# louiskirsch/speechT

Measured on AMD Instinct MI355X. Metric: utterances/sec (training step, 10 s@16 kHz, batch 32), higher is better.
Workload: dtype f32

## Files before the change

include/speecht_hip.h:

```cpp
#ifndef SPEECHT_HIP_H
#define SPEECHT_HIP_H

#include <stddef.h>
#include <stdint.h>

#ifdef __cplusplus
extern "C" {
#endif

#define ST_OK 0
#define ST_EINVAL (-1)
#define ST_ELAUNCH (-2)
#define ST_EWORKSPACE (-3)
#define ST_ECOMM (-4)

typedef struct st_tensor3 {
  float* base;
  int32_t batch;
  int32_t frames;
  int32_t channels;
  int32_t halo;
  int32_t t_pitch;
  int32_t c_pitch;
} st_tensor3;

int st_version(void);
const char* st_last_error(void);

int st_trace_begin(void);
int st_trace_begin_timed(void);
int st_trace_timed_filter(const char* text);
size_t st_trace_end(char* host_buf, size_t capacity);
int st_set_tuning(const char* name, int value);
uint32_t st_host_crc32c(const void* host_data, size_t n, uint32_t crc);

int st_packed_dims(int width, int cin_pitch, int cout, int* k_valid, int* k_pad, int* n_pad);
int st_pack_filters_f32(const float* filters, int width, int cin, int cout, int cin_pitch,
                        float* packed, void* stream);
int st_unpack_filters_f32(const float* packed, int width, int cin, int cout, int cin_pitch,
                          float* filters, void* stream);
int st_filters_flip_transpose_f32(const float* packed, int width, int cin, int cout,
                                  int cin_pitch, int cout_pitch, float* packed_t, void* stream);

int st_conv1d_nwc_fwd_f32(const st_tensor3* x, const float* packed, const float* bias, int width,
                          int stride, int pad_left, int relu, const st_tensor3* y, void* stream);
size_t st_conv1d_fwd_ws(const st_tensor3* x, const st_tensor3* y, int width);
int st_conv1d_nwc_fwd_ws_f32(const st_tensor3* x, const float* packed, const float* bias, int width,
                             int stride, int pad_left, int relu, const st_tensor3* y, void* workspace,
                             size_t workspace_bytes, void* stream);

int st_conv1d_fft_plan(int width, int frames, int batch, int* n, int* valid, int* blocks, int* bins, int* rows_pad);
int st_gemm_nn_batched_f32(const float* a, int64_t lda, int64_t a_batch, const float* b, int64_t b_batch, float* c,
                           int64_t ldc, int64_t c_batch, int m, int k, int n, int batches, void* stream);
size_t st_gemm_nn_batched_ws_bytes(void);
size_t st_gemm_nn_batched_ctrl_bytes(void);
int st_streamk_lost_ptr(void** device_word);
int st_streamk_lost_count(unsigned* count);
int st_streamk_lost_fetch_async(unsigned* host_word, void* stream);
int st_gemm_nn_batched_ws_f32(const float* a, int64_t lda, int64_t a_batch, const float* b, int64_t b_batch, float* c,
                              int64_t ldc, int64_t c_batch, int m, int k, int n, int batches, void* workspace,
                              size_t workspace_bytes, void* stream);
int st_gemm_nn_batched_bt_ws_f32(const float* a, int64_t lda, int64_t a_batch, const float* bt, int64_t bt_batch, float* c,
                                 int64_t ldc, int64_t c_batch, int m, int k, int n, int batches, void* workspace,
                                 size_t workspace_bytes, void* stream);
int st_gemm_tn_batched_f32(const float* a, int64_t lda, int64_t a_batch, const float* z, int64_t ldz, int64_t z_batch,
                           float* out, int64_t out_batch, int m, int k, int n, int batches, void* stream);
int st_gemm_tn_batched_shared_f32(const float* a, int64_t lda, int64_t a_batch, const float* z, int64_t ldz, int64_t z_batch,
                                  float* out, int64_t out_batch, int m, int k, int n, int batches, int z_batch_shift, void* stream);
int st_gemm_tn_batched_tile_f32(const float* a, int64_t lda, int64_t a_batch, const float* z, int64_t ldz, int64_t z_batch,
                                float* out, int64_t out_batch, int m, int k, int n, int batches, int z_batch_shift, int tile_n,
                                void* stream);
int st_gemm_nn_g3_batched_f32(const float* a, int64_t lda, int64_t a_batch, const int64_t* a_off, const float* b, int64_t ldb,
                              int64_t b_batch, const int64_t* b_off, int b_transposed, float* c, int64_t ldc, int64_t c_batch,
                              int64_t c_off2, int m, int k, int n, int batches, void* stream);
int st_gemm_tn_g3_batched_f32(const float* a, int64_t lda, int64_t a_batch, const int64_t* a_off, const float* z, int64_t ldz,
                              int64_t z_batch, const int64_t* z_off, float* out, int64_t out_batch, int64_t out_part, int m, int k,
                              int n, int batches, void* stream);
int st_conv1d_fft_three_products(int width, int cin_pitch, int cout);
size_t st_conv1d_fft_table_floats(void);
int st_conv1d_fft_tables_f32(int width, int pad_left, float* tables, size_t table_floats, void* stream);
size_t st_conv1d_fft_filter_floats(int width, int cin_pitch, int cout);
int st_conv1d_fft_filters_f32(const float* packed, int width, int cin, int cout, int cin_pitch, const float* tables, float* gfwd,
                              void* stream);
size_t st_conv1d_fft_sf_floats(const st_tensor3* x, const st_tensor3* y, int width);
size_t st_conv1d_fft_zf_floats(const st_tensor3* dz, int width);
size_t st_conv1d_fft_ws(const st_tensor3* x, const st_tensor3* y, int width);
int st_conv1d_nwc_fwd_fft_f32(const st_tensor3* x, const float* gfwd, const float* bias, int width, int pad_left, int relu,
                              const st_tensor3* y, const float* tables, float* sf, void* workspace,
                              size_t workspace_bytes, void* stream);
int st_conv1d_nwc_fwd_fft_chain_f32(const st_tensor3* x, const float* gfwd, const float* bias, int width, int pad_left, int relu,
                                    const st_tensor3* y, const float* tables, float* sf, int sf_ready, const float* next_tables,
                                    float* next_sf, int next_width, int next_pad_left, int* next_sf_written, void* workspace,
                                    size_t workspace_bytes, void* stream);
int st_conv1d_fft_dz_spectra_f32(const st_tensor3* dz, int width, const float* tables, float* zf, void* stream);
int st_conv1d_fft_bias_grad_f32(const st_tensor3* dz, int width, const float* zf, float* dbias, void* stream);
int st_conv1d_nwc_bwd_data_fft_f32(const st_tensor3* dz, const float* zf, const float* gfwd, int width, int pad_left,
                                   const st_tensor3* act, const st_tensor3* dx, const float* tables, void* workspace,
                                   size_t workspace_bytes, void* stream);
int st_conv1d_nwc_bwd_data_fft_chain_f32(const st_tensor3* dz, const float* zf, const float* gfwd, int width, int pad_left,
                                         const st_tensor3* act, const st_tensor3* dx, const float* tables, const float* below_tables,
                                         float* below_zf, int below_width, int* below_zf_written, void* workspace,
                                         size_t workspace_bytes, void* stream);
int st_conv1d_nwc_bwd_filter_fft_f32(const st_tensor3* x, const st_tensor3* dz, const float* sf, const float* zf, int width,
                                     const float* tables, float* dpacked, void* workspace, size_t workspace_bytes,
                                     void* stream);

size_t st_conv1d_fft_filter_plane_elems(int width, int cin_pitch, int cout);
int st_conv1d_fft_filters_planes(const float* packed, int width, int cin, int cout, int cin_pitch, const float* tables, void* g_planes,
                                 void* gt_planes, int planes, void* stream);
size_t st_conv1d_fft_planes_ws(const st_tensor3* x, const st_tensor3* y, int width, int planes);
int st_conv1d_nwc_fwd_fft_planes(const st_tensor3* x, const void* x_bf16, const void* gt_planes, const float* bias, int width,
                                 int pad_left, int relu, const st_tensor3* y, void* y_bf16, const float* tables, void* sf_planes,
                                 int planes, void* workspace, size_t workspace_bytes, void* stream);
int st_conv1d_fft_dz_spectra_planes(const st_tensor3* dz, const void* dz_bf16, int width, const float* tables, void* zf_planes,
                                    int planes, float* dc, void* stream);
int st_conv1d_fft_bias_grad_dc_f32(const float* dc, int rows, int channels, int n_pad, float* dbias, void* stream);
int st_conv1d_nwc_bwd_data_fft_planes(const st_tensor3* dz, const void* zf_planes, const void* g_planes, int width, int pad_left,
                                      const st_tensor3* act, const void* act_bf16, const st_tensor3* dx, void* dx_bf16,
                                      const float* tables, int planes, void* workspace, size_t workspace_bytes, void* stream);
int st_conv1d_nwc_bwd_filter_fft_planes(const st_tensor3* x, const st_tensor3* dz, const void* sf_planes, const void* zf_planes, int width,
                                        const float* tables, float* dpacked, int planes, void* workspace, size_t workspace_bytes,
                                        void* stream);

size_t st_conv1d_bwd_data_ws(const st_tensor3* dz, const st_tensor3* dx, int width);
int st_conv1d_nwc_bwd_data_f32(const st_tensor3* dz, const float* packed_t, int width,
                               int pad_left, const st_tensor3* act, const st_tensor3* dx,
                               void* workspace, size_t workspace_bytes, void* stream);
size_t st_conv1d_bwd_data_bias_ws(const st_tensor3* dz, const st_tensor3* dx, int width);
int st_conv1d_nwc_bwd_data_bias_f32(const st_tensor3* dz, const float* packed_t, int width, int pad_left,
                                    const st_tensor3* act, const st_tensor3* dx, float* dbias_dx,
                                    void* workspace, size_t workspace_bytes, void* stream);
int st_conv1d_1tap_bwd_data_bias_f32(const st_tensor3* dz, const float* packed, const st_tensor3* act, const st_tensor3* dx,
                                     float* dbias_dx, void* workspace, size_t workspace_bytes, void* stream);
size_t st_conv1d_bwd_filter_ws(const st_tensor3* x, const st_tensor3* dz, int width);
size_t st_bias_grad_ws(const st_tensor3* dz);
int st_bias_grad_f32(const st_tensor3* dz, float* dbias, void* workspace, size_t workspace_bytes, void* stream);
int st_conv1d_nwc_bwd_filter_f32(const st_tensor3* x, const st_tensor3* dz, int width, int stride,
                                 int pad_left, float* dpacked, float* dbias, void* workspace,
                                 size_t workspace_bytes, void* stream);

size_t st_ctc_ws(int batch, int frames, int max_label_len);
int st_ctc_loss_grad_f32(const st_tensor3* logits, const int32_t* label_ids,
                         const int32_t* label_offsets, const int32_t* seq_lens, int max_label_len,
                         float grad_scale, float* loss, const st_tensor3* grad, int32_t* status,
                         void* workspace, size_t workspace_bytes, void* stream);
int st_ctc_loss_grad_hilo_f32(const st_tensor3* logits, const int32_t* label_ids,
                              const int32_t* label_offsets, const int32_t* seq_lens, int max_label_len,
                              float grad_scale, float* loss, float* loss_lo, const st_tensor3* grad, int32_t* status,
                              void* workspace, size_t workspace_bytes, void* stream);

int st_ctc_greedy_decode(const st_tensor3* logits, const int32_t* seq_lens, int merge_repeated,
                         int32_t* ids, int max_out, int32_t* out_lens, float* neg_sum_logits,
                         void* stream);

size_t st_ctc_align_ws(int batch, int frames, int max_label_len);
int st_ctc_align_f32(const st_tensor3* logits, const int32_t* label_ids, const int32_t* label_offsets,
                     const int32_t* seq_lens, int max_label_len, int32_t* spans, int32_t* states, float* score,
                     int32_t* status, void* workspace, size_t workspace_bytes, void* stream);
int st_ctc_align_host(const float* logits, int batch, int frames, int classes, const int32_t* label_ids,
                      const int32_t* label_offsets, const int32_t* seq_lens, int max_label_len, int32_t* spans,
                      int32_t* states, float* score, int32_t* status, void* workspace, size_t workspace_bytes);

size_t st_ctc_align_long_ws(long frames, int label_len);
int st_ctc_align_long_f32(const float* logits, long frames, int classes, int row_pitch, const int32_t* label_ids, int label_len,
                          int32_t* spans, double* score, int32_t* status, void* workspace, size_t workspace_bytes,
                          void* stream);
int st_ctc_align_long_host(const float* logits, long frames, int classes, int row_pitch, const int32_t* label_ids, int label_len,
                           int32_t* spans, double* score, int32_t* status, void* workspace, size_t workspace_bytes);

size_t st_ctc_word_conf_ws(int batch, int frames, int max_label_len, int max_jobs);
int st_ctc_word_conf_f32(const st_tensor3* logits, const int32_t* label_ids, const int32_t* label_offsets,
                         const int32_t* seq_lens, int max_label_len, int space_id, const int32_t* word_spans, int n_words,
                         double* log_prob, double* log_conf, int32_t* status, void* workspace, size_t workspace_bytes,
                         void* stream);
int st_ctc_word_conf_host(const float* logits, int batch, int frames, int classes, const int32_t* label_ids,
                          const int32_t* label_offsets, const int32_t* seq_lens, int max_label_len, int space_id,
                          const int32_t* word_spans, int n_words, double* log_prob, double* log_conf, int32_t* status,
                          void* workspace, size_t workspace_bytes);

size_t st_ctc_spot_ws(int batch, int frames, int max_keyword_len, int n_jobs);
int st_ctc_spot_f32(const st_tensor3* logits, const int32_t* seq_lens, const int32_t* kw_ids, const int32_t* kw_offsets,
                    int n_keywords, int max_keyword_len, const int32_t* jobs, int n_jobs, double* score, int32_t* span,
                    double* trace_score, int32_t* trace_start, int32_t* status, void* workspace, size_t workspace_bytes,
                    void* stream);
int st_ctc_spot_host(const float* logits, int batch, int frames, int classes, const int32_t* seq_lens, const int32_t* kw_ids,
                     const int32_t* kw_offsets, int n_keywords, int max_keyword_len, const int32_t* jobs, int n_jobs,
                     double* score, int32_t* span, double* trace_score, int32_t* trace_start, int32_t* status, void* workspace,
                     size_t workspace_bytes);

size_t st_ctc_beam_ws(int batch, int frames, int beam_width);
int st_ctc_beam_search_decode(const st_tensor3* logits, const int32_t* seq_lens, int beam_width,
                              int32_t* ids, int max_out, int32_t* out_lens, float* log_prob,
                              void* workspace, size_t workspace_bytes, void* stream);
int st_ctc_beam_search_decode_ex(const st_tensor3* logits, const int32_t* seq_lens, int beam_width, int input_transform,
                                 int32_t* ids, int max_out, int32_t* out_lens, float* log_prob,
                                 void* workspace, size_t workspace_bytes, void* stream);

int st_lm_create_arpa(const char* text, size_t bytes, void** handle, char* err, size_t errlen);
int st_lm_info(void* handle, int* order, int64_t* counts, int64_t* skipped_words, int64_t* trie_nodes, size_t* device_bytes);
int st_lm_upload(void* handle, void* stream);
int st_lm_word_id(void* handle, const char* word, int32_t* id);
int st_lm_query_host(void* handle, const int32_t* ctx, int n, int32_t word, float* logp);
int st_lm_trie_lookup(void* handle, const char* prefix, int32_t* node, float* min_logp, int32_t* word);
int st_lm_destroy(void* handle);
int st_ctc_beam_search_decode_lm(const st_tensor3* logits, const int32_t* seq_lens, int beam_width, int input_transform, void* lm,
                                 float lm_weight, float word_count_weight, float valid_word_count_weight, float oov_score,
                                 int32_t* ids, int max_out, int32_t* out_lens, float* log_prob, void* workspace,
                                 size_t workspace_bytes, void* stream);
size_t st_ctc_beam_lm_candidates_ws(int batch, int frames, int beam_width, int candidates);
int st_ctc_beam_search_decode_lm_candidates(const st_tensor3* logits, const int32_t* seq_lens, int beam_width, int input_transform,
                                            void* lm, const float* weights, int candidates, float oov_score, int32_t* ids,
                                            int max_out, int32_t* out_lens, float* log_prob, void* workspace,
                                            size_t workspace_bytes, void* stream);

int st_ctc_beam_search_decode_nbest(const st_tensor3* logits, const int32_t* seq_lens, int beam_width, int input_transform, int n_best,
                                    int32_t* ids, int max_out, int32_t* out_lens, float* log_prob, int32_t* n_hyps, void* workspace,
                                    size_t workspace_bytes, void* stream);
int st_ctc_beam_search_decode_lm_nbest(const st_tensor3* logits, const int32_t* seq_lens, int beam_width, int input_transform, void* lm,
                                       float lm_weight, float word_count_weight, float valid_word_count_weight, float oov_score,
                                       int n_best, int32_t* ids, int max_out, int32_t* out_lens, float* log_prob, int32_t* n_hyps,
                                       void* workspace, size_t workspace_bytes, void* stream);

typedef struct st_bias_tables {
  const int32_t* next;
  const float* gain;
  const float* fin;
  int32_t n_states;
} st_bias_tables;
int st_ctc_beam_search_decode_bias_nbest(const st_tensor3* logits, const int32_t* seq_lens, int beam_width, int input_transform,
                                         const st_bias_tables* bias, int n_best, int32_t* ids, int max_out, int32_t* out_lens,
                                         float* log_prob, int32_t* n_hyps, void* workspace, size_t workspace_bytes, void* stream);
int st_ctc_beam_search_decode_lm_bias_nbest(const st_tensor3* logits, const int32_t* seq_lens, int beam_width, int input_transform,
                                            void* lm, float lm_weight, float word_count_weight, float valid_word_count_weight,
                                            float oov_score, const st_bias_tables* bias, int n_best, int32_t* ids, int max_out,
                                            int32_t* out_lens, float* log_prob, int32_t* n_hyps, void* workspace,
                                            size_t workspace_bytes, void* stream);

int st_lm_score_prefixes_f64(void* lm, const int32_t* ids, int pitch, const int32_t* lens, int n, double* g, int32_t* n_words,
                             int32_t* n_valid, void* stream);
int st_lm_score_prefixes_host(void* lm, const int32_t* ids, int pitch, const int32_t* lens, int n, double* g, int32_t* n_words,
                              int32_t* n_valid);

int st_edit_distance_max_len(void);
int st_edit_distance_pairs(const int32_t* expected, int expected_rows, int expected_pitch, const int32_t* expected_lens,
                           const int32_t* decoded, int decoded_rows, int decoded_pitch, const int32_t* decoded_lens,
                           const int32_t* pairs, int n_pairs, int32_t* distances, void* stream);

size_t st_global_norm_ws(size_t n);
int st_global_norm_clip_adam_f32(float* params, const float* grads, float* m, float* v, size_t n,
                                 float clip_norm, float lr_t, float beta1, float beta2, float eps,
                                 float* stats, void* workspace, size_t workspace_bytes,
                                 void* stream);
int st_ctc_status_gate_f32(const int32_t* status, int batch, float* gate, void* stream);
int st_ctc_status_gate_loss_f32(const int32_t* status, int batch, const float* loss_hi, const float* loss_lo, float loss_scale,
                                float* gate, void* stream);
int st_global_norm_clip_adam_gated_f32(float* params, const float* grads, float* m, float* v, size_t n,
                                       float clip_norm, float lr_t, float beta1, float beta2, float eps,
                                       float* stats, const float* gate, void* workspace,
// ... 224 lines not shown
```

speecht_amd/_lib.py:

```python
import ctypes
import os
from ctypes import POINTER, c_char_p, c_float, c_int, c_int32, c_int64, c_long, c_size_t, c_void_p

from .build import LIB_PATH


class Tensor3(ctypes.Structure):
  _fields_ = [('base', c_void_p), ('batch', c_int32), ('frames', c_int32), ('channels', c_int32),
              ('halo', c_int32), ('t_pitch', c_int32), ('c_pitch', c_int32)]


class BiasTables(ctypes.Structure):
  _fields_ = [('next', c_void_p), ('gain', c_void_p), ('fin', c_void_p), ('n_states', c_int32)]


class SpeechtHipError(RuntimeError):
  pass


_T3P = POINTER(Tensor3)
_SIGNATURES = {
    'st_version': (c_int, []),
    'st_last_error': (c_char_p, []),
    'st_trace_begin': (c_int, []),
    'st_trace_begin_timed': (c_int, []),
    'st_trace_timed_filter': (c_int, [c_char_p]),
    'st_trace_end': (c_size_t, [c_char_p, c_size_t]),
    'st_set_tuning': (c_int, [c_char_p, c_int]),
    'st_host_crc32c': (ctypes.c_uint32, [c_void_p, c_size_t, ctypes.c_uint32]),
    'st_packed_dims': (c_int, [c_int, c_int, c_int, POINTER(c_int), POINTER(c_int), POINTER(c_int)]),
    'st_pack_filters_f32': (c_int, [c_void_p, c_int, c_int, c_int, c_int, c_void_p, c_void_p]),
    'st_unpack_filters_f32': (c_int, [c_void_p, c_int, c_int, c_int, c_int, c_void_p, c_void_p]),
    'st_filters_flip_transpose_f32': (c_int, [c_void_p, c_int, c_int, c_int, c_int, c_int, c_void_p, c_void_p]),
    'st_conv1d_nwc_fwd_f32': (c_int, [_T3P, c_void_p, c_void_p, c_int, c_int, c_int, c_int, _T3P, c_void_p]),
    'st_conv1d_fwd_ws': (c_size_t, [_T3P, _T3P, c_int]),
    'st_conv1d_nwc_fwd_ws_f32': (c_int, [_T3P, c_void_p, c_void_p, c_int, c_int, c_int, c_int, _T3P, c_void_p, c_size_t,
                                          c_void_p]),
    'st_conv1d_fft_plan': (c_int, [c_int, c_int, c_int, POINTER(c_int), POINTER(c_int), POINTER(c_int), POINTER(c_int),
                                   POINTER(c_int)]),
    'st_gemm_nn_batched_f32': (c_int, [c_void_p, c_int64, c_int64, c_void_p, c_int64, c_void_p, c_int64, c_int64, c_int, c_int,
                                       c_int, c_int, c_void_p]),
    'st_gemm_nn_batched_ws_bytes': (c_size_t, []),
    'st_gemm_nn_batched_ctrl_bytes': (c_size_t, []),
    'st_streamk_lost_ptr': (c_int, [POINTER(c_void_p)]),
    'st_streamk_lost_count': (c_int, [POINTER(ctypes.c_uint32)]),
    'st_streamk_lost_fetch_async': (c_int, [c_void_p, c_void_p]),
    'st_gemm_nn_batched_ws_f32': (c_int, [c_void_p, c_int64, c_int64, c_void_p, c_int64, c_void_p, c_int64, c_int64, c_int, c_int,
                                          c_int, c_int, c_void_p, c_size_t, c_void_p]),
    'st_gemm_nn_batched_bt_ws_f32': (c_int, [c_void_p, c_int64, c_int64, c_void_p, c_int64, c_void_p, c_int64, c_int64, c_int, c_int,
                                             c_int, c_int, c_void_p, c_size_t, c_void_p]),
    'st_gemm_tn_batched_f32': (c_int, [c_void_p, c_int64, c_int64, c_void_p, c_int64, c_int64, c_void_p, c_int64, c_int, c_int,
                                       c_int, c_int, c_void_p]),
    'st_gemm_tn_batched_shared_f32': (c_int, [c_void_p, c_int64, c_int64, c_void_p, c_int64, c_int64, c_void_p, c_int64, c_int, c_int,
                                              c_int, c_int, c_int, c_void_p]),
    'st_gemm_tn_batched_tile_f32': (c_int, [c_void_p, c_int64, c_int64, c_void_p, c_int64, c_int64, c_void_p, c_int64, c_int, c_int,
                                            c_int, c_int, c_int, c_int, c_void_p]),
    'st_gemm_nn_g3_batched_f32': (c_int, [c_void_p, c_int64, c_int64, POINTER(c_int64), c_void_p, c_int64, c_int64, POINTER(c_int64), c_int,
                                          c_void_p, c_int64, c_int64, c_int64, c_int, c_int, c_int, c_int, c_void_p]),
    'st_gemm_tn_g3_batched_f32': (c_int, [c_void_p, c_int64, c_int64, POINTER(c_int64), c_void_p, c_int64, c_int64, POINTER(c_int64),
                                          c_void_p, c_int64, c_int64, c_int, c_int, c_int, c_int, c_void_p]),
    'st_conv1d_fft_three_products': (c_int, [c_int, c_int, c_int]),
    'st_conv1d_fft_table_floats': (c_size_t, []),
    'st_conv1d_fft_tables_f32': (c_int, [c_int, c_int, c_void_p, c_size_t, c_void_p]),
    'st_conv1d_fft_filter_floats': (c_size_t, [c_int, c_int, c_int]),
    'st_conv1d_fft_filters_f32': (c_int, [c_void_p, c_int, c_int, c_int, c_int, c_void_p, c_void_p, c_void_p]),
    'st_conv1d_fft_sf_floats': (c_size_t, [_T3P, _T3P, c_int]),
    'st_conv1d_fft_zf_floats': (c_size_t, [_T3P, c_int]),
    'st_conv1d_fft_ws': (c_size_t, [_T3P, _T3P, c_int]),
    'st_conv1d_nwc_fwd_fft_f32': (c_int, [_T3P, c_void_p, c_void_p, c_int, c_int, c_int, _T3P, c_void_p, c_void_p, c_void_p,
                                          c_size_t, c_void_p]),
    'st_conv1d_nwc_fwd_fft_chain_f32': (c_int, [_T3P, c_void_p, c_void_p, c_int, c_int, c_int, _T3P, c_void_p, c_void_p, c_int, c_void_p,
                                                c_void_p, c_int, c_int, POINTER(c_int), c_void_p, c_size_t, c_void_p]),
    'st_conv1d_nwc_bwd_data_fft_chain_f32': (c_int, [_T3P, c_void_p, c_void_p, c_int, c_int, _T3P, _T3P, c_void_p, c_void_p, c_void_p, c_int,
                                                     POINTER(c_int), c_void_p, c_size_t, c_void_p]),
    'st_conv1d_fft_filter_plane_elems': (c_size_t, [c_int, c_int, c_int]),
    'st_conv1d_fft_filters_planes': (c_int, [c_void_p, c_int, c_int, c_int, c_int, c_void_p, c_void_p, c_void_p, c_int, c_void_p]),
    'st_conv1d_fft_planes_ws': (c_size_t, [_T3P, _T3P, c_int, c_int]),
    'st_conv1d_nwc_fwd_fft_planes': (c_int, [_T3P, c_void_p, c_void_p, c_void_p, c_int, c_int, c_int, _T3P, c_void_p, c_void_p, c_void_p,
                                             c_int, c_void_p, c_size_t, c_void_p]),
    'st_conv1d_fft_dz_spectra_planes': (c_int, [_T3P, c_void_p, c_int, c_void_p, c_void_p, c_int, c_void_p, c_void_p]),
    'st_conv1d_fft_bias_grad_dc_f32': (c_int, [c_void_p, c_int, c_int, c_int, c_void_p, c_void_p]),
    'st_conv1d_nwc_bwd_data_fft_planes': (c_int, [_T3P, c_void_p, c_void_p, c_int, c_int, _T3P, c_void_p, _T3P, c_void_p, c_void_p, c_int,
                                                  c_void_p, c_size_t, c_void_p]),
    'st_conv1d_nwc_bwd_filter_fft_planes': (c_int, [_T3P, _T3P, c_void_p, c_void_p, c_int, c_void_p, c_void_p, c_int, c_void_p, c_size_t,
                                                    c_void_p]),
    'st_conv1d_fft_dz_spectra_f32': (c_int, [_T3P, c_int, c_void_p, c_void_p, c_void_p]),
    'st_conv1d_fft_bias_grad_f32': (c_int, [_T3P, c_int, c_void_p, c_void_p, c_void_p]),
    'st_conv1d_nwc_bwd_data_fft_f32': (c_int, [_T3P, c_void_p, c_void_p, c_int, c_int, _T3P, _T3P, c_void_p, c_void_p, c_size_t,
                                               c_void_p]),
    'st_conv1d_nwc_bwd_filter_fft_f32': (c_int, [_T3P, _T3P, c_void_p, c_void_p, c_int, c_void_p, c_void_p, c_void_p,
                                                 c_size_t, c_void_p]),
    'st_conv1d_bwd_data_ws': (c_size_t, [_T3P, _T3P, c_int]),
    'st_conv1d_nwc_bwd_data_f32': (c_int, [_T3P, c_void_p, c_int, c_int, _T3P, _T3P, c_void_p, c_size_t, c_void_p]),
    'st_conv1d_bwd_data_bias_ws': (c_size_t, [_T3P, _T3P, c_int]),
    'st_conv1d_nwc_bwd_data_bias_f32': (c_int, [_T3P, c_void_p, c_int, c_int, _T3P, _T3P, c_void_p, c_void_p, c_size_t,
                                                c_void_p]),
    'st_conv1d_1tap_bwd_data_bias_f32': (c_int, [_T3P, c_void_p, _T3P, _T3P, c_void_p, c_void_p, c_size_t, c_void_p]),
    'st_conv1d_bwd_filter_ws': (c_size_t, [_T3P, _T3P, c_int]),
    'st_conv1d_nwc_bwd_filter_f32': (c_int, [_T3P, _T3P, c_int, c_int, c_int, c_void_p, c_void_p, c_void_p,
                                             c_size_t, c_void_p]),
    'st_bias_grad_ws': (c_size_t, [_T3P]),
    'st_bias_grad_f32': (c_int, [_T3P, c_void_p, c_void_p, c_size_t, c_void_p]),
    'st_ctc_ws': (c_size_t, [c_int, c_int, c_int]),
    'st_ctc_loss_grad_f32': (c_int, [_T3P, c_void_p, c_void_p, c_void_p, c_int, c_float, c_void_p, _T3P,
                                     c_void_p, c_void_p, c_size_t, c_void_p]),
    'st_ctc_loss_grad_hilo_f32': (c_int, [_T3P, c_void_p, c_void_p, c_void_p, c_int, c_float, c_void_p, c_void_p, _T3P,
                                     c_void_p, c_void_p, c_size_t, c_void_p]),
    'st_ctc_greedy_decode': (c_int, [_T3P, c_void_p, c_int, c_void_p, c_int, c_void_p, c_void_p, c_void_p]),
    'st_ctc_align_ws': (c_size_t, [c_int, c_int, c_int]),
    'st_ctc_align_f32': (c_int, [_T3P, c_void_p, c_void_p, c_void_p, c_int, c_void_p, c_void_p, c_void_p, c_void_p,
                                 c_void_p, c_size_t, c_void_p]),
    'st_ctc_align_host': (c_int, [c_void_p, c_int, c_int, c_int, c_void_p, c_void_p, c_void_p, c_int, c_void_p, c_void_p,
                                  c_void_p, c_void_p, c_void_p, c_size_t]),
    'st_ctc_align_long_ws': (c_size_t, [c_long, c_int]),
    'st_ctc_align_long_f32': (c_int, [c_void_p, c_long, c_int, c_int, c_void_p, c_int, c_void_p, c_void_p, c_void_p, c_void_p,
                                      c_size_t, c_void_p]),
    'st_ctc_align_long_host': (c_int, [c_void_p, c_long, c_int, c_int, c_void_p, c_int, c_void_p, c_void_p, c_void_p, c_void_p,
                                       c_size_t]),
    'st_ctc_word_conf_ws': (c_size_t, [c_int, c_int, c_int, c_int]),
    'st_ctc_word_conf_f32': (c_int, [_T3P, c_void_p, c_void_p, c_void_p, c_int, c_int, c_void_p, c_int, c_void_p, c_void_p,
                                     c_void_p, c_void_p, c_size_t, c_void_p]),
    'st_ctc_word_conf_host': (c_int, [c_void_p, c_int, c_int, c_int, c_void_p, c_void_p, c_void_p, c_int, c_int, c_void_p, c_int,
                                      c_void_p, c_void_p, c_void_p, c_void_p, c_size_t]),
    'st_ctc_spot_ws': (c_size_t, [c_int, c_int, c_int, c_int]),
    'st_ctc_spot_f32': (c_int, [_T3P, c_void_p, c_void_p, c_void_p, c_int, c_int, c_void_p, c_int, c_void_p, c_void_p, c_void_p,
                                c_void_p, c_void_p, c_void_p, c_size_t, c_void_p]),
    'st_ctc_spot_host': (c_int, [c_void_p, c_int, c_int, c_int, c_void_p, c_void_p, c_void_p, c_int, c_int, c_void_p, c_int,
                                 c_void_p, c_void_p, c_void_p, c_void_p, c_void_p, c_void_p, c_size_t]),
    'st_ctc_beam_ws': (c_size_t, [c_int, c_int, c_int]),
    'st_ctc_beam_search_decode': (c_int, [_T3P, c_void_p, c_int, c_void_p, c_int, c_void_p, c_void_p, c_void_p,
                                          c_size_t, c_void_p]),
    'st_ctc_beam_search_decode_ex': (c_int, [_T3P, c_void_p, c_int, c_int, c_void_p, c_int, c_void_p, c_void_p, c_void_p,
                                             c_size_t, c_void_p]),
    'st_lm_create_arpa': (c_int, [c_char_p, c_size_t, POINTER(c_void_p), c_char_p, c_size_t]),
    'st_lm_info': (c_int, [c_void_p, POINTER(c_int), POINTER(c_int64), POINTER(c_int64), POINTER(c_int64), POINTER(c_size_t)]),
    'st_lm_upload': (c_int, [c_void_p, c_void_p]),
    'st_lm_word_id': (c_int, [c_void_p, c_char_p, POINTER(c_int32)]),
    'st_lm_query_host': (c_int, [c_void_p, POINTER(c_int32), c_int, c_int32, POINTER(c_float)]),
    'st_lm_trie_lookup': (c_int, [c_void_p, c_char_p, POINTER(c_int32), POINTER(c_float), POINTER(c_int32)]),
    'st_lm_destroy': (c_int, [c_void_p]),
    'st_ctc_beam_search_decode_lm': (c_int, [_T3P, c_void_p, c_int, c_int, c_void_p, c_float, c_float, c_float, c_float, c_void_p,
                                             c_int, c_void_p, c_void_p, c_void_p, c_size_t, c_void_p]),
    'st_ctc_beam_lm_candidates_ws': (c_size_t, [c_int, c_int, c_int, c_int]),
    'st_ctc_beam_search_decode_lm_candidates': (c_int, [_T3P, c_void_p, c_int, c_int, c_void_p, POINTER(c_float), c_int, c_float,
                                                        c_void_p, c_int, c_void_p, c_void_p, c_void_p, c_size_t, c_void_p]),
    'st_ctc_beam_search_decode_nbest': (c_int, [_T3P, c_void_p, c_int, c_int, c_int, c_void_p, c_int, c_void_p, c_void_p, c_void_p,
                                                c_void_p, c_size_t, c_void_p]),
    'st_ctc_beam_search_decode_lm_nbest': (c_int, [_T3P, c_void_p, c_int, c_int, c_void_p, c_float, c_float, c_float, c_float, c_int,
                                                   c_void_p, c_int, c_void_p, c_void_p, c_void_p, c_void_p, c_size_t, c_void_p]),
    'st_ctc_beam_search_decode_bias_nbest': (c_int, [_T3P, c_void_p, c_int, c_int, c_void_p, c_int, c_void_p, c_int, c_void_p, c_void_p,
                                                     c_void_p, c_void_p, c_size_t, c_void_p]),
    'st_ctc_beam_search_decode_lm_bias_nbest': (c_int, [_T3P, c_void_p, c_int, c_int, c_void_p, c_float, c_float, c_float, c_float,
                                                        c_void_p, c_int, c_void_p, c_int, c_void_p, c_void_p, c_void_p, c_void_p,
                                                        c_size_t, c_void_p]),
    'st_lm_score_prefixes_f64': (c_int, [c_void_p, c_void_p, c_int, c_void_p, c_int, c_void_p, c_void_p, c_void_p, c_void_p]),
    'st_lm_score_prefixes_host': (c_int, [c_void_p, c_void_p, c_int, c_void_p, c_int, c_void_p, c_void_p, c_void_p]),
    'st_edit_distance_max_len': (c_int, []),
    'st_edit_distance_pairs': (c_int, [c_void_p, c_int, c_int, c_void_p, c_void_p, c_int, c_int, c_void_p, c_void_p, c_int, c_void_p,
                                       c_void_p]),
    'st_global_norm_ws': (c_size_t, [c_size_t]),
    'st_global_norm_clip_adam_f32': (c_int, [c_void_p, c_void_p, c_void_p, c_void_p, c_size_t, c_float, c_float,
                                             c_float, c_float, c_float, c_void_p, c_void_p, c_size_t, c_void_p]),
    'st_ctc_status_gate_f32': (c_int, [c_void_p, c_int, c_void_p, c_void_p]),
    'st_ctc_status_gate_loss_f32': (c_int, [c_void_p, c_int, c_void_p, c_void_p, c_float, c_void_p, c_void_p]),
    'st_global_norm_clip_adam_gated_f32': (c_int, [c_void_p, c_void_p, c_void_p, c_void_p, c_size_t, c_float, c_float,
                                                   c_float, c_float, c_float, c_void_p, c_void_p, c_void_p, c_size_t,
                                                   c_void_p]),
    'st_global_norm_clip_adam_counted_f32': (c_int, [c_void_p, c_void_p, c_void_p, c_void_p, c_size_t, c_float, ctypes.c_double,
                                                     ctypes.c_double, ctypes.c_double, c_float, c_void_p, c_void_p, c_void_p, c_void_p,
                                                     c_size_t, c_void_p]),
    'st_global_norm_f32': (c_int, [c_void_p, c_size_t, c_float, c_void_p, c_void_p, c_size_t, c_void_p]),
    'st_melspec_plan_bytes': (c_size_t, []),
    'st_melspec_plan_f32': (c_int, [c_void_p, c_int, c_int, c_void_p, c_size_t, c_void_p]),
    'st_melspec_planned_f32': (c_int, [c_void_p, c_void_p, c_int, c_int64, c_void_p, c_int, c_int, c_int, c_void_p,
                                       c_int64, c_void_p, c_void_p, c_size_t, c_void_p]),
    'st_melspec_ws': (c_size_t, [c_int, c_int64, c_int]),
    'st_melspec_f32': (c_int, [c_void_p, c_void_p, c_int, c_int64, c_void_p, c_int, c_int, c_int, c_void_p,
                               c_int64, c_void_p, c_void_p, c_size_t, c_void_p]),
    'st_cast_bf16': (c_int, [c_void_p, c_size_t, c_void_p, c_void_p]),
    'st_filters_bf16': (c_int, [c_void_p, c_int, c_int, c_void_p, c_void_p]),
    'st_filters_bwd_bf16': (c_int, [c_void_p, c_int, c_int, c_int, c_int, c_int, c_void_p, c_void_p]),
    'st_conv1d_nwc_fwd_bf16': (c_int, [_T3P, c_void_p, c_void_p, c_void_p, c_int, c_int, c_int, c_int, _T3P, c_void_p,
                                       c_void_p, c_void_p]),
    'st_conv1d_fwd_bf16_ws': (c_size_t, [_T3P, _T3P, c_int]),
    'st_conv1d_nwc_fwd_ws_bf16': (c_int, [_T3P, c_void_p, c_void_p, c_void_p, c_int, c_int, c_int, c_int, _T3P, c_void_p,
                                          c_void_p, c_void_p, c_size_t, c_void_p]),
    'st_conv1d_bwd_data_bf16_ws': (c_size_t, [_T3P, _T3P, c_int]),
    'st_conv1d_nwc_bwd_data_bf16': (c_int, [_T3P, c_void_p, c_void_p, c_int, c_int, _T3P, c_void_p, _T3P, c_void_p,
                                            c_void_p, c_size_t, c_void_p]),
    'st_conv1d_bwd_filter_bf16_ws': (c_size_t, [_T3P, _T3P, c_int, c_int, c_int]),
    'st_conv1d_nwc_bwd_filter_bf16': (c_int, [_T3P, c_void_p, _T3P, c_void_p, c_int, c_int, c_int, c_void_p, c_void_p,
                                              c_void_p, c_size_t, c_void_p]),
    'st_conv1d_bwd_filter_tr_bf16_slack_rows': (c_int, []),
    'st_conv1d_bwd_filter_tr_bf16_ws': (c_size_t, [_T3P, _T3P, c_int, c_int, c_int]),
    'st_conv1d_nwc_bwd_filter_tr_bf16': (c_int, [_T3P, c_void_p, _T3P, c_void_p, c_int, c_int, c_int, c_void_p, c_void_p,
                                                 c_void_p, c_size_t, c_void_p]),
    'st_comm_unique_id_bytes': (c_int, []),
    'st_comm_unique_id': (c_int, [c_void_p, c_size_t]),
    'st_comm_init': (c_int, [c_void_p, c_size_t, c_int, c_int, POINTER(c_void_p)]),
    'st_comm_destroy': (c_int, [c_void_p]),
    'st_comm_count': (c_int, [c_void_p, POINTER(c_int)]),
    'st_allreduce_f32': (c_int, [c_void_p, c_void_p, c_size_t, c_void_p]),
    'st_allreduce_buckets_f32': (c_int, [c_void_p, c_void_p, POINTER(c_size_t), POINTER(c_size_t), c_int, c_void_p]),
    'st_mfcc_ws': (c_size_t, [c_int, c_int64, c_int, c_int]),
    'st_mfcc_f32': (c_int, [c_void_p, c_void_p, c_int, c_int64, c_void_p, c_int, c_int, c_int, c_int, c_void_p,
                            c_int64, c_void_p, c_void_p, c_size_t, c_void_p]),
    'st_resample_kaiser_f32': (c_int, [c_void_p, c_void_p, c_int, c_void_p, c_int, c_void_p, c_void_p, c_int64, c_void_p, c_int64,
                                       c_void_p, c_void_p]),
    'st_resample_kaiser_host': (c_int, [c_void_p, c_void_p, c_int, c_void_p, c_int, c_void_p, c_void_p, c_void_p, c_int64, c_void_p]),
    'st_resample_stream_state_bytes': (c_size_t, [c_int, c_int]),
    'st_resample_stream_f32': (c_int, [c_void_p, c_void_p, c_int, c_int, c_void_p, c_int64, c_void_p, c_size_t, c_int, c_void_p, c_int64,
                                       c_void_p, c_void_p]),
    'st_resample_stream_host': (c_int, [c_void_p, c_void_p, c_int, c_int, c_void_p, c_int64, c_void_p, c_size_t, c_int, c_void_p, c_void_p,
                                        c_int64, c_void_p]),
    'st_segment_chunks_f32': (c_int, [c_void_p, c_void_p, c_void_p, c_void_p, c_int, c_int64, c_float, c_void_p, c_void_p, c_void_p,
                                      c_void_p, c_void_p, c_void_p]),
    'st_segment_runs': (c_int, [c_void_p, c_void_p, c_void_p, c_int, c_int, c_int, c_void_p, c_void_p, c_void_p, c_void_p, c_void_p,
                                c_void_p, c_void_p, c_void_p]),
    'st_segment_gather_f32': (c_int, [c_void_p, c_void_p, c_void_p, c_void_p, c_void_p, c_int, c_int64, c_void_p, c_void_p]),
    'st_mask_rows': (c_int, [_T3P, c_void_p, c_int, c_void_p]),
    'st_stream_conv_slices': (c_int, [c_int, c_int, c_int, POINTER(c_int), POINTER(c_int)]),
    'st_stream_conv_ws': (c_size_t, [c_int, c_int, c_int, c_int]),
    'st_stream_conv_f32': (c_int, [c_void_p, c_int, c_int, c_void_p, c_void_p, c_int, c_int, c_void_p, c_void_p, c_int, c_int, c_int,
                                   c_int, c_void_p, c_int, c_int, c_void_p, c_void_p, c_size_t, c_void_p]),
    'st_stream_feed_f32': (c_int, [c_void_p, c_int, c_void_p, c_int, c_int, c_void_p, c_int, c_int, c_void_p]),
    'st_stream_advance': (c_int, [c_void_p, c_int, c_void_p, c_int, c_void_p]),
    'st_melspec_stream_state_bytes': (c_size_t, [c_int, c_int, c_int, c_int]),
    'st_melspec_stream_ws': (c_size_t, [c_int, c_int]),
    'st_melspec_stream_f32': (c_int, [c_void_p, c_void_p, c_int, c_int, c_void_p, c_int, c_int, c_int, c_int, c_int, c_float, c_float,
                                      c_float, c_void_p, c_size_t, c_void_p, c_int, c_int, c_void_p, c_size_t, c_void_p]),
    'st_ctc_greedy_stream': (c_int, [c_void_p, c_int, c_int, c_void_p, c_void_p, c_int, c_void_p, c_void_p, c_void_p, c_int, c_void_p,
                                     c_void_p, c_void_p]),
    'st_ctc_beam_stream_state_bytes': (c_size_t, [c_int, c_int]),
    'st_ctc_beam_stream_pool_bytes': (c_size_t, [c_int, c_int]),
    'st_ctc_beam_stream_ws': (c_size_t, [c_int]),
    'st_ctc_beam_stream_step': (c_int, [c_void_p, c_int, c_int, c_void_p, c_void_p, c_int, c_int, c_int, c_int, c_void_p, c_float, c_float,
                                        c_float, c_float, c_void_p, c_void_p, c_int, c_void_p, c_size_t, c_void_p]),
    'st_ctc_beam_stream_read': (c_int, [c_void_p, c_int, c_int, c_void_p, c_float, c_float, c_float, c_float, c_void_p, c_void_p, c_int,
                                        c_void_p, c_int, c_void_p, c_void_p]),
    'st_stream_endpoint_state_bytes': (c_size_t, []),
    'st_stream_endpoint_score_bytes': (c_size_t, []),
    'st_stream_endpoint_pieces': (c_int, [c_int, c_int, c_int, c_int]),
    'st_ctc_greedy_endpoint_stream': (c_int, [c_void_p, c_int, c_int, c_void_p, c_void_p, c_int, c_int, c_int, c_int, c_int, c_int, c_void_p,
                                              c_void_p, c_void_p, c_int, c_void_p, c_void_p, c_void_p, c_void_p, c_int, c_void_p]),
    'st_stream_endpoint_host': (c_int, [c_void_p, c_int, c_int, c_void_p, c_void_p, c_int, c_int, c_int, c_int, c_int, c_int, c_void_p,
                                        c_void_p, c_void_p, c_int, c_void_p, c_void_p, c_void_p, c_void_p, c_int]),
    'st_ctc_beam_stream_step_pieces': (c_int, [c_void_p, c_int, c_int, c_void_p, c_void_p, c_int, c_int, c_int, c_int, c_int, c_void_p,
                                               c_float, c_float, c_float, c_float, c_void_p, c_void_p, c_int, c_void_p, c_size_t, c_void_p,
                                               c_int, c_void_p, c_void_p]),
    'st_ctc_beam_stream_bias_state_bytes': (c_size_t, [c_int, c_int]),
    'st_ctc_beam_stream_step_bias': (c_int, [c_void_p, c_int, c_int, c_void_p, c_void_p, c_int, c_int, c_int, c_int, c_void_p, c_float,
                                             c_float, c_float, c_float, c_void_p, c_void_p, c_int, c_void_p, c_size_t, c_void_p, c_void_p,
                                             c_void_p]),
    'st_ctc_beam_stream_read_bias': (c_int, [c_void_p, c_int, c_int, c_void_p, c_float, c_float, c_float, c_float, c_void_p, c_void_p,
                                             c_int, c_void_p, c_int, c_void_p, c_void_p, c_void_p, c_void_p]),
    'st_ctc_beam_stream_step_pieces_bias': (c_int, [c_void_p, c_int, c_int, c_void_p, c_void_p, c_int, c_int, c_int, c_int, c_int, c_void_p,
                                                    c_float, c_float, c_float, c_float, c_void_p, c_void_p, c_int, c_void_p, c_size_t,
                                                    c_void_p, c_int, c_void_p, c_void_p, c_void_p, c_void_p]),
    'st_ctc_beam_stream_read_nbest': (c_int, [c_void_p, c_int, c_int, c_void_p, c_float, c_float, c_float, c_float, c_void_p, c_void_p,
                                              c_int, c_void_p, c_int, c_void_p, c_void_p, c_void_p, c_void_p, c_int, c_void_p, c_int,
                                              c_void_p]),
    'st_ctc_beam_stream_step_pieces_nbest': (c_int, [c_void_p, c_int, c_int, c_void_p, c_void_p, c_int, c_int, c_int, c_int, c_int, c_void_p,
                                                     c_float, c_float, c_float, c_float, c_void_p, c_void_p, c_int, c_void_p, c_size_t,
                                                     c_void_p, c_int, c_void_p, c_void_p, c_void_p, c_void_p, c_int, c_void_p, c_int,
                                                     c_void_p]),
    'st_stream_keep_rows': (c_int, [c_int, c_int]),
    'st_stream_keep_f32': (c_int, [c_void_p, c_int, c_int, c_void_p, c_int, c_int, c_void_p, c_int, c_void_p]),
    'st_ctc_align_ring_f32': (c_int, [c_void_p, c_int, c_int, c_int, c_void_p, c_int, c_int, c_void_p, c_void_p, c_int, c_void_p, c_void_p,
                                      c_void_p, c_void_p, c_void_p, c_size_t, c_void_p]),
    'st_ctc_align_ring_host': (c_int, [c_void_p, c_int, c_int, c_int, c_void_p, c_int, c_int, c_void_p, c_void_p, c_int, c_void_p, c_void_p,
                                       c_void_p, c_void_p, c_void_p, c_size_t]),
    'st_ctc_word_conf_ring_f32': (c_int, [c_void_p, c_int, c_int, c_int, c_void_p, c_int, c_int, c_void_p, c_void_p, c_int, c_int, c_void_p,
                                          c_int, c_void_p, c_void_p, c_void_p, c_void_p, c_size_t, c_void_p]),
    'st_ctc_word_conf_ring_host': (c_int, [c_void_p, c_int, c_int, c_int, c_void_p, c_int, c_int, c_void_p, c_void_p, c_int, c_int, c_void_p,
                                           c_int, c_void_p, c_void_p, c_void_p, c_void_p, c_size_t]),
    'st_ctc_spot_stream_plan_bytes': (c_size_t, [c_void_p, c_void_p, c_int, c_int, c_int]),
    'st_ctc_spot_stream_plan': (c_int, [c_void_p, c_void_p, c_int, c_int, c_int, c_void_p, c_void_p]),
    'st_ctc_spot_stream_plan_bind': (c_int, [c_void_p, c_void_p]),
    'st_ctc_spot_stream_state_bytes': (c_size_t, [c_void_p]),
    'st_ctc_spot_stream_step': (c_int, [c_void_p, c_int, c_int, c_void_p, c_void_p, c_int, c_int, c_void_p, ctypes.c_double, c_int,
                                        c_void_p, c_void_p, c_int, c_void_p, c_void_p]),
    'st_ctc_spot_stream_host': (c_int, [c_void_p, c_int, c_int, c_void_p, c_void_p, c_int, c_int, c_void_p, ctypes.c_double, c_int,
                                        c_void_p, c_void_p, c_int, c_void_p]),
    'st_ctc_follow_stream_state_bytes': (c_size_t, [c_int]),
    'st_ctc_follow_stream_ws': (c_size_t, [c_int, c_int, c_int]),
    'st_ctc_follow_stream_step': (c_int, [c_void_p, c_int, c_int, c_void_p, c_void_p, c_int, c_int, c_int, c_int, c_void_p, c_void_p,
                                          c_void_p, c_void_p, c_int, c_int, c_void_p, c_void_p, c_int, c_void_p, c_void_p, c_void_p,
                                          c_size_t, c_void_p]),
    'st_ctc_follow_stream_host': (c_int, [c_void_p, c_int, c_int, c_void_p, c_void_p, c_int, c_int, c_int, c_int, c_void_p, c_void_p,
                                          c_void_p, c_void_p, c_int, c_int, c_void_p, c_void_p, c_int, c_void_p, c_void_p, c_void_p,
                                          c_size_t]),
    'st_spec_augment_f32': (c_int, [c_void_p, c_int, c_int, c_int, c_void_p, c_void_p, ctypes.c_uint64, c_int, c_int, c_int, c_int, c_int,
                                    c_int, _T3P, c_void_p, c_void_p]),
    'st_spec_augment_host': (c_int, [c_void_p, c_int, c_int, c_int, c_void_p, c_void_p, ctypes.c_uint64, c_int, c_int, c_int, c_int, c_int,
                                     c_int, _T3P, c_void_p]),
    'st_spec_augment_plan_host': (c_int, [c_void_p, c_void_p, c_int, c_int, ctypes.c_uint64, c_int, c_int, c_int, c_int, c_int, c_int,
                                          c_void_p]),
    'st_fill_f32': (c_int, [c_void_p, c_float, c_size_t, c_void_p]),
    'st_zero_halos_f32': (c_int, [_T3P, c_void_p]),
    'st_zero_regions': (c_int, [c_void_p, c_int, c_void_p]),
}
EXPORTED_SYMBOLS = tuple(_SIGNATURES)

_EXPERIMENTAL = {
    'st_exp_split3_bf16': (c_int, [c_void_p, c_size_t, c_void_p, c_void_p]),
    'st_exp_split3_transpose_bf16': (c_int, [c_void_p, c_int, c_int, c_void_p, c_void_p]),
    'st_exp_conv1d_fwd_bf16x6': (c_int, [_T3P, c_void_p, c_void_p, c_void_p, c_int, c_int, c_int, c_int, _T3P,
                                         c_void_p, c_void_p]),
    'st_exp_conv1d_bwd_data_bf16x6_ws': (c_size_t, [_T3P, _T3P, c_int]),
    'st_exp_conv1d_bwd_data_bf16x6': (c_int, [_T3P, c_void_p, c_void_p, c_int, c_int, _T3P, _T3P, c_void_p, c_void_p, c_size_t,
                                              c_void_p]),
    'st_exp_transpose_split3_bf16': (c_int, [_T3P, c_int, c_int, c_int, c_size_t, c_void_p, c_void_p]),
    'st_exp_conv1d_bwd_filter_bf16x6': (c_int, [c_void_p, c_void_p, c_int, c_int, c_int, c_int, c_int, c_int, c_void_p, c_void_p]),
}

_lib = None


def load():
  global _lib
  if _lib is None:
    import torch
    bundled = os.path.join(os.path.dirname(torch.__file__), 'lib', 'libamdhip64.so')
    if os.path.exists(bundled):
      ctypes.CDLL(bundled, mode=ctypes.RTLD_GLOBAL)
    if not os.path.exists(LIB_PATH):
      raise SpeechtHipError('{} is missing: build it with `python -c "import __graft_entry__ as g; g.build()"` '
                            '(there is no CPU fallback)'.format(LIB_PATH))
    lib = ctypes.CDLL(LIB_PATH)
    for name, (res, args) in list(_SIGNATURES.items()) + list(_EXPERIMENTAL.items()):
      fn = getattr(lib, name)
      fn.restype = res
      fn.argtypes = args
    _lib = lib
    for item in filter(None, os.environ.get('ST_TUNE', '').split(',')):
      name, _, value = item.partition('=')
      check(lib.st_set_tuning(name.strip().encode(), int(value)), 'ST_TUNE ' + item)
  return _lib


def check(code, what):
  if code != 0:
    raise SpeechtHipError('{} failed ({}): {}'.format(what, code, load().st_last_error().decode()))


def call(name, *args):
  check(getattr(load(), name)(*args), name)


class launch_trace:

  def __init__(self, timed=False, only=None):
    self.timed, self.only = timed, only

  def __enter__(self):
    if self.timed:
      load().st_trace_timed_filter((self.only or '').encode())
      load().st_trace_begin_timed()
    else:
      load().st_trace_begin()
    self.lines = []
    return self

  def __exit__(self, *exc):
    lib = load()
    need = lib.st_trace_end(None, 0)
    buf = ctypes.create_string_buffer(int(need))
    lib.st_trace_end(buf, need)
    self.lines = [l for l in buf.value.decode().split('\n') if l]
    return False


TUNING_EPOCH = [0]


def set_tuning(name, value):
  TUNING_EPOCH[0] += 1
  call('st_set_tuning', name.encode(), int(value))
```

speecht_amd/csrc/api.hip:

```cpp
#include <algorithm>
#include <atomic>
#include <mutex>
#include <string>
#include <vector>
#include <string.h>

#include "st_common.h"

namespace st {
static thread_local char g_err[512] = "";
void set_error(const char* fmt, ...) {
  va_list ap;
  va_start(ap, fmt);
  vsnprintf(g_err, sizeof(g_err), fmt, ap);
  va_end(ap);
}

static std::atomic<int> g_trace_on{0};
static std::mutex g_trace_mu;
static std::vector<std::string> g_lines;
constexpr int kMaxTimed = 1 << 14;
struct TimedLaunch { int line; hipEvent_t e0, e1; };
static std::vector<TimedLaunch> g_timed;
static thread_local int g_last_line = -1;
static std::string g_timed_filter;
bool trace_on() { return g_trace_on.load(std::memory_order_relaxed) != 0; }
void trace(const char* fmt, ...) {
  if (!trace_on()) return;
  char line[320];
  va_list ap;
  va_start(ap, fmt);
  vsnprintf(line, sizeof(line), fmt, ap);
  va_end(ap);
  std::lock_guard<std::mutex> lock(g_trace_mu);
  if (g_lines.size() < (1u << 16)) {
    g_last_line = (int)g_lines.size();
    g_lines.emplace_back(line);
  } else {
    g_last_line = -1;
  }
}
LaunchTimer::LaunchTimer(hipStream_t) : start_(nullptr), stop_(nullptr) {
  const int line = g_last_line;
  g_last_line = -1;
  if (g_trace_on.load(std::memory_order_relaxed) != 2 || line < 0) return;
  hipEvent_t e0 = nullptr, e1 = nullptr;
  if (hipEventCreate(&e0) != hipSuccess) return;
  if (hipEventCreate(&e1) != hipSuccess) { hipEventDestroy(e0); return; }
  std::lock_guard<std::mutex> lock(g_trace_mu);
  if ((int)g_timed.size() >= kMaxTimed || line >= (int)g_lines.size() ||
      (!g_timed_filter.empty() && g_lines[line].find(g_timed_filter) == std::string::npos)) {
    hipEventDestroy(e0);
    hipEventDestroy(e1);
    return;
  }
  g_timed.push_back(TimedLaunch{line, e0, e1});
  start_ = e0;
  stop_ = e1;
}

static const char* const kTuneNames[TUNE_COUNT] = {"streamk", "streamk_slots", "streamk_test_drop", "no_fused_transforms",
                                                   "bf16_lag_copies", "filters_idft_valu", "bf16_taps_panel", "no_g3", "g3_tile"};
static std::atomic<int> g_tune[TUNE_COUNT];
int tuning(int key) { return g_tune[key].load(std::memory_order_relaxed); }
}

extern "C" {
int st_version(void) { return 200; }
const char* st_last_error(void) { return st::g_err; }

static int trace_begin(int mode) {
  std::lock_guard<std::mutex> lock(st::g_trace_mu);
  st::g_lines.clear();
  for (auto& t : st::g_timed) { hipEventDestroy(t.e0); hipEventDestroy(t.e1); }
  st::g_timed.clear();
  st::g_last_line = -1;
  st::g_trace_on.store(mode);
  return ST_OK;
}
int st_trace_begin(void) { return trace_begin(1); }
int st_trace_begin_timed(void) { return trace_begin(2); }
int st_trace_timed_filter(const char* text) {
  std::lock_guard<std::mutex> lock(st::g_trace_mu);
  st::g_timed_filter = text ? text : "";
  return ST_OK;
}

size_t st_trace_end(char* host_buf, size_t capacity) {
  st::g_trace_on.store(0);
  std::lock_guard<std::mutex> lock(st::g_trace_mu);
  for (auto& t : st::g_timed) {
    float ms = -1.f;
    if (hipEventSynchronize(t.e1) != hipSuccess || hipEventElapsedTime(&ms, t.e0, t.e1) != hipSuccess) ms = -1.f;
    char tail[48];
    snprintf(tail, sizeof(tail), " ms=%.5f", ms);
    if (t.line >= 0 && t.line < (int)st::g_lines.size()) st::g_lines[t.line] += tail;
    hipEventDestroy(t.e0);
    hipEventDestroy(t.e1);
  }
  st::g_timed.clear();
  size_t need = 1;
  for (const auto& l : st::g_lines) need += l.size() + 1;
  if (host_buf && capacity > 0) {
    size_t at = 0;
    for (const auto& l : st::g_lines) {
      if (at + l.size() + 1 >= capacity) break;
      memcpy(host_buf + at, l.data(), l.size());
      at += l.size();
      host_buf[at++] = '\n';
    }
    host_buf[at] = 0;
  }
  return need;
}

uint32_t st_host_crc32c(const void* host_data, size_t n, uint32_t crc) {
  static uint32_t table[8][256];
  static std::once_flag once;
  std::call_once(once, [] {
    for (uint32_t i = 0; i < 256; ++i) {
      uint32_t c = i;
      for (int k = 0; k < 8; ++k) c = (c >> 1) ^ (0x82F63B78u & (0u - (c & 1u)));
      table[0][i] = c;
    }
    for (uint32_t i = 0; i < 256; ++i)
      for (int t = 1; t < 8; ++t) table[t][i] = (table[t - 1][i] >> 8) ^ table[0][table[t - 1][i] & 0xFF];
  });
  const unsigned char* p = reinterpret_cast<const unsigned char*>(host_data);
  crc = ~crc;
  while (n >= 8) {
    uint32_t lo, hi;
    memcpy(&lo, p, 4);
    memcpy(&hi, p + 4, 4);
    lo ^= crc;
    crc = table[7][lo & 0xFF] ^ table[6][(lo >> 8) & 0xFF] ^ table[5][(lo >> 16) & 0xFF] ^ table[4][lo >> 24] ^
          table[3][hi & 0xFF] ^ table[2][(hi >> 8) & 0xFF] ^ table[1][(hi >> 16) & 0xFF] ^ table[0][hi >> 24];
    p += 8;
    n -= 8;
  }
  while (n--) crc = (crc >> 8) ^ table[0][(crc ^ *p++) & 0xFF];
  return ~crc;
}

int st_set_tuning(const char* name, int value) {
  ST_REQUIRE(name, "st_set_tuning: null name");
  for (int i = 0; i < st::TUNE_COUNT; ++i)
    if (!strcmp(name, st::kTuneNames[i])) {
      st::g_tune[i].store(value);
      return ST_OK;
    }
  st::set_error("st_set_tuning: unknown knob '%s'", name);
  return ST_EINVAL;
}
}
```

speecht_amd/csrc/conv_fft.hip:

```cpp
#include <algorithm>

#include "st_common.h"

namespace {

typedef float f32x2 __attribute__((ext_vector_type(2)));
typedef float f32x4 __attribute__((ext_vector_type(4)));
typedef float f32x16 __attribute__((ext_vector_type(16)));

constexpr int V = 64;
constexpr int KP = 96;
constexpr int HB = KP / 2;
constexpr int T_FS = 0;
constexpr int T_FZ = T_FS + KP * KP;
constexpr int T_IY = T_FZ + KP * KP;
constexpr int T_IX = T_IY + V * KP;
constexpr int T_TW = T_IX + 3 * V * KP;
constexpr int T_FW = T_TW + 256;
constexpr int T_FP = T_FW + HB * 34 * 2;
constexpr int FUSE_BLOCKS = 8, FUSE_HALO = 4, FUSE_Q = 32 + FUSE_HALO;
constexpr int T_IW = T_FP + FUSE_Q * KP * 2;
constexpr int T_ZP = T_IW + KP * KP;
constexpr int T_END = T_ZP + 32 * KP * 2;
__host__ __device__ inline int fused_column(int q, int hh, int n, int pad_left) {
  const int right = n - V - pad_left;
  if (q < 32) return pad_left + 32 * (q >> 4) + (q & 3) + 8 * ((q & 15) >> 2) + 4 * hh;
  if (hh == 0) return (q - 32) < pad_left ? (q - 32) : -1;
  return (q - 32) < right ? V + pad_left + (q - 32) : -1;
}

int half_of(int cp) { return (int)st::round_up(cp, 64); }

struct Plan {
  int n, blocks, bins, rows, rows_pad;
};
constexpr int ROWS_F32 = 64;
Plan make_plan(int width, int frames, int batch, int row_granule = 128) {
  Plan p;
  p.n = V + width - 1;
  p.blocks = st::ceil_div(frames, V);
  p.bins = p.n / 2 + 1;
  p.rows = batch * p.blocks;
  p.rows_pad = (int)st::round_up(p.rows, row_granule);
  return p;
}

__global__ void tables_kernel(int n, int pad_left, float* __restrict__ t) {
  const int bins = n / 2 + 1, width = n - V + 1;
  const float inv_n = 1.f / (float)n;
  for (int i = blockIdx.x * blockDim.x + threadIdx.x; i < T_END; i += gridDim.x * blockDim.x) {
    float val = 0.f;
    if (i < T_IY) {
      const int z = i >= T_FZ, r = (i - (z ? T_FZ : T_FS)) / KP, col = (i - (z ? T_FZ : T_FS)) % KP;
      const int k = r < HB ? r : r - HB;
      if (k < bins && col < (z ? V : n)) {
        float sn, cs;
        sincospif(2.0f * (float)((k * col) % n) * inv_n, &sn, &cs);
        val = r < HB ? cs : -sn;
      }
    } else if (i < T_TW) {
      const int which = i < T_IX ? 0 : 1 + (i - T_IX) / (V * KP);
      const int rem = i < T_IX ? i - T_IY : (i - T_IX) % (V * KP);
      const int tp = rem / KP, col = rem % KP;
      const int k = col < HB ? col : col - HB;
      int m = tp;
      if (which == 1) m = tp + pad_left;
      if (which == 2) m = tp + V + pad_left;
      if (which == 3) m = tp - V + pad_left;
      if (k < bins && m >= 0 && m < n) {
        const float wk = (k == 0 || 2 * k == n) ? inv_n : 2.f * inv_n;
        float sn, cs;
        sincospif(2.0f * (float)((k * m) % n) * inv_n, &sn, &cs);
        val = col < HB ? wk * cs : -wk * sn;
      }
    } else if (i < T_FW) {
      const int j = (i - T_TW) / 2;
      if (j < n) {
        float sn, cs;
        sincospif(2.0f * (float)j * inv_n, &sn, &cs);
        val = (i - T_TW) % 2 ? sn : cs;
      }
    } else if (i < T_FP) {
      const int e = (i - T_FW) / 2, k = e / width, w = e % width;
      if (k < bins) {
        float sn, cs;
        sincospif(2.0f * (float)((k * w) % n) * inv_n, &sn, &cs);
        val = (i - T_FW) % 2 ? sn : cs;
      }
    } else if (i < T_IW) {
      const int e = i - T_FP, q = e / (KP * 2), r = (e - q * (KP * 2)) >> 1, hh = e & 1;
      const int k = r < HB ? r : r - HB, col = fused_column(q, hh, n, pad_left);
      if (k < bins && col >= 0 && col < n) {
        float sn, cs;
        sincospif(2.0f * (float)((k * col) % n) * inv_n, &sn, &cs);
        val = r < HB ? cs : -sn;
      }
    } else if (i < T_ZP) {
      const int e = i - T_IW, r = e / KP, col = e % KP;
      const int k = col < HB ? col : col - HB;
      int m = -1;
      if (r < V) m = r + pad_left;
      else if (r < V + 4) m = (r - V) < pad_left ? r - V : -1;
      else if (r < V + 8) m = (r - V - 4) < width - 1 - pad_left ? V + pad_left + (r - V - 4) : -1;
      if (k < bins && m >= 0 && m < n) {
        const float wk = (k == 0 || 2 * k == n) ? inv_n : 2.f * inv_n;
        float sn, cs;
        sincospif(2.0f * (float)((k * m) % n) * inv_n, &sn, &cs);
        val = col < HB ? wk * cs : -wk * sn;
      }
    } else {
      const int e = i - T_ZP, q = e / (KP * 2), r = (e - q * (KP * 2)) >> 1, hh = e & 1;
      const int k = r < HB ? r : r - HB, col = fused_column(q, hh, V, 0);
      if (k < bins && col < V) {
        float sn, cs;
        sincospif(2.0f * (float)((k * col) % n) * inv_n, &sn, &cs);
        val = r < HB ? cs : -sn;
      }
    }
    t[i] = val;
  }
}

struct RowsIn {
  const float* base;
  const unsigned short* base_b;
  long batch_stride;
  int c_pitch, channels_read;
  int t_lo, t_hi;
};

constexpr int CH = 12;

template <int R, int COUNT = 1>
__device__ inline void stage_matrix(float* __restrict__ dst, const float* __restrict__ src) {
  constexpr int IT = R * KP / 4 / 256;
  static_assert(IT * 256 * 4 == R * KP, "the matrix must be a whole number of 256-thread passes");
  f32x4 v[COUNT * IT];
#pragma unroll
  for (int it = 0; it < COUNT * IT; ++it) v[it] = reinterpret_cast<const f32x4*>(src)[threadIdx.x + 256 * it];
#pragma unroll
  for (int it = 0; it < COUNT * IT; ++it) {
    const int m = it / IT, i = threadIdx.x + 256 * (it % IT);
    const int row = (i * 4) / KP, k = (i * 4) % KP;
    f32x2* d = reinterpret_cast<f32x2*>(dst + m * R * KP) + ((k >> 1) * R + row);
    d[0] = f32x2{v[it][0], v[it][1]};
    d[R] = f32x2{v[it][2], v[it][3]};
  }
}

__device__ __forceinline__ void split3_bits(float x, unsigned short& h, unsigned short& m, unsigned short& l) {
  const __bf16 bh = (__bf16)x;
  const float r1 = x - (float)bh;
  const __bf16 bm = (__bf16)r1;
  const __bf16 bl = (__bf16)(r1 - (float)bm);
// ... 320 lines not shown
    else { if (j + 1 < blocks && e < right_next) v = halo[j + 1][0][e][l31]; }
#pragma unroll
    for (int i = 0; i < 3; ++i) sacc[i] = __builtin_amdgcn_mfma_f32_32x32x2f32(af2[((32 + e) * KP + i * 32) * 2], v, sacc[i], 0, 0, 0);
  }
  if (c < half_next) {
#pragma unroll
    for (int i = 0; i < 3; ++i)
#pragma unroll
      for (int r = 0; r < 16; ++r) {
        const int m = i * 32 + (r & 3) + 8 * (r >> 2) + 4 * h;
        const int bin = m < HB ? m : m - HB, col = (m < HB ? 0 : half_next) + c;
        if (bin < bins_next) {
          const long o = (long)bin * bin_stride + (long)row * 2 * half_next;
          out[o + col] = sacc[i][r];
          if (out2) out2[o + (m < HB ? half_next : 0) + c] = m < HB ? -sacc[i][r] : sacc[i][r];
        }
      }
  }
}

template <int HP>
__global__ __launch_bounds__(64 * FUSE_BLOCKS, 1) void idft_ola_dft_rows_kernel(
    const float* __restrict__ in, const float* __restrict__ winv, int blocks, int rows_pad, int bins, int half_in, int nchunks, RowsOut y,
    int pad_left, int right, const float* __restrict__ mask, long mask_batch_stride, int mask_c_pitch,
    const float* __restrict__ wz_below, int bins_below, int half_below, float* __restrict__ zf_below) {
  constexpr int NST = 2 * HP / CH;
  static_assert(2 * HP % CH == 0 && HP <= HB / 2, "pairs per term must fill whole stages");
  __shared__ __attribute__((aligned(16))) float wl[KP * KP];
  __shared__ __attribute__((aligned(16))) float wf[32 * KP * 2];
  constexpr int SPILL = FUSE_BLOCKS * FUSE_HALO * 32;
  constexpr bool SPILL_IN_WL = (HB / 2 - HP) * KP * 2 >= SPILL;
  __shared__ float spill_own[SPILL_IN_WL ? 32 : 2 * SPILL];
  float* const spill_before = SPILL_IN_WL ? wl + HP * KP * 2 : spill_own;
  float* const spill_after = SPILL_IN_WL ? wl + (HB / 2 + HP) * KP * 2 : spill_own + SPILL;
  const int tid = threadIdx.x, lane = tid & 63, l31 = lane & 31, h = lane >> 5;
  const int wave = __builtin_amdgcn_readfirstlane(tid >> 6);
  const int b = blockIdx.x / nchunks, chunk = blockIdx.x - b * nchunks;
  const int j = wave, row = b * blocks + j, c = chunk * 32 + l31;
  const bool active = j < blocks;
  const long plane = (long)rows_pad * 2 * half_in;
  const bool cok = c < half_in;
  const float* src = in + (long)(active ? row : 0) * 2 * half_in + min(c, half_in - 1);
  auto load = [&](float (&bf)[CH], int st) {
#pragma unroll
    for (int s = 0; s < CH; ++s) {
      const int p = st * CH + s;
      const int bin = (p < HP ? 2 * p : 2 * (p - HP)) + h;
      bf[s] = src[(long)min(bin, bins - 1) * plane + (p < HP ? 0 : half_in)];
    }
  };
  float bfr[NST][CH];
  float mk[2][16];
  if (active) {
#pragma unroll
    for (int st = 0; st < NST; ++st) load(bfr[st], st);
    if (mask) {
      const float* mp = mask + (long)b * mask_batch_stride + min(c, mask_c_pitch - 1);
#pragma unroll
      for (int i = 0; i < 2; ++i)
#pragma unroll
        for (int r = 0; r < 16; ++r)
          mk[i][r] = mp[(long)min(j * V + i * 32 + (r & 3) + 8 * (r >> 2) + 4 * h, y.frames - 1) * mask_c_pitch];
    }
  }
  if (tid < 256) stage_matrix<KP, 1>(wl, winv);
  if (wz_below) {
    constexpr int N4 = 32 * KP * 2 / 4;
    for (int idx = tid; idx < N4; idx += 64 * FUSE_BLOCKS) reinterpret_cast<f32x4*>(wf)[idx] = reinterpret_cast<const f32x4*>(wz_below)[idx];
  }
  __syncthreads();
  f32x16 acc[3];
#pragma unroll
  for (int i = 0; i < 3; ++i)
#pragma unroll
    for (int r = 0; r < 16; ++r) acc[i][r] = 0.f;
  if (active) {
    const float* afrag = wl + 2 * l31 + h;
#pragma unroll
    for (int st = 0; st < NST; ++st) {
      __builtin_amdgcn_sched_barrier(0);
#pragma unroll
      for (int s = 0; s < CH; ++s) {
        const int p = st * CH + s;
        const int bin = (p < HP ? 2 * p : 2 * (p - HP)) + h;
        const unsigned keep = (cok && bin < bins) ? 0xffffffffu : 0u;
        const float v = __uint_as_float(__float_as_uint(bfr[st][s]) & keep);
        const int sidx = p < HP ? p : HB / 2 + (p - HP);
#pragma unroll
        for (int i = 0; i < 3; ++i) acc[i] = __builtin_amdgcn_mfma_f32_32x32x2f32(afrag[(sidx * KP + i * 32) * 2], v, acc[i], 0, 0, 0);
      }
      __builtin_amdgcn_sched_barrier(0);
    }
#pragma unroll
    for (int e = 0; e < FUSE_HALO; ++e) (h ? spill_after : spill_before)[(j * FUSE_HALO + e) * 32 + l31] = acc[2][e];
  }
  __syncthreads();
  if (!active) return;
#pragma unroll
  for (int e = 0; e < FUSE_HALO; ++e) {
    if (h == 0) { if (j > 0 && e < right) acc[0][e] += spill_after[((j - 1) * FUSE_HALO + e) * 32 + l31]; }
    else { if (j + 1 < blocks && e >= FUSE_HALO - pad_left) acc[1][12 + e] += spill_before[((j + 1) * FUSE_HALO + e - (FUSE_HALO - pad_left)) * 32 + l31]; }
  }
#pragma unroll
  for (int i = 0; i < 2; ++i)
#pragma unroll
    for (int r = 0; r < 16; ++r) {
      const int t = j * V + i * 32 + (r & 3) + 8 * (r >> 2) + 4 * h;
      float val = c < y.channels ? acc[i][r] : 0.f;
      if (mask) val = mk[i][r] > 0.f ? val : 0.f;
      val = t < y.frames ? val : 0.f;
      asm volatile("" : "+v"(val));
      acc[i][r] = val;
    }
  if (c < y.c_pitch) {
    float* yp = y.base + (long)b * y.batch_stride + c;
#pragma unroll
    for (int i = 0; i < 2; ++i)
#pragma unroll
      for (int r = 0; r < 16; ++r) {
        const int t = j * V + i * 32 + (r & 3) + 8 * (r >> 2) + 4 * h;
        if (t < y.frames) yp[(long)t * y.c_pitch] = acc[i][r];
      }
  }
  if (!wz_below) return;
  f32x16 sacc[3];
#pragma unroll
  for (int i = 0; i < 3; ++i)
#pragma unroll
    for (int r = 0; r < 16; ++r) sacc[i][r] = 0.f;
  const float* af2 = wf + 2 * l31 + h;
#pragma unroll
  for (int q = 0; q < 32; ++q) {
    const float v = acc[q >> 4][q & 15];
#pragma unroll
    for (int i = 0; i < 3; ++i) sacc[i] = __builtin_amdgcn_mfma_f32_32x32x2f32(af2[(q * KP + i * 32) * 2], v, sacc[i], 0, 0, 0);
  }
  if (c < half_below) {
    const long zplane = (long)rows_pad * 2 * half_below;
#pragma unroll
    for (int i = 0; i < 3; ++i)
#pragma unroll
      for (int r = 0; r < 16; ++r) {
        const int m = i * 32 + (r & 3) + 8 * (r >> 2) + 4 * h;
        const int bin = m < HB ? m : m - HB, col = (m < HB ? 0 : half_below) + c;
        if (bin < bins_below) zf_below[(long)bin * zplane + (long)row * 2 * half_below + col] = sacc[i][r];
      }
  }
}

template <int WT, int OUTP = 0>
__global__ __launch_bounds__(256) void filters_dft_fwd_kernel(const float* __restrict__ packed, int width_rt, int cin, int cout,
                                                              int cpi, int cph, int npo, int n, int bins,
                                                              const f32x2* __restrict__ tw, float* __restrict__ gfwd,
                                                              unsigned short* __restrict__ gb, size_t g_plane) {
  const int width = WT ? WT : width_rt;
  const int o = blockIdx.x * 256 + threadIdx.x, c = blockIdx.y;
  if (o >= npo) return;
  float f[WT ? WT : 64];
  const bool live = c < cin && o < cout;
#pragma unroll
  for (int w = 0; w < width; ++w) f[w] = live ? packed[((long)w * cpi + c) * npo + o] : 0.f;
  const long plane = (long)2 * cph * 2 * npo;
  const int per = (bins + gridDim.z - 1) / gridDim.z, k_lo = blockIdx.z * per, k_hi = min(bins, k_lo + per);
  for (int k = k_lo; k < k_hi; ++k) {
    float gr = 0.f, gi = 0.f;
    const f32x2* row = tw + k * width;
#pragma unroll
    for (int w = 0; w < width; ++w) {
      const f32x2 t = row[w];
      gr = fmaf(f[w], t[0], gr);
      gi = fmaf(-f[w], t[1], gi);
    }
    auto put = [&](long o_, float v) {
      if (OUTP == 0) gfwd[o_] = v;
      else if (OUTP == 1) gb[o_] = __builtin_bit_cast(unsigned short, (__bf16)v);
      else {
        unsigned short sh, sm, sl;
        split3_bits(v, sh, sm, sl);
        gb[o_] = sh; gb[g_plane + o_] = sm; gb[2 * g_plane + o_] = sl;
      }
    };
    if constexpr (OUTP == 4) {
      const long g3 = (long)k * 3 * cph * npo + (long)c * npo + o;
      gfwd[g3] = gr;
      gfwd[g3 + (long)cph * npo] = gi - gr;
      gfwd[g3 + 2L * cph * npo] = -(gr + gi);
      continue;
    }
    const long g0 = (long)k * plane;
    put(g0 + (long)c * 2 * npo + o, gr);
    put(g0 + (long)c * 2 * npo + npo + o, -gi);
    put(g0 + (long)(cph + c) * 2 * npo + o, gi);
    put(g0 + (long)(cph + c) * 2 * npo + npo + o, gr);
  }
}

template <int WT>
__global__ __launch_bounds__(256) void filters_idft_kernel(const float* __restrict__ q, int width_rt, int cin, int cout, int cpi, int cph,
                                                           int npo, int n, int bins, const f32x2* __restrict__ tw,
                                                           float* __restrict__ dpacked, int split) {
  const int width = WT ? WT : width_rt;
  const int o = blockIdx.x * 256 + threadIdx.x, c = blockIdx.y;
  if (o >= npo) return;
  float acc[WT ? WT : 64];
#pragma unroll
  for (int w = 0; w < width; ++w) acc[w] = 0.f;
  const bool live = c < cin && o < cout;
  const long plane = split ? (long)2 * cph * npo : (long)2 * cph * 2 * npo;
  const float inv_n = 1.f / (float)n;
  if (live) {
    for (int k = 0; k < bins; ++k) {
      const float* p = q + (long)k * plane;
      const float wk = (k == 0 || 2 * k == n) ? inv_n : 2.f * inv_n;
      float re, im;
      if (split) {
        re = p[(long)c * npo + o] * wk;
        im = p[(long)cph * npo + (long)c * npo + o] * wk;
      } else {
        re = (p[(long)c * 2 * npo + o] + p[(long)(cph + c) * 2 * npo + npo + o]) * wk;
        im = (p[(long)(cph + c) * 2 * npo + o] - p[(long)c * 2 * npo + npo + o]) * wk;
      }
      const f32x2* row = tw + k * width;
#pragma unroll
      for (int w = 0; w < width; ++w) {
        const f32x2 t = row[w];
        acc[w] = fmaf(re, t[0], acc[w]);
        acc[w] = fmaf(-im, t[1], acc[w]);
      }
    }
  }
#pragma unroll
  for (int w = 0; w < width; ++w) dpacked[((long)w * cpi + c) * npo + o] = acc[w];
}

constexpr int FI_CH = 12;
constexpr int FI_SMAX = 96;
struct IdftParts { long off[4]; };
template <int VW>
__global__ __launch_bounds__(256, 2) void filters_idft_mfma_kernel(const float* __restrict__ q, int width, int cin, int cout, int cpi,
                                                                   int npo, int n, int bins, const f32x2* __restrict__ tw,
                                                                   float* __restrict__ dpacked, int pshift, long plane, IdftParts parts,
                                                                   int ld, int ochunks, int items) {
  typedef float vec __attribute__((ext_vector_type(VW)));
  __shared__ float tl[FI_SMAX * 32 * 2];
  const int nparts = 1 << pshift, S = (nparts * bins) >> 1, stages = (S + FI_CH - 1) / FI_CH;
  {
    const float inv_n = 1.f / (float)n;
    for (int i = threadIdx.x; i < stages * FI_CH * 64; i += 256) {
      const int hh = i & 1, m = (i >> 1) & 31, sidx = i >> 6;
      float v = 0.f;
      if (sidx < S && m < width) {
        const int kk = 2 * sidx + hh, k = kk >> pshift, part = kk & (nparts - 1);
        const float wk = (k == 0 || 2 * k == n) ? inv_n : 2.f * inv_n;
        const f32x2 t = tw[k * width + m];
        if (nparts == 2) v = part == 0 ? wk * t[0] : -wk * t[1];
        else v = part < 2 ? wk * t[0] : (part == 2 ? -wk * t[1] : wk * t[1]);
      }
      tl[i] = v;
    }
  }
  __syncthreads();
  const int lane = threadIdx.x & 63, l31 = lane & 31, h = lane >> 5;
  const int gw = blockIdx.x * 4 + (threadIdx.x >> 6), total = gridDim.x * 4;
  const float* afrag = tl + 2 * l31 + h;
  for (int item = gw; item < items; item += total) {
    const int c = item / ochunks, o0 = (item - c * ochunks) * (32 * VW) + l31 * VW;
    f32x16 acc[VW];
#pragma unroll
    for (int e = 0; e < VW; ++e)
#pragma unroll
      for (int r = 0; r < 16; ++r) acc[e][r] = 0.f;
    if (c < cin) {
      const float* base = q + (long)c * ld + o0;
      auto load = [&](vec (&bf)[FI_CH], int st) {
#pragma unroll
        for (int j = 0; j < FI_CH; ++j) {
          const int kk = 2 * min(st * FI_CH + j, S - 1) + h;
          bf[j] = *reinterpret_cast<const vec*>(base + (long)(kk >> pshift) * plane + parts.off[kk & (nparts - 1)]);
        }
      };
      auto mac = [&](const vec (&bf)[FI_CH], int st) {
        const float* a = afrag + st * (FI_CH * 64);
#pragma unroll
        for (int j = 0; j < FI_CH; ++j)
#pragma unroll
          for (int e = 0; e < VW; ++e) {
            acc[e] = __builtin_amdgcn_mfma_f32_32x32x2f32(a[j * 64], bf[j][e], acc[e], 0, 0, 0);
          }
      };
      vec bfr[2][FI_CH];
      load(bfr[0], 0);
      for (int st = 0; st < stages; st += 2) {
        if (st + 1 < stages) load(bfr[1], st + 1);
        __builtin_amdgcn_sched_barrier(0);
        mac(bfr[0], st);
        __builtin_amdgcn_sched_barrier(0);
        if (st + 1 < stages) {
          if (st + 2 < stages) load(bfr[0], st + 2);
          __builtin_amdgcn_sched_barrier(0);
          mac(bfr[1], st + 1);
          __builtin_amdgcn_sched_barrier(0);
        }
      }
    }
    if (c < cpi) {
#pragma unroll
      for (int r = 0; r < 16; ++r) {
        const int w = (r & 3) + 8 * (r >> 2) + 4 * h;
        if (w < width) {
          vec v;
#pragma unroll
          for (int e = 0; e < VW; ++e) {
            v[e] = o0 + e < cout ? acc[e][r] : 0.f;
          }
          *reinterpret_cast<vec*>(dpacked + ((long)w * cpi + c) * npo + o0) = v;
        }
      }
    }
  }
}

__global__ __launch_bounds__(256) void bias_from_spectra_kernel(const float* __restrict__ zf, int rows, int ld, int channels, int np,
                                                                float* __restrict__ dbias) {
  __shared__ float red[8][33];
  const int cl = threadIdx.x & 31, r = threadIdx.x >> 5;
  const int c = blockIdx.x * 32 + cl;
  float s = 0.f;
  if (c < channels) {
    float p0 = 0.f, p1 = 0.f, p2 = 0.f, p3 = 0.f;
    int k = r;
    for (; k + 24 < rows; k += 32) {
      const float a = zf[(long)k * ld + c], b = zf[(long)(k + 8) * ld + c], d = zf[(long)(k + 16) * ld + c],
                  e = zf[(long)(k + 24) * ld + c];
      p0 += a; p1 += b; p2 += d; p3 += e;
    }
    for (; k < rows; k += 8) p0 += zf[(long)k * ld + c];
    s = (p0 + p1) + (p2 + p3);
  }
  red[r][cl] = s;
  __syncthreads();
  if (r == 0 && c < np) {
    float t = red[0][cl];
#pragma unroll
    for (int k = 1; k < 8; ++k) t += red[k][cl];
    dbias[c] = t;
  }
}

RowsIn rows_in(const st_tensor3& t) {
  RowsIn r;
  r.base_b = nullptr;
  r.base = t.base + (long)t.halo * t.c_pitch;
  r.batch_stride = (long)t.t_pitch * t.c_pitch;
  r.c_pitch = t.c_pitch;
  r.channels_read = t.c_pitch;
  r.t_lo = -t.halo;
  r.t_hi = t.t_pitch - t.halo;
  return r;
}

constexpr int TRANSFORM_WGS_DEFAULT = 512;

void launch_dft(const st_tensor3& t, const void* tb, const Plan& pl, const float* wm, int start, int frames_used, int half, float* out,
                void* outb, int planes, size_t out_plane, float* dc, hipStream_t s, long bin_stride = 0, float* out2 = nullptr,
                int form = 0) {
  if (bin_stride == 0) bin_stride = (long)pl.rows_pad * (form == 4 ? 4 : form == 5 ? 3 : 2) * half;
  const int nchunks = st::ceil_div(half, 32);
  const int wgs = std::min(TRANSFORM_WGS_DEFAULT, st::ceil_div(pl.rows_pad * nchunks, 4));
  const int nst = frames_used <= 6 * CH ? 3 : 4;
  const double esz_in = tb ? 2.0 : 4.0, esz_out = planes == 0 ? 4.0 : 2.0 * planes;
  st::trace("dft_rows<%d%s%s> rows=%d chunks=%d bins=%d gflop=%.3f mb=%.2f", nst, tb ? ",bf16-in" : "",
            planes == 1 ? ",bf16-out" : planes == 3 ? ",x3-out" : form == 4 ? ",4-part" : form == 5 ? ",3-part" : "",
            pl.rows, nchunks, pl.bins, 4096e-9 * pl.rows * (double)nchunks * nst * CH * 3,
            1e-6 * ((double)t.batch * t.frames * t.c_pitch * esz_in +
                    (double)pl.bins * pl.rows * half * esz_out * (form == 4 ? 4 : form == 5 ? 3 : out2 ? 4 : 2)));
  RowsIn x = rows_in(t);
  if (tb) x.base_b = reinterpret_cast<const unsigned short*>(tb) + (long)t.halo * t.c_pitch;
  unsigned short* ob = reinterpret_cast<unsigned short*>(outb);
  st::LaunchTimer timer(s);
#define ST_DFT(NSTV, INB, OUTPV)                                                                                         \
  st::launch_timed(timer, dft_rows_kernel<NSTV, INB, OUTPV>, dim3(wgs), dim3(256), s, x, wm, pl.blocks, pl.rows, pl.rows_pad, start, \
                   pl.bins, half, nchunks, out, ob, out_plane, dc, bin_stride, out2)
#define ST_DFT_N(INB, OUTPV) do { if (nst == 3) ST_DFT(3, INB, OUTPV); else ST_DFT(4, INB, OUTPV); } while (0)
  if (!tb && planes == 0 && form == 4) ST_DFT_N(false, 4);
  else if (!tb && planes == 0 && form == 5) ST_DFT_N(false, 5);
  else if (!tb && planes == 0) ST_DFT_N(false, 0);
  else if (!tb && planes == 3) ST_DFT_N(false, 3);
  else if (tb && planes == 1) ST_DFT_N(true, 1);
  else st::set_error("dft: unsupported operand form (bf16 in: %d, planes %d)", tb ? 1 : 0, planes);
#undef ST_DFT_N
#undef ST_DFT
}

template <int TERMS>
void launch_idft(const float* in, const float* winv, const Plan& p, int half_in, int nchunks, const RowsOut& out, const float* bias,
                 int relu, const void* mask, long mask_batch_stride, int mask_c_pitch, hipStream_t s) {
  const dim3 grid(std::min(TRANSFORM_WGS_DEFAULT, st::ceil_div(p.rows * nchunks, 4)));
  const int hp = p.bins <= 36 ? 18 : 24;
  const bool bf = out.base_b != nullptr;
  st::trace("idft_rows<%d,%d%s> rows=%d chunks=%d bins=%d gflop=%.3f mb=%.2f", TERMS, hp, bf ? ",bf16" : "", p.rows, nchunks, p.bins,
            4096e-9 * p.rows * (double)nchunks * 2 * hp * (TERMS + 1),
            1e-6 * ((double)p.bins * p.rows * 2 * half_in * 4 + (double)p.rows * V * out.c_pitch * (bf ? 2.0 : 4.0) * (mask ? 2 : 1)));
  const float* mk = reinterpret_cast<const float*>(mask);
  st::LaunchTimer timer(s);
#define ST_IDFT(HPV, BFV)                                                                                                     \
  st::launch_timed(timer, idft_rows_kernel<TERMS, HPV, BFV>, grid, dim3(256), s, in, winv, p.blocks, p.rows, p.rows_pad, p.bins, half_in, \
                   nchunks, out, bias, relu, mk, mask_batch_stride, mask_c_pitch)
  if (p.bins <= 36) { if (bf) ST_IDFT(18, true); else ST_IDFT(18, false); }
  else { if (bf) ST_IDFT(24, true); else ST_IDFT(24, false); }
#undef ST_IDFT
}

bool width_ok(int width) { return width >= 2 && V + width - 1 <= KP && (V + width - 1) / 2 + 1 <= HB; }
constexpr int G3_MIN_WIDTH = 2 * FUSE_HALO + 2;
bool zf3_form(int width, int cout) { return width >= G3_MIN_WIDTH && st::npad_of(cout) >= 512 && st::tuning(st::TUNE_NO_G3) == 0; }
bool g3_form(int width, int cin_pitch, int cout) { return zf3_form(width, cout) && half_of(cin_pitch) % 128 == 0; }
bool split_lag_products(int half) { return half % 128 == 0; }

template <int OUTP>
void launch_filters_planes(int width, const dim3& grid, hipStream_t s, const float* packed, int cin, int cout, int cin_pitch, int cph,
                           int npo, int n, int bins, const f32x2* tw, unsigned short* gb, size_t g_plane) {
  float* none = nullptr;
  if (width == 32) hipLaunchKernelGGL((filters_dft_fwd_kernel<32, OUTP>), grid, dim3(256), 0, s, packed, width, cin, cout, cin_pitch, cph, npo, n, bins, tw, none, gb, g_plane);
  else if (width == 25) hipLaunchKernelGGL((filters_dft_fwd_kernel<25, OUTP>), grid, dim3(256), 0, s, packed, width, cin, cout, cin_pitch, cph, npo, n, bins, tw, none, gb, g_plane);
  else if (width == 7) hipLaunchKernelGGL((filters_dft_fwd_kernel<7, OUTP>), grid, dim3(256), 0, s, packed, width, cin, cout, cin_pitch, cph, npo, n, bins, tw, none, gb, g_plane);
  else hipLaunchKernelGGL((filters_dft_fwd_kernel<0, OUTP>), grid, dim3(256), 0, s, packed, width, cin, cout, cin_pitch, cph, npo, n, bins, tw, none, gb, g_plane);
}

bool planes_ok(int planes) { return planes == 1 || planes == 3; }

bool can_fuse_next(const Plan& p, const st_tensor3& y, int next_width, int next_pad_left) {
  if (next_width < 2 || !width_ok(next_width) || next_pad_left < 0 || next_pad_left >= next_width) return false;
  const int right = next_width - 1 - next_pad_left;
  return p.blocks <= FUSE_BLOCKS && p.rows == p.rows_pad && next_pad_left <= FUSE_HALO && right <= FUSE_HALO &&
         half_of(y.c_pitch) == y.c_pitch && y.c_pitch % 32 == 0 && st::tuning(st::TUNE_NO_FUSED_TRANSFORMS) == 0;
}


void launch_filters_idft(const float* qf, int width, int cin, int cout, int cpi, int cph, int npo, int n, int bins, const f32x2* tw,
                         float* dpacked, int split, hipStream_t s) {
  if (width <= 32 && npo % 128 == 0 && (split ? 2 : 4) * bins <= 2 * FI_SMAX && st::tuning(st::TUNE_FILTERS_IDFT_VALU) == 0) {
    IdftParts parts;
    long plane;
    int ld;
    if (split) {
      plane = 2L * cph * npo; ld = npo;
      parts.off[0] = 0; parts.off[1] = (long)cph * npo; parts.off[2] = parts.off[3] = 0;
    } else {
      plane = 2L * cph * 2 * npo; ld = 2 * npo;
      parts.off[0] = 0; parts.off[1] = (long)cph * 2 * npo + npo; parts.off[2] = (long)cph * 2 * npo; parts.off[3] = npo;
    }
    const int vw = (long)cpi * (npo / 128) >= 2048 ? 4 : ((long)cpi * (npo / 64) >= 2048 ? 2 : 1);
    const int ochunks = npo / (32 * vw), items = cpi * ochunks;
    const dim3 grid(std::min(1024, st::ceil_div(items, 4)));
    st::trace("filters_idft_mfma<%d> taps=%d bins=%d parts=%d items=%d gflop=%.3f mb=%.2f", vw, width, bins, split ? 2 : 4, items,
              4096e-9 * items * (double)vw * st::ceil_div((split ? 2 : 4) * bins / 2, FI_CH) * FI_CH,
              1e-6 * 4 * ((double)(split ? 2 : 4) * bins * cin * npo + (double)width * cpi * npo));
    st::LaunchTimer timer(s);
#define ST_FI(VWV) st::launch_timed(timer, filters_idft_mfma_kernel<VWV>, grid, dim3(256), s, qf, width, cin, cout, cpi, npo, n, bins, tw, dpacked, \
                                    split ? 1 : 2, plane, parts, ld, ochunks, items)
    if (vw == 4) ST_FI(4); else if (vw == 2) ST_FI(2); else ST_FI(1);
#undef ST_FI
    return;
  }
  const dim3 grid(st::ceil_div(npo, 256), cpi);
  if (width == 32) hipLaunchKernelGGL(filters_idft_kernel<32>, grid, dim3(256), 0, s, qf, width, cin, cout, cpi, cph, npo, n, bins, tw, dpacked, split);
  else if (width == 25) hipLaunchKernelGGL(filters_idft_kernel<25>, grid, dim3(256), 0, s, qf, width, cin, cout, cpi, cph, npo, n, bins, tw, dpacked, split);
  else if (width == 7) hipLaunchKernelGGL(filters_idft_kernel<7>, grid, dim3(256), 0, s, qf, width, cin, cout, cpi, cph, npo, n, bins, tw, dpacked, split);
  else hipLaunchKernelGGL(filters_idft_kernel<0>, grid, dim3(256), 0, s, qf, width, cin, cout, cpi, cph, npo, n, bins, tw, dpacked, split);
}

}

extern "C" {

int st_gemm_nn_batched_f32(const float* a, int64_t lda, int64_t a_batch, const float* b, int64_t b_batch, float* c,
                           int64_t ldc, int64_t c_batch, int m, int k, int n, int batches, void* stream) {
  return st::gemm_nn_batched(a, lda, a_batch, b, b_batch, c, ldc, c_batch, m, k, n, batches, st::as_stream(stream));
}

size_t st_gemm_nn_batched_ws_bytes(void) { return (size_t)st::SK_WS_FLOATS * sizeof(float); }
size_t st_gemm_nn_batched_ctrl_bytes(void) { return (size_t)st::SK_CTRL_WORDS * sizeof(unsigned); }

int st_gemm_nn_batched_ws_f32(const float* a, int64_t lda, int64_t a_batch, const float* b, int64_t b_batch, float* c, int64_t ldc,
                              int64_t c_batch, int m, int k, int n, int batches, void* workspace, size_t workspace_bytes,
                              void* stream) {
  float* sk = (workspace && workspace_bytes >= st_gemm_nn_batched_ws_bytes()) ? reinterpret_cast<float*>(workspace) : nullptr;
  return st::gemm_nn_batched(a, lda, a_batch, b, b_batch, c, ldc, c_batch, m, k, n, batches, st::as_stream(stream), sk);
}

int st_gemm_nn_batched_bt_ws_f32(const float* a, int64_t lda, int64_t a_batch, const float* bt, int64_t bt_batch, float* c, int64_t ldc,
                                 int64_t c_batch, int m, int k, int n, int batches, void* workspace, size_t workspace_bytes,
                                 void* stream) {
  float* sk = (workspace && workspace_bytes >= st_gemm_nn_batched_ws_bytes()) ? reinterpret_cast<float*>(workspace) : nullptr;
  return st::gemm_nn_batched(a, lda, a_batch, bt, bt_batch, c, ldc, c_batch, m, k, n, batches, st::as_stream(stream), sk, true);
}

int st_gemm_tn_batched_f32(const float* a, int64_t lda, int64_t a_batch, const float* z, int64_t ldz, int64_t z_batch, float* out,
                           int64_t out_batch, int m, int k, int n, int batches, void* stream) {
  return st::gemm_tn_batched(a, lda, a_batch, z, ldz, z_batch, out, out_batch, m, k, n, batches, st::as_stream(stream));
}

int st_gemm_tn_batched_shared_f32(const float* a, int64_t lda, int64_t a_batch, const float* z, int64_t ldz, int64_t z_batch, float* out,
                                  int64_t out_batch, int m, int k, int n, int batches, int z_batch_shift, void* stream) {
  ST_REQUIRE(z_batch_shift >= 0 && z_batch_shift < 8, "gemm_tn_batched_shared: bad shift");
  return st::gemm_tn_batched(a, lda, a_batch, z, ldz, z_batch, out, out_batch, m, k, n, batches, st::as_stream(stream), z_batch_shift);
}

int st_gemm_tn_batched_tile_f32(const float* a, int64_t lda, int64_t a_batch, const float* z, int64_t ldz, int64_t z_batch, float* out,
                                int64_t out_batch, int m, int k, int n, int batches, int z_batch_shift, int tile_n, void* stream) {
  ST_REQUIRE(z_batch_shift >= 0 && z_batch_shift < 8, "gemm_tn_batched_tile: bad shift");
  ST_REQUIRE(tile_n == 64 || tile_n == 128, "gemm_tn_batched_tile: tile_n is 64 or 128");
  return st::gemm_tn_batched(a, lda, a_batch, z, ldz, z_batch, out, out_batch, m, k, n, batches, st::as_stream(stream), z_batch_shift, tile_n);
}

int st_gemm_nn_g3_batched_f32(const float* a, int64_t lda, int64_t a_batch, const int64_t* a_off, const float* b, int64_t ldb, int64_t b_batch,
                              const int64_t* b_off, int b_transposed, float* c, int64_t ldc, int64_t c_batch, int64_t c_off2, int m, int k, int n,
                              int batches, void* stream) {
  ST_REQUIRE(a_off && b_off, "gemm_nn_g3_batched: null offsets");
  const long ao[3] = {(long)a_off[0], (long)a_off[1], (long)a_off[2]}, bo[3] = {(long)b_off[0], (long)b_off[1], (long)b_off[2]};
  return st::gemm_nn_g3_batched(a, lda, a_batch, ao, b, ldb, b_batch, bo, c, ldc, c_batch, c_off2, m, k, n, batches, st::as_stream(stream),
                                b_transposed != 0);
}

int st_gemm_tn_g3_batched_f32(const float* a, int64_t lda, int64_t a_batch, const int64_t* a_off, const float* z, int64_t ldz, int64_t z_batch,
                              const int64_t* z_off, float* out, int64_t out_batch, int64_t out_part, int m, int k, int n, int batches,
                              void* stream) {
  ST_REQUIRE(a_off && z_off, "gemm_tn_g3_batched: null offsets");
  const long ao[3] = {(long)a_off[0], (long)a_off[1], (long)a_off[2]}, zo[3] = {(long)z_off[0], (long)z_off[1], (long)z_off[2]};
  return st::gemm_tn_g3_batched(a, lda, a_batch, ao, z, ldz, z_batch, zo, out, out_batch, out_part, m, k, n, batches, st::as_stream(stream));
}

int st_conv1d_fft_three_products(int width, int cin_pitch, int cout) {
  return g3_form(width, cin_pitch, cout) ? 2 : (zf3_form(width, cout) ? 1 : 0);
}

int st_conv1d_fft_plan(int width, int frames, int batch, int* n, int* valid, int* blocks, int* bins, int* rows_pad) {
  ST_REQUIRE(width_ok(width) && frames > 0 && batch > 0, "fft plan: filter width must be in [2, 32]");
  const Plan p = make_plan(width, frames, batch);
  if (n) *n = p.n;
  if (valid) *valid = V;
  if (blocks) *blocks = p.blocks;
  if (bins) *bins = p.bins;
  if (rows_pad) *rows_pad = p.rows_pad;
  return ST_OK;
}

size_t st_conv1d_fft_table_floats(void) { return T_END; }

int st_conv1d_fft_tables_f32(int width, int pad_left, float* tables, size_t table_floats, void* stream) {
  ST_REQUIRE(width_ok(width) && pad_left >= 0 && pad_left < width && tables && table_floats >= (size_t)T_END,
             "fft tables: bad argument");
  hipLaunchKernelGGL(tables_kernel, dim3(64), dim3(256), 0, st::as_stream(stream), V + width - 1, pad_left, tables);
  return st::check_launch("fft tables");
}

size_t st_conv1d_fft_filter_floats(int width, int cin_pitch, int cout) {
  if (!width_ok(width)) return 0;
  const size_t bins = (V + width - 1) / 2 + 1;
  return bins * 2 * half_of(cin_pitch) * 2 * st::npad_of(cout);
}

int st_conv1d_fft_filters_f32(const float* packed, int width, int cin, int cout, int cin_pitch, const float* tables, float* gfwd,
                              void* stream) {
  ST_REQUIRE(width_ok(width) && cin_pitch % 16 == 0 && tables && packed && gfwd, "fft filters: bad argument");
  ST_REQUIRE(st::npad_of(cout) % 128 == 0, "fft filters: the output channels must pack to a multiple of 128");
  hipStream_t s = st::as_stream(stream);
  const int n = V + width - 1, bins = n / 2 + 1;
  const f32x2* tw = reinterpret_cast<const f32x2*>(tables + T_FW);
  const int npo = st::npad_of(cout);
#define ST_FFT_WIDTH_DISPATCH(KERNEL, ...)                                                                   \
  do {                                                                                                       \
    if (width == 32) hipLaunchKernelGGL(KERNEL<32>, grid, dim3(256), 0, s, __VA_ARGS__);                     \
    else if (width == 25) hipLaunchKernelGGL(KERNEL<25>, grid, dim3(256), 0, s, __VA_ARGS__);                \
    else if (width == 7) hipLaunchKernelGGL(KERNEL<7>, grid, dim3(256), 0, s, __VA_ARGS__);                  \
    else hipLaunchKernelGGL(KERNEL<0>, grid, dim3(256), 0, s, __VA_ARGS__);                                  \
  } while (0)
  const int gx = st::ceil_div(npo, 256), gy = half_of(cin_pitch);
  const dim3 grid(gx, gy, gx * gy < 1024 ? 4 : 1);
  if (g3_form(width, cin_pitch, cout)) {
    if (width == 32) hipLaunchKernelGGL((filters_dft_fwd_kernel<32, 4>), grid, dim3(256), 0, s, packed, width, cin, cout, cin_pitch, half_of(cin_pitch), npo, n, bins, tw, gfwd, (unsigned short*)nullptr, (size_t)0);
    else hipLaunchKernelGGL((filters_dft_fwd_kernel<0, 4>), grid, dim3(256), 0, s, packed, width, cin, cout, cin_pitch, half_of(cin_pitch), npo, n, bins, tw, gfwd, (unsigned short*)nullptr, (size_t)0);
    return st::check_launch("fft filters (three planes)");
  }
  ST_FFT_WIDTH_DISPATCH(filters_dft_fwd_kernel, packed, width, cin, cout, cin_pitch, half_of(cin_pitch), npo, n, bins, tw, gfwd,
                        (unsigned short*)nullptr, (size_t)0);
  return st::check_launch("fft filters");
}

size_t st_conv1d_fft_sf_floats(const st_tensor3* x, const st_tensor3* y, int width) {
  if (!x || !y || !width_ok(width)) return 0;
  const Plan p = make_plan(width, y->frames, y->batch);
  return (size_t)p.bins * 2 * p.rows_pad * 2 * half_of(x->c_pitch);
}

size_t st_conv1d_fft_zf_floats(const st_tensor3* dz, int width) {
  if (!dz || !width_ok(width)) return 0;
  const Plan p = make_plan(width, dz->frames, dz->batch);
  const bool three = width >= G3_MIN_WIDTH && st::npad_of(dz->channels) >= 512;
  return (size_t)p.bins * p.rows_pad * (three ? 3 : 2) * st::npad_of(dz->channels);
}

size_t st_conv1d_fft_ws(const st_tensor3* x, const st_tensor3* y, int width) {
  if (!x || !y || !width_ok(width)) return 0;
  const Plan p = make_plan(width, y->frames, y->batch);
  const size_t nf = 2 * (size_t)st::npad_of(y->channels), ka = 2 * (size_t)half_of(x->c_pitch), nb = ka;
  const size_t yf = (size_t)p.bins * p.rows_pad * nf, xf = (size_t)p.bins * p.rows_pad * nb, qf = (size_t)p.bins * ka * nf;
  return (st::SK_WS_FLOATS + std::max(yf, std::max(xf, qf)) + 64) * sizeof(float);
}

int st_conv1d_nwc_fwd_fft_chain_f32(const st_tensor3* x, const float* gfwd, const float* bias, int width, int pad_left, int relu,
                                    const st_tensor3* y, const float* tables, float* sf, int sf_ready, const float* next_tables,
                                    float* next_sf, int next_width, int next_pad_left, int* next_sf_written, void* workspace,
                                    size_t workspace_bytes, void* stream) {
  ST_REQUIRE(st::tensor_ok(x) && st::tensor_ok(y) && gfwd && sf && workspace && tables && width_ok(width), "conv fft fwd: bad argument");
  ST_REQUIRE(x->batch == y->batch && x->frames == y->frames && pad_left >= 0 && pad_left < width, "conv fft fwd: stride-1 SAME layers only");
  ST_REQUIRE(st::npad_of(y->channels) % 128 == 0 && workspace_bytes >= st_conv1d_fft_ws(x, y, width), "conv fft fwd: workspace / shape");
  if (next_sf_written) *next_sf_written = 0;
  hipStream_t s = st::as_stream(stream);
  const Plan p = make_plan(width, y->frames, y->batch, ROWS_F32);
  const int ka = 2 * half_of(x->c_pitch), npo = st::npad_of(y->channels), nf = 2 * npo;
  float* const sk = reinterpret_cast<float*>(workspace);
  float* yf = sk + st::SK_WS_FLOATS;
  const int half = half_of(x->c_pitch);
  const long s_bin = 2L * p.rows_pad * ka;
  if (g3_form(width, x->c_pitch, y->channels)) {
    ST_REQUIRE(!sf_ready, "conv fft fwd: a layer in the three-product form transforms its own input");
    launch_dft(*x, nullptr, p, tables + T_FS, -pad_left, p.n, half, sf, nullptr, 0, 0, nullptr, s, 0, nullptr, 4);
    const long plane = (long)half * npo;
    const long a_off[3] = {0, half, 2L * half}, b_off[3] = {0, plane, 2 * plane};
    if (int e = st::gemm_nn_g3_batched(sf, 4L * half, s_bin, a_off, gfwd, npo, 3 * plane, b_off, yf, nf, (long)p.rows_pad * nf, npo,
                                       p.rows_pad, half, npo, p.bins, s))
      return e;
  } else {
  if (!sf_ready)
    launch_dft(*x, nullptr, p, tables + T_FS, -pad_left, p.n, half, sf, nullptr, 0, 0, nullptr, s, s_bin,
               split_lag_products(half) ? sf + (long)p.rows_pad * ka : nullptr);
  if (int e = st::gemm_nn_batched(sf, ka, s_bin, gfwd, (long)ka * nf, yf, nf, (long)p.rows_pad * nf, p.rows_pad, ka, nf, p.bins, s, sk))
    return e;
  }
  RowsOut out{y->base + (long)y->halo * y->c_pitch, (long)y->t_pitch * y->c_pitch, y->c_pitch, y->channels, y->frames, nullptr};
  const int nchunks = st::ceil_div(y->c_pitch, 32);
  if (next_tables && next_sf && can_fuse_next(p, *y, next_width, next_pad_left)) {
    const Plan pn = make_plan(next_width, y->frames, y->batch, ROWS_F32);
    const int half_n = half_of(y->c_pitch), ka_n = 2 * half_n;
    const long sn_bin = 2L * pn.rows_pad * ka_n;
    float* rot = split_lag_products(half_n) ? next_sf + (long)pn.rows_pad * ka_n : nullptr;
    st::trace("idft_dft_rows<%d> rows=%d chunks=%d bins=%d next_bins=%d gflop=%.3f mb=%.2f", p.bins <= 36 ? 18 : 24, p.rows, nchunks, p.bins, pn.bins,
              4096e-9 * p.rows * (double)nchunks * (2 * (p.bins <= 36 ? 18 : 24) * 2 + (32 + FUSE_HALO) * 3),
              1e-6 * 4 * ((double)p.bins * p.rows * 2 * npo + (double)p.rows * V * y->c_pitch + (double)pn.bins * p.rows * 2 * half_n * (rot ? 2 : 1)));
    const dim3 grid(y->batch * nchunks), block(64 * FUSE_BLOCKS);
    st::LaunchTimer timer(s);
    if (p.bins <= 36)
      st::launch_timed(timer, idft_dft_rows_kernel<18>, grid, block, s, yf, tables + T_IY, p.blocks, p.rows_pad, p.bins, npo, nchunks, out, bias, relu,
                       next_tables + T_FP, pn.n, next_pad_left, pn.bins, half_n, next_sf, sn_bin, rot);
    else
      st::launch_timed(timer, idft_dft_rows_kernel<24>, grid, block, s, yf, tables + T_IY, p.blocks, p.rows_pad, p.bins, npo, nchunks, out, bias, relu,
                       next_tables + T_FP, pn.n, next_pad_left, pn.bins, half_n, next_sf, sn_bin, rot);
    if (next_sf_written) *next_sf_written = 1;
    return st::check_launch("conv fft fwd (fused transforms)");
  }
  launch_idft<1>(yf, tables + T_IY, p, npo, nchunks, out, bias, relu, nullptr, 0L, 0, s);
  return st::check_launch("conv fft fwd");
}

int st_conv1d_nwc_fwd_fft_f32(const st_tensor3* x, const float* gfwd, const float* bias, int width, int pad_left, int relu,
                              const st_tensor3* y, const float* tables, float* sf, void* workspace,
                              size_t workspace_bytes, void* stream) {
  return st_conv1d_nwc_fwd_fft_chain_f32(x, gfwd, bias, width, pad_left, relu, y, tables, sf, 0, nullptr, nullptr, 0, 0, nullptr, workspace,
                                         workspace_bytes, stream);
}

int st_conv1d_fft_dz_spectra_f32(const st_tensor3* dz, int width, const float* tables, float* zf, void* stream) {
  ST_REQUIRE(st::tensor_ok(dz) && tables && zf && width_ok(width) && st::npad_of(dz->channels) % 128 == 0, "conv fft dz spectra: bad argument");
  const Plan p = make_plan(width, dz->frames, dz->batch, ROWS_F32);
  launch_dft(*dz, nullptr, p, tables + T_FZ, 0, V, st::npad_of(dz->channels), zf, nullptr, 0, 0, nullptr, st::as_stream(stream), 0, nullptr,
             zf3_form(width, dz->channels) ? 5 : 0);
  return st::check_launch("conv fft dz spectra");
}

int st_conv1d_fft_bias_grad_f32(const st_tensor3* dz, int width, const float* zf, float* dbias, void* stream) {
  ST_REQUIRE(st::tensor_ok(dz) && zf && dbias && width_ok(width) && st::npad_of(dz->channels) % 128 == 0, "conv fft bias grad: bad argument");
  const Plan p = make_plan(width, dz->frames, dz->batch, ROWS_F32);
  const int np = st::npad_of(dz->channels);
  const bool zf3 = zf3_form(width, dz->channels);
  hipLaunchKernelGGL(bias_from_spectra_kernel, dim3(st::ceil_div(np, 32)), dim3(256), 0, st::as_stream(stream), zf + (zf3 ? np : 0), p.rows,
                     (zf3 ? 3 : 2) * np, dz->channels, np, dbias);
  return st::check_launch("conv fft bias grad");
}

int st_conv1d_nwc_bwd_data_fft_chain_f32(const st_tensor3* dz, const float* zf, const float* gfwd, int width, int pad_left,
                                         const st_tensor3* act, const st_tensor3* dx, const float* tables, const float* below_tables,
                                         float* below_zf, int below_width, int* below_zf_written, void* workspace,
                                         size_t workspace_bytes, void* stream) {
  ST_REQUIRE(st::tensor_ok(dz) && st::tensor_ok(dx) && zf && gfwd && workspace && tables && width_ok(width), "conv fft bwd_data: bad argument");
  ST_REQUIRE(dz->batch == dx->batch && dz->frames == dx->frames && pad_left >= 0 && pad_left < width, "conv fft bwd_data: stride-1 layers only");
  ST_REQUIRE(st::npad_of(dz->channels) % 128 == 0 && workspace_bytes >= st_conv1d_fft_ws(dx, dz, width), "conv fft bwd_data: workspace / shape");
  if (act) ST_REQUIRE(st::tensor_ok(act) && act->batch == dx->batch && act->frames == dx->frames && act->c_pitch >= dx->c_pitch,
                      "conv fft bwd_data: mask tensor mismatch");
  if (below_zf_written) *below_zf_written = 0;
  hipStream_t s = st::as_stream(stream);
  const Plan p = make_plan(width, dz->frames, dz->batch, ROWS_F32);
  const int kz = 2 * st::npad_of(dz->channels), cph = half_of(dx->c_pitch), nb = 2 * cph;
  float* const sk = reinterpret_cast<float*>(workspace);
  float* xf = sk + st::SK_WS_FLOATS;
  const int npz = st::npad_of(dz->channels);
  const bool zf3 = zf3_form(width, dz->channels);
  if (g3_form(width, dx->c_pitch, dz->channels)) {
    const long plane = (long)cph * npz;
    const long a_off[3] = {0, 2L * npz, npz}, b_off[3] = {0, 2 * plane, plane};
    if (int e = st::gemm_nn_g3_batched(zf, 3L * npz, (long)p.rows_pad * 3 * npz, a_off, gfwd, npz, 3 * plane, b_off, xf, nb, (long)p.rows_pad * nb,
                                       cph, p.rows_pad, npz, cph, p.bins, s, true))
      return e;
  } else if (int e = st::gemm_nn_batched(zf + (zf3 ? npz : 0), zf3 ? 3L * npz : kz, (long)p.rows_pad * (zf3 ? 3 * npz : kz), gfwd, (long)nb * kz, xf, nb,
                                         (long)p.rows_pad * nb, p.rows_pad, kz, nb, p.bins, s, sk, true))
    return e;
  RowsOut out{dx->base + (long)dx->halo * dx->c_pitch, (long)dx->t_pitch * dx->c_pitch, dx->c_pitch, dx->channels, dx->frames, nullptr};
  const int nchunks = st::ceil_div(dx->c_pitch, 32);
  const float* mask = act ? act->base + (long)act->halo * act->c_pitch : nullptr;
  const long mask_bs = act ? (long)act->t_pitch * act->c_pitch : 0L;
  const int right = width - 1 - pad_left;
  const bool window_form = p.blocks <= FUSE_BLOCKS && p.rows == p.rows_pad && pad_left <= FUSE_HALO && right <= FUSE_HALO &&
                           st::tuning(st::TUNE_NO_FUSED_TRANSFORMS) == 0;
  if (window_form) {
    const bool below = below_tables && below_zf && width_ok(below_width) && st::npad_of(dx->channels) % 128 == 0 &&
                       st::npad_of(dx->channels) == cph && 32 * nchunks == cph && !zf3_form(below_width, dx->channels);
    const Plan pb = make_plan(below ? below_width : width, dx->frames, dx->batch, ROWS_F32);
    st::trace("idft_ola_dft_rows<%d%s> rows=%d chunks=%d bins=%d gflop=%.3f mb=%.2f", p.bins <= 36 ? 18 : 24, below ? ",dz-spectra" : "", p.rows, nchunks, p.bins,
              4096e-9 * p.rows * (double)nchunks * (2 * (p.bins <= 36 ? 18 : 24) * 3 + (below ? 32 * 3 : 0)),
              1e-6 * 4 * ((double)p.bins * p.rows * 2 * cph + (double)p.rows * V * dx->c_pitch * (mask ? 2 : 1) + (below ? (double)pb.bins * p.rows * 2 * cph : 0.0)));
    const dim3 grid(dx->batch * nchunks), block(64 * FUSE_BLOCKS);
    const float* wz = below ? below_tables + T_ZP : nullptr;
    st::LaunchTimer timer(s);
    if (p.bins <= 36)
      st::launch_timed(timer, idft_ola_dft_rows_kernel<18>, grid, block, s, xf, tables + T_IW, p.blocks, p.rows_pad, p.bins, cph, nchunks, out,
                       pad_left, right, mask, mask_bs, act ? act->c_pitch : 0, wz, pb.bins, cph, below ? below_zf : nullptr);
    else
      st::launch_timed(timer, idft_ola_dft_rows_kernel<24>, grid, block, s, xf, tables + T_IW, p.blocks, p.rows_pad, p.bins, cph, nchunks, out,
                       pad_left, right, mask, mask_bs, act ? act->c_pitch : 0, wz, pb.bins, cph, below ? below_zf : nullptr);
    if (below && below_zf_written) *below_zf_written = 1;
    return st::check_launch("conv fft bwd_data (window form)");
  }
  launch_idft<3>(xf, tables + T_IX, p, cph, nchunks, out, nullptr, 0, mask, mask_bs, act ? act->c_pitch : 0, s);
  return st::check_launch("conv fft bwd_data");
}

int st_conv1d_nwc_bwd_data_fft_f32(const st_tensor3* dz, const float* zf, const float* gfwd, int width, int pad_left,
                                   const st_tensor3* act, const st_tensor3* dx, const float* tables, void* workspace,
                                   size_t workspace_bytes, void* stream) {
  return st_conv1d_nwc_bwd_data_fft_chain_f32(dz, zf, gfwd, width, pad_left, act, dx, tables, nullptr, nullptr, 0, nullptr, workspace,
                                              workspace_bytes, stream);
}


size_t st_conv1d_fft_filter_plane_elems(int width, int cin_pitch, int cout) { return st_conv1d_fft_filter_floats(width, cin_pitch, cout); }

int st_conv1d_fft_filters_planes(const float* packed, int width, int cin, int cout, int cin_pitch, const float* tables, void* g_planes,
                                 void* gt_planes, int planes, void* stream) {
  ST_REQUIRE(width_ok(width) && cin_pitch % 16 == 0 && tables && packed && g_planes && gt_planes && planes_ok(planes), "fft filter planes: bad argument");
  ST_REQUIRE(st::npad_of(cout) % 128 == 0, "fft filter planes: the output channels must pack to a multiple of 128");
  hipStream_t s = st::as_stream(stream);
  const int n = V + width - 1, bins = n / 2 + 1, npo = st::npad_of(cout), cph = half_of(cin_pitch);
  const f32x2* tw = reinterpret_cast<const f32x2*>(tables + T_FW);
  const size_t plane = (size_t)bins * 2 * cph * 2 * npo;
  const int gx = st::ceil_div(npo, 256), gy = cph;
  const dim3 grid(gx, gy, gx * gy < 1024 ? 4 : 1);
  unsigned short* g = reinterpret_cast<unsigned short*>(g_planes);
  if (planes == 1) launch_filters_planes<1>(width, grid, s, packed, cin, cout, cin_pitch, cph, npo, n, bins, tw, g, plane);
  else launch_filters_planes<3>(width, grid, s, packed, cin, cout, cin_pitch, cph, npo, n, bins, tw, g, plane);
  if (int e = st::check_launch("fft filter planes")) return e;
  for (int pl = 0; pl < planes; ++pl)
    if (int e = st::transpose_bf16_bins(g + pl * plane, reinterpret_cast<unsigned short*>(gt_planes) + pl * plane, bins, 2 * cph, 2 * npo, s))
      return e;
  return ST_OK;
}

size_t st_conv1d_fft_planes_ws(const st_tensor3* x, const st_tensor3* y, int width, int planes) {
  if (!x || !y || !width_ok(width) || !planes_ok(planes)) return 0;
  const Plan p = make_plan(width, y->frames, y->batch);
  const size_t nf = 2 * (size_t)st::npad_of(y->channels), ka = 2 * (size_t)half_of(x->c_pitch);
  const size_t red = (size_t)p.bins * p.rows_pad;
  const size_t prod = std::max((size_t)p.bins * p.rows_pad * nf, (size_t)p.bins * ka * nf);
  return (st::SK_WS_FLOATS + prod + 64) * sizeof(float) + planes * (2 * ka + nf) * red * 2 + 512;
}

int st_conv1d_nwc_fwd_fft_planes(const st_tensor3* x, const void* x_bf16, const void* gt_planes, const float* bias, int width,
                                 int pad_left, int relu, const st_tensor3* y, void* y_bf16, const float* tables, void* sf_planes,
                                 int planes, void* workspace, size_t workspace_bytes, void* stream) {
  ST_REQUIRE(st::tensor_ok(x) && st::tensor_ok(y) && gt_planes && sf_planes && workspace && tables && width_ok(width) && planes_ok(planes),
             "conv fft planes fwd: bad argument");
  ST_REQUIRE((planes == 1) == (x_bf16 != nullptr) && (planes == 1) == (y_bf16 != nullptr),
             "conv fft planes fwd: one plane goes with bf16 tensors, three planes with fp32 tensors");
  ST_REQUIRE(x->batch == y->batch && x->frames == y->frames && pad_left >= 0 && pad_left < width, "conv fft planes fwd: stride-1 SAME layers only");
  ST_REQUIRE(st::npad_of(y->channels) % 128 == 0 && workspace_bytes >= st_conv1d_fft_planes_ws(x, y, width, planes), "conv fft planes fwd: workspace / shape");
  hipStream_t s = st::as_stream(stream);
  const Plan p = make_plan(width, y->frames, y->batch);
  const int ka = 2 * half_of(x->c_pitch), npo = st::npad_of(y->channels), nf = 2 * npo;
  const size_t s_plane = (size_t)p.bins * p.rows_pad * ka, g_plane = (size_t)p.bins * ka * nf;
  float* yf = reinterpret_cast<float*>(workspace) + st::SK_WS_FLOATS;
  launch_dft(*x, x_bf16, p, tables + T_FS, -pad_left, p.n, half_of(x->c_pitch), nullptr, sf_planes, planes, s_plane, nullptr, s);
  if (int e = st::gemm_bf16_bins(planes, sf_planes, s_plane, ka, (long)p.rows_pad * ka, gt_planes, g_plane, (long)p.bins * ka, ka, yf, nf,
                                 p.rows_pad, ka, nf, p.bins, s))
    return e;
  RowsOut out{y->base + (long)y->halo * y->c_pitch, (long)y->t_pitch * y->c_pitch, y->c_pitch, y->channels, y->frames,
              y_bf16 ? reinterpret_cast<unsigned short*>(y_bf16) + (long)y->halo * y->c_pitch : nullptr};
  launch_idft<1>(yf, tables + T_IY, p, npo, st::ceil_div(y->c_pitch, 32), out, bias, relu, nullptr, 0L, 0, s);
  return st::check_launch("conv fft planes fwd");
}

int st_conv1d_fft_dz_spectra_planes(const st_tensor3* dz, const void* dz_bf16, int width, const float* tables, void* zf_planes,
                                    int planes, float* dc, void* stream) {
  ST_REQUIRE(st::tensor_ok(dz) && tables && zf_planes && width_ok(width) && planes_ok(planes) && st::npad_of(dz->channels) % 128 == 0 &&
                 (planes == 1) == (dz_bf16 != nullptr), "conv fft planes dz spectra: bad argument");
  const Plan p = make_plan(width, dz->frames, dz->batch);
  const int npo = st::npad_of(dz->channels);
  launch_dft(*dz, dz_bf16, p, tables + T_FZ, 0, V, npo, nullptr, zf_planes, planes, (size_t)p.bins * p.rows_pad * 2 * npo, dc,
             st::as_stream(stream));
  return st::check_launch("conv fft planes dz spectra");
}

int st_conv1d_fft_bias_grad_dc_f32(const float* dc, int rows, int channels, int n_pad, float* dbias, void* stream) {
  ST_REQUIRE(dc && dbias && rows > 0 && channels > 0 && n_pad >= channels, "conv fft bias grad (dc): bad argument");
  hipLaunchKernelGGL(bias_from_spectra_kernel, dim3(st::ceil_div(n_pad, 32)), dim3(256), 0, st::as_stream(stream), dc, rows, n_pad, channels,
                     n_pad, dbias);
  return st::check_launch("conv fft bias grad (dc)");
}

int st_conv1d_nwc_bwd_data_fft_planes(const st_tensor3* dz, const void* zf_planes, const void* g_planes, int width, int pad_left,
                                      const st_tensor3* act, const void* act_bf16, const st_tensor3* dx, void* dx_bf16,
                                      const float* tables, int planes, void* workspace, size_t workspace_bytes, void* stream) {
  ST_REQUIRE(st::tensor_ok(dz) && st::tensor_ok(dx) && zf_planes && g_planes && workspace && tables && width_ok(width) && planes_ok(planes),
             "conv fft planes bwd_data: bad argument");
  ST_REQUIRE(dz->batch == dx->batch && dz->frames == dx->frames && pad_left >= 0 && pad_left < width, "conv fft planes bwd_data: stride-1 layers only");
  ST_REQUIRE((planes == 1) == (dx_bf16 != nullptr) && (!act || (planes == 1) == (act_bf16 != nullptr)),
             "conv fft planes bwd_data: one plane goes with bf16 tensors, three planes with fp32 tensors");
  ST_REQUIRE(st::npad_of(dz->channels) % 128 == 0 && workspace_bytes >= st_conv1d_fft_planes_ws(dx, dz, width, planes), "conv fft planes bwd_data: workspace / shape");
  if (act) ST_REQUIRE(st::tensor_ok(act) && act->batch == dx->batch && act->frames == dx->frames && act->c_pitch >= dx->c_pitch,
                      "conv fft planes bwd_data: mask tensor mismatch");
  hipStream_t s = st::as_stream(stream);
  const Plan p = make_plan(width, dz->frames, dz->batch);
  const int kz = 2 * st::npad_of(dz->channels), cph = half_of(dx->c_pitch), nb = 2 * cph;
  float* xf = reinterpret_cast<float*>(workspace) + st::SK_WS_FLOATS;
  if (int e = st::gemm_bf16_bins(planes, zf_planes, (size_t)p.bins * p.rows_pad * kz, kz, (long)p.rows_pad * kz, g_planes, (size_t)p.bins * nb * kz,
                                 kz, (long)nb * kz, xf, nb, p.rows_pad, kz, nb, p.bins, s))
    return e;
  RowsOut out{dx->base + (long)dx->halo * dx->c_pitch, (long)dx->t_pitch * dx->c_pitch, dx->c_pitch, dx->channels, dx->frames,
              dx_bf16 ? reinterpret_cast<unsigned short*>(dx_bf16) + (long)dx->halo * dx->c_pitch : nullptr};
  const void* mask = nullptr;
  if (act) mask = act_bf16 ? static_cast<const void*>(reinterpret_cast<const unsigned short*>(act_bf16) + (long)act->halo * act->c_pitch)
                           : static_cast<const void*>(act->base + (long)act->halo * act->c_pitch);
  launch_idft<3>(xf, tables + T_IX, p, cph, st::ceil_div(dx->c_pitch, 32), out, nullptr, 0, mask, act ? (long)act->t_pitch * act->c_pitch : 0L,
                 act ? act->c_pitch : 0, s);
  return st::check_launch("conv fft planes bwd_data");
}

int st_conv1d_nwc_bwd_filter_fft_planes(const st_tensor3* x, const st_tensor3* dz, const void* sf_planes, const void* zf_planes, int width,
                                        const float* tables, float* dpacked, int planes, void* workspace, size_t workspace_bytes,
                                        void* stream) {
  ST_REQUIRE(st::tensor_ok(x) && st::tensor_ok(dz) && sf_planes && zf_planes && dpacked && workspace && tables && width_ok(width) && planes_ok(planes),
             "conv fft planes bwd_filter: bad argument");
  ST_REQUIRE(x->batch == dz->batch && x->frames == dz->frames, "conv fft planes bwd_filter: stride-1 layers only");
  ST_REQUIRE(st::npad_of(dz->channels) % 128 == 0 && workspace_bytes >= st_conv1d_fft_planes_ws(x, dz, width, planes), "conv fft planes bwd_filter: workspace / shape");
  hipStream_t s = st::as_stream(stream);
  const Plan p = make_plan(width, dz->frames, dz->batch);
  const f32x2* tw = reinterpret_cast<const f32x2*>(tables + T_FW);
  const int half = half_of(x->c_pitch), ka = 2 * half, npo = st::npad_of(dz->channels), nf = 2 * npo;
  const long red = (long)p.bins * p.rows_pad;
  const size_t prod = std::max((size_t)p.bins * p.rows_pad * nf, (size_t)p.bins * ka * nf);
  float* qf = reinterpret_cast<float*>(workspace) + st::SK_WS_FLOATS;
  unsigned short* st_planes = reinterpret_cast<unsigned short*>(qf + prod + 64);
  unsigned short* zt_planes = st_planes + (size_t)planes * 2 * ka * red;
  const unsigned short* sfp = reinterpret_cast<const unsigned short*>(sf_planes);
  const unsigned short* zfp = reinterpret_cast<const unsigned short*>(zf_planes);
  if (split_lag_products(half) && planes == 1 && npo % 128 == 0 && (2 * p.rows_pad) % 32 == 0 && st::tuning(st::TUNE_BF16_LAG_COPIES) == 0) {
    if (int e = st::lag_products_tr_bf16(sfp, zfp, p.bins, p.rows_pad, half, npo, qf, s)) return e;
    launch_filters_idft(qf, width, x->channels, dz->channels, x->c_pitch, half, npo, p.n, p.bins, tw, dpacked, 1, s);
    return st::check_launch("conv fft planes bwd_filter");
  }
  if (split_lag_products(half)) {
    for (int pl = 0; pl < planes; ++pl) {
      if (int e = st::transpose_bf16_bins_split(sfp + (size_t)pl * red * ka, st_planes + (size_t)pl * 2 * ka * red, p.bins, p.rows_pad, ka, 2, s)) return e;
      if (int e = st::transpose_bf16_bins_split(zfp + (size_t)pl * red * nf, zt_planes + (size_t)pl * nf * red, p.bins, p.rows_pad, nf, 1, s)) return e;
    }
    if (int e = st::gemm_bf16_bins(planes, st_planes, (size_t)2 * ka * red, 4 * red, 2L * p.rows_pad, zt_planes, (size_t)nf * red, 2 * red,
                                   2L * p.rows_pad, qf, npo, half, 2 * p.rows_pad, npo, 2 * p.bins, s, 1))
      return e;
    launch_filters_idft(qf, width, x->channels, dz->channels, x->c_pitch, half, npo, p.n, p.bins, tw, dpacked, 1, s);
    return st::check_launch("conv fft planes bwd_filter");
  }
  for (int pl = 0; pl < planes; ++pl) {
    if (int e = st::transpose_bf16_bins(sfp + (size_t)pl * red * ka, st_planes + (size_t)pl * ka * red, p.bins, p.rows_pad, ka, s)) return e;
    if (int e = st::transpose_bf16_bins(zfp + (size_t)pl * red * nf, zt_planes + (size_t)pl * nf * red, p.bins, p.rows_pad, nf, s)) return e;
  }
  if (int e = st::gemm_bf16_bins(planes, st_planes, (size_t)ka * red, red, p.rows_pad, zt_planes, (size_t)nf * red, red, p.rows_pad, qf, nf, ka,
                                 p.rows_pad, nf, p.bins, s))
    return e;
  launch_filters_idft(qf, width, x->channels, dz->channels, x->c_pitch, half, npo, p.n, p.bins, tw, dpacked, 0, s);
  return st::check_launch("conv fft planes bwd_filter");
}

int st_conv1d_nwc_bwd_filter_fft_f32(const st_tensor3* x, const st_tensor3* dz, const float* sf, const float* zf, int width,
                                     const float* tables, float* dpacked, void* workspace, size_t workspace_bytes, void* stream) {
  ST_REQUIRE(st::tensor_ok(x) && st::tensor_ok(dz) && sf && zf && dpacked && workspace && tables && width_ok(width), "conv fft bwd_filter: bad argument");
  ST_REQUIRE(x->batch == dz->batch && x->frames == dz->frames, "conv fft bwd_filter: stride-1 layers only");
  ST_REQUIRE(st::npad_of(dz->channels) % 128 == 0 && workspace_bytes >= st_conv1d_fft_ws(x, dz, width), "conv fft bwd_filter: workspace / shape");
  hipStream_t s = st::as_stream(stream);
  const Plan p = make_plan(width, dz->frames, dz->batch, ROWS_F32);
  const f32x2* tw = reinterpret_cast<const f32x2*>(tables + T_FW);
  const int half = half_of(x->c_pitch), ka = 2 * half, npo = st::npad_of(dz->channels), nf = 2 * npo;
  float* qf = reinterpret_cast<float*>(workspace) + st::SK_WS_FLOATS;
  const long s_bin = 2L * p.rows_pad * ka;
  const bool zf3 = zf3_form(width, dz->channels);
  if (g3_form(width, x->c_pitch, dz->channels)) {
    const long a_off[3] = {2L * half, 3L * half, 0}, z_off[3] = {0, 2L * npo, npo};
    if (int e = st::gemm_tn_g3_batched(sf, 4L * half, s_bin, a_off, zf, 3L * npo, (long)p.rows_pad * 3 * npo, z_off, qf, 2L * half * npo,
                                       (long)half * npo, p.rows_pad, half, npo, p.bins, s))
      return e;
    launch_filters_idft(qf, width, x->channels, dz->channels, x->c_pitch, half, npo, p.n, p.bins, tw, dpacked, 1, s);
  } else if (split_lag_products(half)) {
    if (int e = st::gemm_tn_batched(sf, half, (long)p.rows_pad * ka, zf, npo, (long)p.rows_pad * nf, qf, (long)half * npo, 2 * p.rows_pad,
                                    half, npo, 2 * p.bins, s, 1))
      return e;
    launch_filters_idft(qf, width, x->channels, dz->channels, x->c_pitch, half, npo, p.n, p.bins, tw, dpacked, 1, s);
  } else {
    if (int e = st::gemm_tn_batched(sf, ka, s_bin, zf + (zf3 ? npo : 0), zf3 ? 3L * npo : nf, (long)p.rows_pad * (zf3 ? 3 * npo : nf), qf, (long)ka * nf,
                                    p.rows_pad, ka, nf, p.bins, s))
      return e;
    launch_filters_idft(qf, width, x->channels, dz->channels, x->c_pitch, half, npo, p.n, p.bins, tw, dpacked, 0, s);
  }
  return st::check_launch("conv fft bwd_filter");
}

}
```

speecht_amd/csrc/conv_gemm.hip:

```cpp
#include <algorithm>
#include <atomic>
#include <cmath>
#include <cstdlib>

#include <type_traits>

#include "st_common.h"
#include "streamk_map.h"

namespace {

typedef float f32x16 __attribute__((ext_vector_type(16)));
typedef float f32x4 __attribute__((ext_vector_type(4)));

constexpr int BK = 32;
constexpr int APITCH = BK + 4;
constexpr int NTHREADS = 256;

struct RowMap {
  int frames;
  int row_stride;
  long batch_stride;
  long row0;
  __device__ __forceinline__ long off(int m) const {
    int b = m / frames;
    int t = m - b * frames;
    return (long)b * batch_stride + row0 + (long)t * row_stride;
  }
};

struct NNParams {
  const float* A;  RowMap amap;
  const float* Bm; int Np;
  float* C;        RowMap cmap;
  const float* mask; RowMap mmap;
  const float* bias;
  int M, Kvalid, Kp, n_store, relu;
  int taps, cp;
  int tiles_m, tiles_n, chunk;
  int gm, tm_per, tn_per;
  int splits, steps_per_split;
  float* slab;
  float* colsum;
  int colsum_rows;
  int batches;
  long a_batch, b_batch, c_batch;
  long bt_ld; int bt_rows;
};


__device__ __forceinline__ void dma16_sv(unsigned lds_byte_addr, const void* sbase, unsigned voff_bytes) {
  unsigned keep;
  asm volatile("s_mov_b32 %0, m0\n\ts_mov_b32 m0, %1\n\ts_nop 0\n\tglobal_load_lds_dwordx4 %2, %3\n\ts_mov_b32 m0, %0"
               : "=&s"(keep) : "s"(lds_byte_addr), "v"(voff_bytes), "s"(sbase) : "memory");
}
__device__ __forceinline__ float* at_bytes(float* ubase, unsigned voff_bytes) {
  return reinterpret_cast<float*>(reinterpret_cast<char*>(ubase) + voff_bytes);
}
__device__ __forceinline__ const float* at_bytes(const float* ubase, unsigned voff_bytes) {
  return reinterpret_cast<const float*>(reinterpret_cast<const char*>(ubase) + voff_bytes);
}
__device__ __forceinline__ void dma_wait_all() { asm volatile("s_waitcnt vmcnt(0)" ::: "memory"); }
__device__ __forceinline__ unsigned lds_addr(const float* p) {
  return (unsigned)(size_t)(__attribute__((address_space(3))) const float*)p;
}

template <int N> struct FVec;
template <> struct FVec<1> { typedef float type; };
template <> struct FVec<2> { typedef float type __attribute__((ext_vector_type(2))); };
template <> struct FVec<4> { typedef float type __attribute__((ext_vector_type(4))); };
template <int N> __device__ __forceinline__ float vget(const typename FVec<N>::type& v, int i) { return v[i]; }
template <> __device__ __forceinline__ float vget<1>(const float& v, int) { return v; }
template <int N> __device__ __forceinline__ void vset(typename FVec<N>::type& v, int i, float x) { v[i] = x; }
template <> __device__ __forceinline__ void vset<1>(float& v, int, float x) { v = x; }

__device__ __forceinline__ int swz_slot4(int lane, int row) { return ((lane & 7) ^ ((row >> 1) & 7)) * 4; }
__device__ __forceinline__ int swz_frag(int row, int q, int h) { return row * BK + (((2 * q + h) ^ ((row >> 1) & 7)) * 4); }

template <int BM, int BN, int WMW, int WNW, bool BT>
struct NNStage {
  static constexpr int WTM = BM / WMW, WTN = BN / WNW;
  static constexpr int MT = WTM / 32, NT = WTN / 32;
  static constexpr int A_DMA = BM / 32;
  static constexpr int B_DMA = BN / 32;
  static constexpr int N_DMA = A_DMA + B_DMA;
  static constexpr int A_SZ = BM * BK, B_SZ = BK * BN;
  typedef typename FVec<NT>::type bvec;

  template <int CUR, bool MORE, typename Dma, typename... Next>
  static __device__ __forceinline__ void run(const float* As, const float* Bs, const int (&a_frag)[4], const int (&bt_frag)[4],
                                             int b_frag, f32x16 (&acc)[MT][NT], int nq, Dma& dma_piece, Next... next) {
    const float* as = As + CUR * A_SZ;
    const float* bs = Bs + CUR * B_SZ + (BT ? 0 : b_frag);
    f32x4 af[4][MT];
    bvec bf[4][4];
    f32x4 bft[4][NT];
    auto read_frags = [&](int q) {
#pragma unroll
      for (int i = 0; i < MT; ++i) af[q][i] = *reinterpret_cast<const f32x4*>(as + a_frag[q] + i * 32 * BK);
      if (BT) {
#pragma unroll
        for (int n = 0; n < NT; ++n) bft[q][n] = *reinterpret_cast<const f32x4*>(bs + bt_frag[q] + n * 32 * BK);
      } else {
#pragma unroll
        for (int j = 0; j < 4; ++j) bf[q][j] = *reinterpret_cast<const bvec*>(bs + (8 * q + j) * BN);
      }
    };
    read_frags(0);
#pragma unroll
    for (int q = 0; q < 4; ++q) {
      if (MORE) {
#pragma unroll
        for (int pc = q; pc < N_DMA; pc += 4) dma_piece(pc, next..., CUR ^ 1);
      }
      if (q < 3) read_frags(q + 1);
      if (q < nq) {
#pragma unroll
        for (int j = 0; j < 4; ++j)
#pragma unroll
          for (int i = 0; i < MT; ++i)
#pragma unroll
            for (int n = 0; n < NT; ++n)
              acc[i][n] = __builtin_amdgcn_mfma_f32_32x32x2f32(af[q][i][j], BT ? bft[q][n][j] : vget<NT>(bf[q][j], n), acc[i][n], 0, 0, 0);
      }
#pragma unroll
      for (int k = 0; k < 4; ++k) {
        __builtin_amdgcn_sched_group_barrier(0x008, 1, 0);
        __builtin_amdgcn_sched_group_barrier(0x100, 1, 0);
      }
#pragma unroll
      for (int k = 0; k < 2; ++k) {
        __builtin_amdgcn_sched_group_barrier(0x008, 2, 0);
        __builtin_amdgcn_sched_group_barrier(0x006, 8, 0);
        __builtin_amdgcn_sched_group_barrier(0x010, 1, 0);
      }
      __builtin_amdgcn_sched_group_barrier(0x008, 8, 0);
      __builtin_amdgcn_sched_barrier(0);
    }
    __syncthreads();
  }
};

__device__ __forceinline__ bool bin_tile(int tiles_m, int tiles_n, int batches, int& bin, int& tile_m, int& tile_n) {
  const int xcd = blockIdx.x & 7, local = blockIdx.x >> 3;
  const int per_bin = tiles_m * tiles_n;
  const int set = local / per_bin, t = local - set * per_bin;
  bin = set * 8 + xcd;
  tile_n = t / tiles_m;
  tile_m = t - tile_n * tiles_m;
  return bin < batches;
}

template <typename Stage> __device__ __forceinline__ void nn_stage_pairs(int nk, Stage& stage) {
  using std::integral_constant;
  using std::true_type;
  using std::false_type;
  int kt = 0;
  for (; kt + 2 < nk; kt += 2) {
    stage(integral_constant<int, 0>{}, true_type{});
// ... 1095 lines not shown
  }
  if (Np % 128) return 1;
  const long tiles128 = (long)st::ceil_div(M, 128) * (Np / 128);
  if (tiles128 >= 128) return 1;
  return (int)std::max<long>(1, std::min<long>(256 / tiles128, nk / 4));
}

template <int BM, int BN, int WMW, int WNW, bool FAST = false, bool BT = false>
void launch_nn(NNParams& p, int epi, hipStream_t s) {
  p.tiles_m = st::ceil_div(p.M, BM);
  p.tiles_n = p.Np / BN;
  {
    const double a_bytes = (double)p.M * p.cp * 4.0, b_bytes = (double)p.Kp * p.Np * 4.0;
    double best = 0.0;
    p.gm = 1;
    for (int gm = 1; gm <= 8; gm *= 2) {
      const int gn = 8 / gm;
      if (gm > p.tiles_m || gn > p.tiles_n) continue;
      const int slots = st::ceil_div(p.tiles_m, gm) * st::ceil_div(p.tiles_n, gn) * 8;
      const double cost = (a_bytes * gn + b_bytes * gm) * ((double)slots / (p.tiles_m * p.tiles_n));
      if (best == 0.0 || cost < best) { best = cost; p.gm = gm; }
    }
    if (8 / p.gm > p.tiles_n) p.gm = 8;
    p.tm_per = st::ceil_div(p.tiles_m, p.gm);
    p.tn_per = st::ceil_div(p.tiles_n, 8 / p.gm);
    p.chunk = p.tm_per * p.tn_per;
  }
  p.colsum_rows = p.tiles_m * WMW;
  if (p.batches > 0) p.chunk = st::ceil_div(p.batches, 8) * p.tiles_m * p.tiles_n;
  dim3 grid(p.chunk * 8, p.splits > 1 ? p.splits : 1), block(NTHREADS);
  const double gflop = 2e-9 * p.tiles_m * BM * (double)p.Np * p.Kp * std::max(1, p.batches);
  if (p.batches > 0)
    st::trace("gemm_nn<%d,%d,%d,%d,%s> batched bins=%d M=%d Np=%d Kp=%d gflop=%.3f", BM, BN, WMW, WNW, FAST ? (BT ? "fast-bt" : "fast") : "clamped",
              p.batches, p.M, p.Np, p.Kp, gflop);
  else
    st::trace("gemm_nn<%d,%d,%d,%d,%s> epi=%d splits=%d M=%d Np=%d Kp=%d taps=%d xcd=%dx%d gflop=%.3f", BM, BN, WMW, WNW,
              FAST ? (BT ? "fast-bt" : "fast") : "clamped", epi, p.splits > 1 ? p.splits : 1, p.M, p.Np, p.Kp, p.taps, p.gm, 8 / p.gm, gflop);
  {
    st::LaunchTimer timer(s);
    if (epi == 0) st::launch_timed(timer, gemm_nn_kernel<BM, BN, WMW, WNW, 0, FAST, BT>, grid, block, s, p);
    else st::launch_timed(timer, gemm_nn_kernel<BM, BN, WMW, WNW, 1, FAST, BT>, grid, block, s, p);
  }
  if (p.splits > 1) {
    const long quads = (long)p.M * (p.n_store / 4);
    hipLaunchKernelGGL(splitk_epilogue_kernel, dim3((unsigned)std::min<long>((quads + 255) / 256, 4096)), dim3(256), 0, s,
                       p, epi);
  }
}

int run_nn(NNParams& p, int epi, hipStream_t s) {
  if (p.bt_ld > 0) {
    if (!(p.Np % 128 == 0 && p.taps == 1 && p.cp % 32 == 0 && p.Kvalid % 32 == 0 && p.Kvalid == p.Kp && p.bt_ld % 4 == 0 && p.bt_rows > 0)) {
      st::set_error("gemm_nn: the transposed-operand form needs n_pad %% 128 == 0, one tap and a reduction length that is a multiple of 32");
      return ST_EINVAL;
    }
    const long tiles128 = (long)st::ceil_div(p.M, 128) * (p.Np / 128) * std::max(1, p.batches);
    if ((p.batches > 0 && (tiles128 < 512 || p.M <= 64)) || (p.batches <= 0 && tiles128 < 192 && p.splits <= 1)) launch_nn<64, 128, 2, 2, true, true>(p, epi, s);
    else launch_nn<128, 128, 2, 2, true, true>(p, epi, s);
    return st::check_launch("gemm_nn (bt)");
  }
  if (p.Np % 128 == 0) {
    long tiles128 = (long)st::ceil_div(p.M, 128) * (p.Np / 128) * std::max(1, p.batches);
    if (p.batches > 0 && (tiles128 < 512 || p.M <= 64)) {
      if (p.cp % 32 == 0 && p.Kvalid % 32 == 0) launch_nn<64, 128, 2, 2, true>(p, epi, s);
      else launch_nn<64, 128, 2, 2>(p, epi, s);
    }
    else if ((tiles128 >= 192 || p.splits > 1) && p.cp % 32 == 0 && p.Kvalid % 32 == 0)
      launch_nn<128, 128, 2, 2, true>(p, epi, s);
    else if (tiles128 >= 192 || p.splits > 1) launch_nn<128, 128, 2, 2>(p, epi, s);
    else launch_nn<64, 128, 2, 2>(p, epi, s);
  } else if (p.Np == 64) {
    launch_nn<128, 64, 2, 2>(p, epi, s);
  } else if (p.Np == 32) {
    launch_nn<128, 32, 4, 1>(p, epi, s);
  } else {
    st::set_error("unsupported packed width n_pad=%d", p.Np);
    return ST_EINVAL;
  }
  return st::check_launch("gemm_nn");
}

}

int st::gemm_nn_batched(const float* A, long lda, long a_batch, const float* B, long b_batch, float* C, long ldc,
                        long c_batch, int M, int K, int N, int batches, hipStream_t s, float* sk_ws, bool b_transposed) {
  if (!(A && B && C && M > 0 && K > 0 && K % 32 == 0 && N % 128 == 0 && batches > 0 && lda % 4 == 0 && ldc % 4 == 0)) {
    st::set_error("gemm_nn_batched: bad shape M=%d K=%d N=%d", M, K, N);
    return ST_EINVAL;
  }
  const int knob = st::tuning(st::TUNE_STREAMK);
  if (sk_ws && knob != 2 && M % 64 == 0 && a_batch % 4 == 0 && b_batch % 4 == 0 && (long)64 * lda < (1L << 30) && (long)32 * N < (1L << 30) &&
      (long)64 * ldc < (1L << 29) && (!b_transposed || (long)128 * K < (1L << 29))) {
    const long tiles = (long)batches * (M / 64) * (N / 128);
    const double per_cu = (double)tiles / 256.0;
    const bool uneven = tiles > 256 && tiles <= 768 && std::ceil(per_cu) / per_cu > 1.2;
    int slots = st::tuning(st::TUNE_STREAMK_SLOTS);
    if (slots != 64 && slots != 96) slots = 64;
    st::SkPlan plan;
    if ((knob == 1 || uneven) && tiles < (1L << 24) && st::sk_make_plan((int)tiles, K / BK, slots, plan)) {
      static std::atomic<unsigned> g_epoch{0};
      unsigned epoch = g_epoch.fetch_add(1, std::memory_order_relaxed) + 1;
      if (epoch == 0) epoch = g_epoch.fetch_add(1, std::memory_order_relaxed) + 1;
      BinsParams q{};
      q.A = A; q.B = B; q.C = C;
      q.lda = lda; q.ldb = b_transposed ? K : N; q.ldc = ldc;
      q.a_batch = a_batch; q.b_batch = b_batch; q.c_batch = c_batch;
      q.tiles_m = M / 64; q.tiles_n = N / 128;
      q.plan = plan;
      q.ctrl = reinterpret_cast<unsigned*>(sk_ws);
      q.partial = sk_ws + st::SK_CTRL_WORDS;
      q.epoch = epoch;
      q.pub_epoch = st::tuning(st::TUNE_STREAMK_TEST_DROP) ? (epoch ^ 0x80000000u) : epoch;
      st::trace("gemm_nn_bins<64,128,2,2%s> batched bins=%d M=%d Np=%d Kp=%d streamk wgs=%d upw=%d gflop=%.3f", b_transposed ? ",bt" : "",
                batches, M, N, K, 8 * plan.wgs_per_xcd, plan.upw, 2e-9 * M * (double)N * K * batches);
      {
        st::LaunchTimer timer(s);
        const dim3 grid(8 * plan.wgs_per_xcd), block(NTHREADS);
        if (b_transposed) st::launch_timed(timer, gemm_nn_bins_kernel<64, 128, 2, 2, true>, grid, block, s, q);
        else st::launch_timed(timer, gemm_nn_bins_kernel<64, 128, 2, 2, false>, grid, block, s, q);
      }
      return st::check_launch("gemm_nn_bins");
    }
  }
  if (M % 128 == 64 && M > 128 && (long)K * N >= (1L << 21) && (long)st::ceil_div(M, 128) * (N / 128) * batches >= 512) {
    if (int e = st::gemm_nn_batched(A, lda, a_batch, B, b_batch, C, ldc, c_batch, M - 64, K, N, batches, s, nullptr, b_transposed)) return e;
    return st::gemm_nn_batched(A + (long)(M - 64) * lda, lda, a_batch, B, b_batch, C + (long)(M - 64) * ldc, ldc, c_batch, 64, K, N, batches, s,
                               nullptr, b_transposed);
  }
  NNParams p{};
  p.A = A;
  p.amap.frames = M; p.amap.row_stride = (int)lda; p.amap.batch_stride = 0; p.amap.row0 = 0;
  p.Bm = B;
  p.Np = N;
  p.C = C;
  p.cmap.frames = M; p.cmap.row_stride = (int)ldc; p.cmap.batch_stride = 0; p.cmap.row0 = 0;
  p.M = M;
  p.Kvalid = K;
  p.Kp = K;
  p.n_store = N;
  p.taps = 1;
  p.cp = K;
  p.batches = batches;
  p.a_batch = a_batch; p.b_batch = b_batch; p.c_batch = c_batch;
  if (b_transposed) { p.bt_ld = K; p.bt_rows = N; }
  return run_nn(p, 0, s);
}

int st::gemm_tn_batched(const float* A, long lda, long a_batch, const float* Z, long ldz, long z_batch, float* out,
                        long o_batch, int M, int K, int N, int batches, hipStream_t s, int z_batch_shift, int tile_n) {
  if (!(A && Z && out && M > 0 && M % 32 == 0 && K % 128 == 0 && N % 128 == 0 && batches > 0 && (tile_n == 0 || tile_n == 64 || tile_n == 128))) {
    st::set_error("gemm_tn_batched: bad shape M=%d K=%d N=%d tile_n=%d", M, K, N, tile_n);
    return ST_EINVAL;
  }
  if (tile_n == 0) {
    const long tiles128 = (long)batches * (K / 128) * (N / 128);
    tile_n = (tiles128 > 256 && tiles128 <= 320 && M <= 512) ? 64 : 128;
  }
  TNParams p{};
  p.A = A;
  p.amap.frames = M; p.amap.row_stride = (int)lda; p.amap.batch_stride = 0; p.amap.row0 = 0;
  p.Z = Z;
  p.zmap.frames = M; p.zmap.row_stride = (int)ldz; p.zmap.batch_stride = 0; p.zmap.row0 = 0;
  p.M = M;
  p.Kvalid = K;
  p.Kp = K;
  p.Np = N;
  p.z_cols = N;
  p.rows_per_split = M;
  p.out = out;
  p.tiles_k = K / 128;
  p.tiles_n = N / tile_n;
  p.amap_batches = 1;
  p.adv_b = 32 / M;
  p.adv_t = 32 % M;
  p.a_batch = a_batch; p.z_batch = z_batch; p.o_batch = o_batch;
  p.z_shift = z_batch_shift;
  st::trace("gemm_tn<%d> batched bins=%d M=%d Kp=%d Np=%d gflop=%.3f", tile_n, batches, M, K, N, 2e-9 * M * (double)K * N * batches);
  {
    st::LaunchTimer timer(s);
    const dim3 grid(p.tiles_k * p.tiles_n, 1, batches);
    if (tile_n == 64) st::launch_timed(timer, gemm_tn_kernel<64, 2, 2>, grid, dim3(TN_THREADS), s, p);
    else st::launch_timed(timer, gemm_tn_kernel<128, 2, 2>, grid, dim3(TN_THREADS), s, p);
  }
  return st::check_launch("gemm_tn_batched");
}

int st::gemm_nn_g3_batched(const float* A, long lda, long a_batch, const long a_off[3], const float* B, long ldb, long b_batch,
                           const long b_off[3], float* C, long ldc, long c_batch, long c_off2, int M, int K, int N, int batches,
                           hipStream_t s, bool b_transposed) {
  if (!(A && B && C && M > 0 && K > 0 && K % 64 == 0 && N % 128 == 0 && batches > 0 && lda % 4 == 0 && ldb % 4 == 0 && ldc % 4 == 0 &&
        c_off2 % 4 == 0 && a_off[0] % 4 == 0 && a_off[1] % 4 == 0 && a_off[2] % 4 == 0 && b_off[0] % 4 == 0 && b_off[1] % 4 == 0 && b_off[2] % 4 == 0)) {
    st::set_error("gemm_nn_g3_batched: bad shape M=%d K=%d N=%d", M, K, N);
    return ST_EINVAL;
  }
  if (M % 128 == 64 && M > 128 && (long)batches * st::ceil_div(M, 128) * (N / 128) >= 512 &&
      st::tuning(st::TUNE_G3_TILE) == 0) {
    if (int e = st::gemm_nn_g3_batched(A, lda, a_batch, a_off, B, ldb, b_batch, b_off, C, ldc, c_batch, c_off2, M - 64, K, N, batches, s, b_transposed)) return e;
    return st::gemm_nn_g3_batched(A + (long)(M - 64) * lda, lda, a_batch, a_off, B, ldb, b_batch, b_off, C + (long)(M - 64) * ldc, ldc, c_batch, c_off2,
                                  64, K, N, batches, s, b_transposed);
  }
  G3Params p{};
  p.A = A; p.lda = lda; p.a_batch = a_batch;
  p.B = B; p.ldb = ldb; p.b_batch = b_batch;
  for (int i = 0; i < 3; ++i) { p.a_off[i] = a_off[i]; p.b_off[i] = b_off[i]; }
  p.C = C; p.ldc = ldc; p.c_batch = c_batch; p.c_off2 = c_off2;
  p.M = M; p.N = N; p.batches = batches;
  const long wgs128 = (long)batches * st::ceil_div(M, 128) * (N / 128), wgs64 = (long)batches * st::ceil_div(M, 64) * (N / 128);
  const int tile = st::tuning(st::TUNE_G3_TILE);
  const bool half_rows = tile == 2 ? false : (tile == 1 || tile == 4 || M <= 64 || wgs128 < 512);
  p.ksplit = (half_rows && K % 128 == 0 && (tile == 4 || (tile == 0 && wgs64 < 512))) ? 2 : 1;
  p.K = K / p.ksplit;
  p.tiles_m = st::ceil_div(M, half_rows ? 64 : 128);
  p.tiles_n = N / 128;
  if (p.ksplit > 1)
    hipLaunchKernelGGL(g3_zero_out_kernel, dim3(st::ceil_div(M, 4), batches), dim3(256), 0, s, C, ldc, c_batch, c_off2, M, N);
  const dim3 grid(st::ceil_div(batches, 8) * p.tiles_m * p.tiles_n * 8, p.ksplit), block(NTHREADS);
  st::trace("gemm_nn_g3<%d%s> batched bins=%d M=%d Np=%d Kp=%d ksplit=%d gflop=%.3f", half_rows ? 64 : 128, b_transposed ? ",bt" : "", batches, M, N, K,
            p.ksplit, 2e-9 * p.tiles_m * (half_rows ? 64 : 128) * (double)N * 3 * K * batches);
  st::LaunchTimer timer(s);
  if (half_rows) {
    if (b_transposed) st::launch_timed(timer, gemm_nn_g3_kernel<64, true>, grid, block, s, p);
    else st::launch_timed(timer, gemm_nn_g3_kernel<64, false>, grid, block, s, p);
  } else {
    if (b_transposed) st::launch_timed(timer, gemm_nn_g3_kernel<128, true>, grid, block, s, p);
    else st::launch_timed(timer, gemm_nn_g3_kernel<128, false>, grid, block, s, p);
  }
  return st::check_launch("gemm_nn_g3");
}

int st::gemm_tn_g3_batched(const float* A, long lda, long a_batch, const long a_off[3], const float* Z, long ldz, long z_batch,
                           const long z_off[3], float* out, long o_batch, long o_part, int M, int K, int N, int batches, hipStream_t s) {
  if (!(A && Z && out && M > 0 && M % 32 == 0 && K % 128 == 0 && N % 128 == 0 && batches > 0 && lda % 4 == 0 && ldz % 4 == 0 &&
        (long)32 * lda < (1L << 29) && (long)32 * ldz < (1L << 29))) {
    st::set_error("gemm_tn_g3_batched: bad shape M=%d K=%d N=%d", M, K, N);
    return ST_EINVAL;
  }
  TN3Params p{};
  p.A = A; p.lda = lda; p.a_batch = a_batch;
  p.Z = Z; p.ldz = ldz; p.z_batch = z_batch;
  for (int i = 0; i < 3; ++i) { p.a_off[i] = a_off[i]; p.z_off[i] = z_off[i]; }
  p.out = out; p.o_batch = o_batch; p.o_part = o_part;
  p.M = M; p.K = K; p.N = N; p.tiles_k = K / 128; p.tiles_n = N / 128; p.batches = batches;
  st::trace("gemm_tn_g3<128> batched bins=%d M=%d Kp=%d Np=%d gflop=%.3f", batches, M, K, N, 2e-9 * 3 * M * (double)K * N * batches);
  st::LaunchTimer timer(s);
  st::launch_timed(timer, gemm_tn_g3_kernel, dim3(st::ceil_div(batches, 8) * p.tiles_k * p.tiles_n * 8), dim3(TN_THREADS), s, p);
  return st::check_launch("gemm_tn_g3_batched");
}

static int bwd_data_impl(const st_tensor3* dz, const float* packed_t, bool forward_filters, int width, int pad_left,
                         const st_tensor3* act, const st_tensor3* dx, float* dbias_dx, void* workspace,
                         size_t workspace_bytes, void* stream);

extern "C" {

int st_streamk_lost_ptr(void** device_word) {
  ST_REQUIRE(device_word, "st_streamk_lost_ptr: null argument");
  void* p = nullptr;
  if (hipGetSymbolAddress(&p, HIP_SYMBOL(g_sk_lost)) != hipSuccess || !p) {
    st::set_error("st_streamk_lost_ptr: hipGetSymbolAddress failed");
    return ST_ELAUNCH;
  }
  *device_word = p;
  return ST_OK;
}

int st_streamk_lost_fetch_async(unsigned* host_word, void* stream) {
  ST_REQUIRE(host_word, "st_streamk_lost_fetch_async: null argument");
  if (hipMemcpyFromSymbolAsync(host_word, HIP_SYMBOL(g_sk_lost), sizeof(unsigned), 0, hipMemcpyDeviceToHost, st::as_stream(stream)) !=
      hipSuccess) {
    st::set_error("st_streamk_lost_fetch_async: hipMemcpyFromSymbolAsync failed");
    return ST_ELAUNCH;
  }
  return ST_OK;
}

int st_streamk_lost_count(unsigned* count) {
  ST_REQUIRE(count, "st_streamk_lost_count: null argument");
  if (hipMemcpyFromSymbol(count, HIP_SYMBOL(g_sk_lost), sizeof(unsigned), 0, hipMemcpyDeviceToHost) != hipSuccess) {
    st::set_error("st_streamk_lost_count: hipMemcpyFromSymbol failed");
    return ST_ELAUNCH;
  }
  return ST_OK;
}

int st_packed_dims(int width, int cin_pitch, int cout, int* k_valid, int* k_pad, int* n_pad) {
  ST_REQUIRE(width > 0 && cin_pitch > 0 && cin_pitch % 16 == 0 && cout > 0, "st_packed_dims: bad shape");
  int kv = width * cin_pitch;
  if (k_valid) *k_valid = kv;
  if (k_pad) *k_pad = (int)st::round_up(kv, BK);
  if (n_pad) *n_pad = st::npad_of(cout);
  return ST_OK;
}

int st_fill_f32(float* dst, float value, size_t n, void* stream) {
  if (n == 0) return ST_OK;
  ST_REQUIRE(dst, "st_fill_f32: null");
  int blocks = (int)std::min<size_t>((n + 255) / 256, 4096);
  hipLaunchKernelGGL(fill_kernel, dim3(blocks), dim3(256), 0, st::as_stream(stream), dst, value, n);
  return st::check_launch("fill");
}

int st_zero_regions(const void* regions_device, int n_regions, void* stream) {
  ST_REQUIRE(regions_device && n_regions >= 0 && ((uintptr_t)regions_device & 15) == 0, "st_zero_regions: bad table");
  if (n_regions == 0) return ST_OK;
  hipLaunchKernelGGL(zero_regions_kernel, dim3(n_regions), dim3(256), 0, st::as_stream(stream),
                     reinterpret_cast<const ZeroRegion*>(regions_device));
  return st::check_launch("zero_regions");
}

int st_zero_halos_f32(const st_tensor3* t, void* stream) {
// ... 306 lines not shown
```

speecht_amd/csrc/st_common.h:

```cpp
#pragma once
#include <hip/hip_runtime.h>
#include <hip/hip_ext.h>
#include <stdarg.h>
#include <stdio.h>

#include "speecht_hip.h"

namespace st {

void set_error(const char* fmt, ...);

bool trace_on();
void trace(const char* fmt, ...);
class LaunchTimer {
 public:
  explicit LaunchTimer(hipStream_t s);
  bool active() const { return start_ != nullptr; }
  hipEvent_t start() const { return start_; }
  hipEvent_t stop() const { return stop_; }

 private:
  hipEvent_t start_, stop_;
};
template <typename... KArgs, typename... Args>
inline void launch_timed(const LaunchTimer& t, void (*kernel)(KArgs...), const dim3& grid, const dim3& block, hipStream_t s,
                         Args&&... args) {
  static_assert(sizeof...(KArgs) == sizeof...(Args), "launch_timed: argument count does not match the kernel");
  if (t.active()) hipExtLaunchKernelGGL(kernel, grid, block, 0, s, t.start(), t.stop(), 0, static_cast<KArgs>(args)...);
  else hipLaunchKernelGGL(kernel, grid, block, 0, s, static_cast<KArgs>(args)...);
}
enum { TUNE_STREAMK, TUNE_STREAMK_SLOTS, TUNE_STREAMK_TEST_DROP, TUNE_NO_FUSED_TRANSFORMS, TUNE_BF16_LAG_COPIES, TUNE_FILTERS_IDFT_VALU,
       TUNE_BF16_TAPS_PANEL, TUNE_NO_G3, TUNE_G3_TILE, TUNE_COUNT };
int tuning(int key);

constexpr int SK_FLAGS = 0, SK_TIMEOUTS = 768, SK_CTRL_WORDS = 1024;
constexpr long SK_WS_FLOATS = SK_CTRL_WORDS + 768L * 64 * 128;
int gemm_nn_batched(const float* A, long lda, long a_batch, const float* B, long b_batch, float* C, long ldc, long c_batch,
                    int M, int K, int N, int batches, hipStream_t s, float* sk_ws = nullptr, bool b_transposed = false);
int gemm_tn_batched(const float* A, long lda, long a_batch, const float* Z, long ldz, long z_batch, float* out, long o_batch,
                    int M, int K, int N, int batches, hipStream_t s, int z_batch_shift = 0, int tile_n = 0);
int gemm_nn_g3_batched(const float* A, long lda, long a_batch, const long a_off[3], const float* B, long ldb, long b_batch,
                       const long b_off[3], float* C, long ldc, long c_batch, long c_off2, int M, int K, int N, int batches,
                       hipStream_t s, bool b_transposed = false);
int gemm_tn_g3_batched(const float* A, long lda, long a_batch, const long a_off[3], const float* Z, long ldz, long z_batch,
                       const long z_off[3], float* out, long o_batch, long o_part, int M, int K, int N, int batches, hipStream_t s);

int gemm_bf16_bins(int planes, const void* a_planes, size_t a_plane, long a_rows_apart, long a_bin, const void* bt_planes,
                   size_t b_plane, long ldb, long b_bin, float* c, long ldc, int rows, int k, int n, int bins, hipStream_t s,
                   int b_bin_shift = 0);
int lag_products_tr_bf16(const void* s_plane, const void* z_plane, int bins, int rows, int half, int npo, float* q, hipStream_t s);
bool conv_taps_bf16_eligible(const st_tensor3& a, const st_tensor3& y, int width, int lead, const st_tensor3* act);
int conv_taps_bf16(const st_tensor3& a, const void* a_plane, const void* filters, const float* bias, int width, int lead, int relu,
                   const st_tensor3* act, const void* act_plane, const st_tensor3& y, void* y_plane, hipStream_t s);
int transpose_bf16_bins(const void* src, void* dst, int bins, int rows, int cols, hipStream_t s);
int transpose_bf16_bins_split(const void* src, void* dst, int bins, int rows, int cols, int forms, hipStream_t s);

inline hipStream_t as_stream(void* s) { return reinterpret_cast<hipStream_t>(s); }

inline int check_launch(const char* what) {
  hipError_t e = hipGetLastError();
  if (e != hipSuccess) {
    set_error("%s: %s", what, hipGetErrorString(e));
    return ST_ELAUNCH;
  }
  return ST_OK;
}

#define ST_REQUIRE(cond, ...)      \
  do {                             \
    if (!(cond)) {                 \
      st::set_error(__VA_ARGS__);  \
      return ST_EINVAL;            \
    }                              \
  } while (0)

inline int ceil_div(int a, int b) { return (a + b - 1) / b; }
inline size_t round_up(size_t a, size_t b) { return (a + b - 1) / b * b; }

inline int npad_of(int cout) { return cout <= 32 ? 32 : (cout <= 64 ? 64 : (int)round_up(cout, 128)); }

inline bool tensor_ok(const st_tensor3* t) {
  return t && t->base && t->batch > 0 && t->frames > 0 && t->channels > 0 && t->halo >= 0 && t->c_pitch % 16 == 0 &&
         t->c_pitch >= t->channels && t->t_pitch >= t->halo + t->frames;
}

inline long row_offset(const st_tensor3& x, int b, int t) {
  return ((long)b * x.t_pitch + x.halo + t) * (long)x.c_pitch;
}

typedef __attribute__((address_space(1))) const void* gptr_t;
typedef __attribute__((address_space(3))) void* lptr_t;

__device__ __forceinline__ float wave_sum(float v) {
#pragma unroll
  for (int o = 32; o > 0; o >>= 1) v += __shfl_xor(v, o, 64);
  return v;
}
__device__ __forceinline__ float wave_max(float v) {
#pragma unroll
  for (int o = 32; o > 0; o >>= 1) v = fmaxf(v, __shfl_xor(v, o, 64));
  return v;
}

}
```

speecht_amd/modes/fp32.py:

```python
import ctypes
import os
from types import SimpleNamespace

import torch

from .. import _lib
from .._lib import call
from .base import ModeBase
from .spectral import SpectralLayers


class Fp32Mode(SpectralLayers, ModeBase):
  _one_tap_in_place = True
  _flip_every_layer = False
  masks_padding = True

  def __init__(self, engine):
    super().__init__(engine)
    self._packed_t_fresh, self._packed_t_layers, self._bwd_ready = False, frozenset(), {}
    self._gfwd_fresh, self._gfwd_ready, self._fft_table_key, self._fft_prev = False, {}, {}, None

  def weights_changed(self):
    self._packed_t_fresh = False
    self._gfwd_fresh = False
# ... 14 lines not shown
      part.wgrad_ws_top, _ = e._storage.view('wgrad_ws_top', ws_top // 4 + 64)
    part.fft_layers = {i for i in range(len(e.layers)) if self._use_fft(i, sh.batch, sh.geo)}
    self._alloc_planes(sh, part)
    self._alloc_fft(sh, part)
    return part

  _top_gradient_beside = True

  def reenter(self, sh):
    self._fft_transition(sh.mode.fft, sh.mode.table_keys)

  def _workspace_bytes(self, lib, sh):
    layers, X, dZ = self.e.layers, sh.X, sh.dZ
    ws = max(lib.st_conv1d_bwd_filter_ws(X[i].ref, dZ[i].ref, l.width) for i, l in enumerate(layers))
    ws = max([ws] + [lib.st_conv1d_bwd_data_bias_ws(dZ[i].ref, dZ[i - 1].ref, l.width) for i, l in enumerate(layers) if i > 0])
    return max([ws] + [lib.st_conv1d_fwd_ws(X[i].ref, X[i + 1].ref, l.width) for i, l in enumerate(layers)])

  def _x6_fwd(self, part, i):
    return False
  _x6_bwd = _x6_wgrad = _x6_fwd

  def _alloc_planes(self, sh, part):
    pass

  def _forward_prologue(self):
    pass
  _backward_prologue = _forward_prologue

  def refresh_under_ctc(self):
    if not self._packed_t_ok() and self._flip_layers():
      self.e._on_side_stream(self._refresh_backward_operands)

  def prepare_forward_graph(self):
    e = self.e
    e._join_side_stream()
    if e.shape.mode.fft and e.fft_conv and not self._gfwd_fresh:
      self._refresh_fft_filters()
    self._wait_gfwd()

  def _transposed_in_place(self, i):
    l = self.e.layers[i]
    return (self._one_tap_in_place and i > 0 and l.width == 1 and l.stride == 1 and l.cout_pitch % 32 == 0 and
            l.n_pad >= l.cout_pitch and l.nt_pad % 128 == 0)

  def _flip_layers(self):
    e = self.e
    fft = e.shape.mode.fft if e.fft_conv else ()
    return [i for i in range(1, len(e.layers)) if self._flip_every_layer or not (i in fft or self._transposed_in_place(i))]

  def _refresh_backward_operands(self):
    e, ptr, s, stream, flip = self.e, self.e._ptr, self.e.stream_ptr, self.e.stream, self._flip_layers()
    self._bwd_ready = {}
    for i in reversed(flip):
      l = e.layers[i]
      call('st_filters_flip_transpose_f32', ptr(e._slice(e.params, i)[0]), l.width, l.cin, l.cout, l.cin_pitch, l.cout_pitch,
           ptr(e.packed_t[i]), s)
      ev = torch.cuda.Event()
      ev.record(stream)
      self._bwd_ready[i] = ev
    self._packed_t_fresh = True
    self._packed_t_layers = frozenset(flip)

  def _packed_t_ok(self):
    return self._packed_t_fresh and frozenset(self._flip_layers()) <= self._packed_t_layers

  def _wait_bwd_operands(self, i=None):
    ready = self._bwd_ready
    if not ready:
      return
    keys = [k for k in ready if i is None or k >= i]
    if keys:
      self.e.stream.wait_event(ready[min(keys)])
      for k in keys:
        del ready[k]

  def forward(self, mask_padding=False):
    if mask_padding and not self.masks_padding:
      raise _lib.SpeechtHipError('forward(mask_padding=True) is not supported by this mode')
    e, ptr, sh, s = self.e, self.e._ptr, self.e.shape, self.e.stream_ptr
    valid, top = (e._mask_lengths(), len(e.layers) - 1) if mask_padding else (None, 0)
    X, geo, part = sh.X, sh.geo, sh.mode
    fft = part.fft if e.fft_conv else {}
    ws = part.wgrad_ws
    ws_bytes = ws.numel() * 4 if e.split_small_batches else 0
    self._forward_prologue()
    sf_ready = False
    for i, l in enumerate(e.layers):
      pf, pb = e._slice(e.params, i)
      if i not in fft:
        sf_ready = False
      if self._x6_fwd(part, i):
        self._x6_forward_layer(i, pb)
      elif i in fft:
        f = fft[i]
        if not self._gfwd_fresh:
          e._join_side_stream()
          self._refresh_fft_filters()
        self._wait_gfwd(i)
        nxt = None if mask_padding else fft.get(i + 1)
        if nxt is not None and nxt['shift'] is not None:
          nxt = None
        written = ctypes.c_int(0)
        call('st_conv1d_nwc_fwd_fft_chain_f32', f['xref'], ptr(f['gfwd']), ptr(pb), f['width'], f['pl'], int(l.relu), X[i + 1].ref,
             ptr(f['tables']), ptr(f['sf']), int(sf_ready), ptr(nxt['tables']) if nxt else None, ptr(nxt['sf']) if nxt else None,
             nxt['width'] if nxt else 0, nxt['pl'] if nxt else 0, ctypes.byref(written), ptr(f['ws']), f['ws'].numel() * 4, s)
        sf_ready = written.value == 1
      else:
        call('st_conv1d_nwc_fwd_ws_f32', X[i].ref, ptr(pf), ptr(pb), l.width, l.stride, geo[i][2], int(l.relu), X[i + 1].ref,
             ptr(ws), ws_bytes, s)
      if mask_padding and i < top:
        call('st_mask_rows', X[i + 1].ref, valid(i), 4, s)

  def backward(self, on_layer_done, wanted):
    e, ptr, sh, s, layers = self.e, self.e._ptr, self.e.shape, self.e.stream_ptr, self.e.layers
    X, dZ, geo, part = sh.X, sh.dZ, sh.geo, sh.mode
    fft = part.fft if e.fft_conv else {}
    wgrad_ws, wgrad_ws_bytes = part.wgrad_ws, part.wgrad_ws.numel() * 4
    if not self._packed_t_ok():
      self._refresh_backward_operands()
    if fft and not self._gfwd_fresh:
      e._join_side_stream()
      self._refresh_fft_filters()
    self._wait_gfwd()
    self._backward_prologue()
    wait_all_below = len(layers) - 3
    side_wgrad, deferred = False, None
    top_pending = None
    hook = on_layer_done
    if hook is not None:
      def on_layer_done(j):
        nonlocal top_pending
        if top_pending is not None and top_pending != j:
          e._join_side_stream(second_only=True)
          hook(top_pending)
          top_pending = None
        if top_pending != j:
          hook(j)
    bias_from_above = False
    zf_ready = False
    for i in reversed(range(len(layers))):
      l = layers[i]
      gf, gb = e._slice(e.grads, i)
      need_bias, bias_from_above = not bias_from_above, False
      if self._x6_wgrad(part, i):
        self._x6_filter_gradient(i, gf, gb, need_bias)
      elif i in fft:
        f = fft[i]
        if not zf_ready:
          call('st_conv1d_fft_dz_spectra_f32', dZ[i].ref, f['width'], ptr(f['tables']), ptr(f['zf']), s)
        zf_ready = False
        polyphase = f['shift'] is not None

        def filter_gradient(f=f, l=l, i=i, gf=gf, gb=gb, need_bias=need_bias, polyphase=polyphase, ws=f.get('ws2', f['ws'])):
          call('st_conv1d_nwc_bwd_filter_fft_f32', f['xref'], dZ[i].ref, ptr(f['sf']), ptr(f['zf']), f['width'], ptr(f['tables']),
               ptr(f['dpacked2'] if polyphase else gf), ptr(ws), ws.numel() * 4, e.stream_ptr)
          if polyphase:
            cp = X[i].c_pitch
            n, o = l.width * cp * l.n_pad, f['shift'] * cp * l.n_pad
            with torch.cuda.stream(e.stream):
              gf[:n].copy_(f['dpacked2'][o:o + n], non_blocking=True)
          if need_bias:
            call('st_conv1d_fft_bias_grad_f32', dZ[i].ref, f['width'], ptr(f['zf']), ptr(gb), e.stream_ptr)
        if 'ws2' in f:
          e._on_side_stream(filter_gradient, second=(i % 2 == 1))
          side_wgrad, deferred = True, i
        else:
          filter_gradient()
      elif i + 1 == len(layers) and part.side_wgrad_top:
        def top_gradient(i=i, l=l, gf=gf, gb=gb, need_bias=need_bias, ws=part.wgrad_ws_top):
          call('st_conv1d_nwc_bwd_filter_f32', X[i].ref, dZ[i].ref, l.width, l.stride, geo[i][2], ptr(gf),
               ptr(gb) if need_bias else None, ptr(ws), ws.numel() * 4, e.stream_ptr)
        e._on_side_stream(top_gradient, second=True)
        top_pending = i
      else:
        call('st_conv1d_nwc_bwd_filter_f32', X[i].ref, dZ[i].ref, l.width, l.stride, geo[i][2], ptr(gf),
             ptr(gb) if need_bias else None, ptr(wgrad_ws), wgrad_ws_bytes, s)
      if on_layer_done is not None and deferred != i and wanted(i):
        if side_wgrad:
          e._join_side_stream()
          side_wgrad = False
        on_layer_done(i)
      if i > 0 and self._x6_bwd(part, i):
        self._x6_back_prop(i)
      elif i > 0 and i in fft:
        f = fft[i]
        act = X[i].ref if layers[i - 1].relu else None
        below = part.fft.get(i - 1)
        written = ctypes.c_int(0)
        call('st_conv1d_nwc_bwd_data_fft_chain_f32', dZ[i].ref, ptr(f['zf']), ptr(f['gfwd']), l.width, geo[i][2], act,
             dZ[i - 1].ref, ptr(f['tables']), ptr(below['tables']) if below else None, ptr(below['zf']) if below else None,
             below['width'] if below else 0, ctypes.byref(written), ptr(f['ws']), f['ws'].numel() * 4, s)
        zf_ready = written.value == 1
      elif i > 0:
        act = X[i].ref if layers[i - 1].relu else None
        if self._transposed_in_place(i):
          call('st_conv1d_1tap_bwd_data_bias_f32', dZ[i].ref, ptr(e._slice(e.params, i)[0]), act, dZ[i - 1].ref,
               ptr(e._slice(e.grads, i - 1)[1]), ptr(wgrad_ws), wgrad_ws_bytes, s)
        else:
          self._wait_bwd_operands(i if i > wait_all_below else None)
          call('st_conv1d_nwc_bwd_data_bias_f32', dZ[i].ref, ptr(e.packed_t[i]), l.width, geo[i][2], act, dZ[i - 1].ref,
               ptr(e._slice(e.grads, i - 1)[1]), ptr(wgrad_ws), wgrad_ws_bytes, s)
        bias_from_above = True
      if deferred == i and on_layer_done is not None and wanted(i):
        e._join_side_stream()
        side_wgrad = False
        on_layer_done(i)
      if deferred == i:
        deferred = None
    if side_wgrad or top_pending is not None:
      e._join_side_stream()
    if top_pending is not None and hook is not None:
      hook(top_pending)
```

speecht_amd/modes/spectral.py:

```python
import ctypes

import torch

from .. import _lib
from .._lib import Tensor3, call


class SpectralLayers:

  def _polyphase(self, i, geo):
    l = self.e.layers[i]
    if l.stride != 2:
      return None
    pl = geo[i][2]
    pl2 = (pl + 1) // 2
    shift = 2 * pl2 - pl
    return (l.width + shift + 1) // 2, pl2, shift

  def _use_fft(self, i, batch, geo):
    e = self.e
    l = e.layers[i]
    wide = l.stride == 1 and l.width >= 16
    if not (e.fft_conv and e.conv_mode in ('fp32', 'bf16x6') and l.n_pad % 128 == 0 and
            batch * geo[i][1] >= (e.fft_min_rows if wide else e.fft_min_rows_narrow)):
      return False
    if l.stride == 2:
      width2 = self._polyphase(i, geo)[0]
      return i == 0 and e.fft_first_layer and e.fft_min_width <= width2 <= 32
    return i > 0 and l.stride == 1 and e.fft_min_width <= l.width <= 32 and l.nt_pad % 128 == 0

  def _alloc_fft(self, sh, part):
    lib = _lib.load()
    e, ptr, X, dZ, batch = self.e, self.e._ptr, sh.X, sh.dZ, sh.batch
    part.fft = {}
    for i, l in enumerate(e.layers):
      t_in, t_out, pl, pr = sh.geo[i]
      if i not in part.fft_layers:
        continue
      view = lambda name, numel: e._storage.view('fft%d_%s' % (i, name), numel)
      f = dict(x=X[i].desc, width=l.width, pl=pl, cin=l.cin, cin_pitch=l.cin_pitch, shift=None)
      if l.stride == 2:
        width2, pl2, shift = self._polyphase(i, sh.geo)
        x = X[i]
        assert x.halo % 2 == 0 and x.t_pitch % 2 == 0
        cp2 = 2 * x.c_pitch
        f.update(x=Tensor3(x.buf.data_ptr(), batch, t_out, cp2, x.halo // 2, x.t_pitch // 2, cp2), width=width2, pl=pl2,
                 cin=cp2, cin_pitch=cp2, shift=shift)
        rows = 2 * width2 * x.c_pitch * l.n_pad
        f['packed2'], fresh_p = view('packed2', rows)
        f['dpacked2'] = view('dpacked2', rows)[0]
        if fresh_p:
          f['packed2'].zero_()
          self._gfwd_fresh = False
      f['xref'] = ctypes.byref(f['x'])
      tables, fresh_tables = view('tables', lib.st_conv1d_fft_table_floats())
      if self._fft_table_key.get(i) != (f['width'], f['pl']):
        fresh_tables = True
      self._fft_table_key[i] = (f['width'], f['pl'])
      gfwd, fresh_f = view('gfwd', lib.st_conv1d_fft_filter_floats(f['width'], f['cin_pitch'], l.cout))
      f.update(tables=tables, gfwd=gfwd, sf=view('sf', lib.st_conv1d_fft_sf_floats(f['xref'], X[i + 1].ref, f['width']))[0],
               zf=view('zf', lib.st_conv1d_fft_zf_floats(dZ[i].ref, f['width']))[0],
               ws=view('ws', lib.st_conv1d_fft_ws(f['xref'], X[i + 1].ref, f['width']) // 4 + 64)[0])
      if e.side_filter_gradient and i > 0 and l.cout <= 512:
        f['ws2'] = view('ws2', lib.st_conv1d_fft_ws(f['xref'], X[i + 1].ref, f['width']) // 4 + 64)[0]
      if fresh_tables:
        call('st_conv1d_fft_tables_f32', f['width'], f['pl'], ptr(tables), tables.numel(), e.stream_ptr)
      if fresh_f:
        self._gfwd_fresh = False
      part.fft[i] = f
    part.table_keys = {i: (f['width'], f['pl']) for i, f in part.fft.items()}
    self._fft_transition(part.fft, None)

  def _fft_transition(self, fft, table_keys):
    for i, key in (table_keys or {}).items():
      if self._fft_table_key.get(i) != key:
        f = fft[i]
        call('st_conv1d_fft_tables_f32', f['width'], f['pl'], self.e._ptr(f['tables']), f['tables'].numel(), self.e.stream_ptr)
        self._fft_table_key[i] = key
    if set(fft) != self._fft_prev:
      self._gfwd_fresh = False
      self._packed_t_fresh = False
    self._fft_prev = set(fft)

  def _refresh_fft_filters(self, layers=None):
    e, ptr = self.e, self.e._ptr
    sh, stream = e.shape, e.stream
    if layers is None:
      self._gfwd_ready = {}
    for i, f in sh.mode.fft.items():
      if layers is not None and i not in layers:
        continue
      l = e.layers[i]
      pf = e._slice(e.params, i)[0]
      if f['shift'] is not None:
        cp = sh.X[i].c_pitch
        n = l.width * cp * l.n_pad
        with torch.cuda.stream(stream):
          f['packed2'][f['shift'] * cp * l.n_pad:f['shift'] * cp * l.n_pad + n].copy_(pf[:n], non_blocking=True)
        pf = f['packed2']
      call('st_conv1d_fft_filters_f32', ptr(pf), f['width'], f['cin'], l.cout, f['cin_pitch'], ptr(f['tables']), ptr(f['gfwd']),
           e.stream_ptr)
      if stream is e._side:
        ev = torch.cuda.Event()
        ev.record(stream)
        self._gfwd_ready[i] = ev
    self._gfwd_fresh = True

  def refresh_after_update(self):
    sh = self.e.shape
    if sh is not None and sh.mode.fft:
      fft = sh.mode.fft
      first = min(fft)
      self._gfwd_ready = {}
      self._refresh_fft_filters(layers=[first])
      rest = [i for i in fft if i != first]
      if rest:
        self.e._on_side_stream(lambda: self._refresh_fft_filters(layers=rest))

  def _wait_gfwd(self, i=None):
    ready = self._gfwd_ready
    if not ready:
      return
    order = sorted(self.e.shape.mode.fft)
    if i is not None and i in order and order.index(i) >= 3:
      i = None
    keys = [k for k in ready if i is None or k <= i]
    if keys:
      self.e.stream.wait_event(ready[max(keys)])
      for k in keys:
        del ready[k]
```

Before: 4884.

## Fold polyphase tap shift and bias reduction into FFT filter kernels

Moves the polyphase tap shift into the filter DFT and IDFT kernels, so the shifted packed2/dpacked2 staging buffers and their copies are dropped. The bias-gradient reduction from the spectra now runs as extra blocks inside the filter IDFT MFMA launch, removing a separate small launch. The gemm_tn tile-size choice also moves to a helper that accounts for how full the last wave is. A new tuning knob restores the old separate-launch behaviour, and the extra blocks can add imbalance to the IDFT grid.

```diff
diff --git a/include/speecht_hip.h b/include/speecht_hip.h
--- a/include/speecht_hip.h
+++ b/include/speecht_hip.h
@@ -32,6 +32,8 @@
 int st_trace_timed_filter(const char* text);
 size_t st_trace_end(char* host_buf, size_t capacity);
 int st_set_tuning(const char* name, int value);
+int st_get_tuning(const char* name);
+
 uint32_t st_host_crc32c(const void* host_data, size_t n, uint32_t crc);
 
 int st_packed_dims(int width, int cin_pitch, int cout, int* k_valid, int* k_pad, int* n_pad);
@@ -82,6 +84,8 @@
 size_t st_conv1d_fft_filter_floats(int width, int cin_pitch, int cout);
 int st_conv1d_fft_filters_f32(const float* packed, int width, int cin, int cout, int cin_pitch, const float* tables, float* gfwd,
                               void* stream);
+int st_conv1d_fft_filters_shifted_f32(const float* packed, int width, int cin, int cout, int cin_pitch, const float* tables, float* gfwd,
+                                      int row_shift, int src_rows, void* stream);
 size_t st_conv1d_fft_sf_floats(const st_tensor3* x, const st_tensor3* y, int width);
 size_t st_conv1d_fft_zf_floats(const st_tensor3* dz, int width);
 size_t st_conv1d_fft_ws(const st_tensor3* x, const st_tensor3* y, int width);
@@ -104,6 +108,9 @@
 int st_conv1d_nwc_bwd_filter_fft_f32(const st_tensor3* x, const st_tensor3* dz, const float* sf, const float* zf, int width,
                                      const float* tables, float* dpacked, void* workspace, size_t workspace_bytes,
                                      void* stream);
+int st_conv1d_nwc_bwd_filter_fft_bias_f32(const st_tensor3* x, const st_tensor3* dz, const float* sf, const float* zf, int width,
+                                          const float* tables, float* dpacked, float* dbias, int row_shift, int dst_rows,
+                                          void* workspace, size_t workspace_bytes, void* stream);
 
 size_t st_conv1d_fft_filter_plane_elems(int width, int cin_pitch, int cout);
 int st_conv1d_fft_filters_planes(const float* packed, int width, int cin, int cout, int cin_pitch, const float* tables, void* g_planes,
diff --git a/speecht_amd/_lib.py b/speecht_amd/_lib.py
--- a/speecht_amd/_lib.py
+++ b/speecht_amd/_lib.py
@@ -27,6 +27,7 @@
     'st_trace_timed_filter': (c_int, [c_char_p]),
     'st_trace_end': (c_size_t, [c_char_p, c_size_t]),
     'st_set_tuning': (c_int, [c_char_p, c_int]),
+    'st_get_tuning': (c_int, [c_char_p]),
     'st_host_crc32c': (ctypes.c_uint32, [c_void_p, c_size_t, ctypes.c_uint32]),
     'st_packed_dims': (c_int, [c_int, c_int, c_int, POINTER(c_int), POINTER(c_int), POINTER(c_int)]),
     'st_pack_filters_f32': (c_int, [c_void_p, c_int, c_int, c_int, c_int, c_void_p, c_void_p]),
@@ -64,6 +65,7 @@
     'st_conv1d_fft_tables_f32': (c_int, [c_int, c_int, c_void_p, c_size_t, c_void_p]),
     'st_conv1d_fft_filter_floats': (c_size_t, [c_int, c_int, c_int]),
     'st_conv1d_fft_filters_f32': (c_int, [c_void_p, c_int, c_int, c_int, c_int, c_void_p, c_void_p, c_void_p]),
+    'st_conv1d_fft_filters_shifted_f32': (c_int, [c_void_p, c_int, c_int, c_int, c_int, c_void_p, c_void_p, c_int, c_int, c_void_p]),
     'st_conv1d_fft_sf_floats': (c_size_t, [_T3P, _T3P, c_int]),
     'st_conv1d_fft_zf_floats': (c_size_t, [_T3P, c_int]),
     'st_conv1d_fft_ws': (c_size_t, [_T3P, _T3P, c_int]),
@@ -90,6 +92,8 @@
                                                c_void_p]),
     'st_conv1d_nwc_bwd_filter_fft_f32': (c_int, [_T3P, _T3P, c_void_p, c_void_p, c_int, c_void_p, c_void_p, c_void_p,
                                                  c_size_t, c_void_p]),
+    'st_conv1d_nwc_bwd_filter_fft_bias_f32': (c_int, [_T3P, _T3P, c_void_p, c_void_p, c_int, c_void_p, c_void_p, c_void_p, c_int, c_int,
+                                                      c_void_p, c_size_t, c_void_p]),
     'st_conv1d_bwd_data_ws': (c_size_t, [_T3P, _T3P, c_int]),
     'st_conv1d_nwc_bwd_data_f32': (c_int, [_T3P, c_void_p, c_int, c_int, _T3P, _T3P, c_void_p, c_size_t, c_void_p]),
     'st_conv1d_bwd_data_bias_ws': (c_size_t, [_T3P, _T3P, c_int]),
@@ -377,3 +381,7 @@
 def set_tuning(name, value):
   TUNING_EPOCH[0] += 1
   call('st_set_tuning', name.encode(), int(value))
+
+
+def get_tuning(name):
+  return int(load().st_get_tuning(name.encode()))
diff --git a/speecht_amd/csrc/api.hip b/speecht_amd/csrc/api.hip
--- a/speecht_amd/csrc/api.hip
+++ b/speecht_amd/csrc/api.hip
@@ -60,7 +60,8 @@
 }
 
 static const char* const kTuneNames[TUNE_COUNT] = {"streamk", "streamk_slots", "streamk_test_drop", "no_fused_transforms",
-                                                   "bf16_lag_copies", "filters_idft_valu", "bf16_taps_panel", "no_g3", "g3_tile"};
+                                                   "bf16_lag_copies", "filters_idft_valu", "bf16_taps_panel", "no_g3", "g3_tile",
+                                                   "separate_small_launches"};
 static std::atomic<int> g_tune[TUNE_COUNT];
 int tuning(int key) { return g_tune[key].load(std::memory_order_relaxed); }
 }
@@ -152,4 +153,11 @@
   st::set_error("st_set_tuning: unknown knob '%s'", name);
   return ST_EINVAL;
 }
+
+int st_get_tuning(const char* name) {
+  if (name)
+    for (int i = 0; i < st::TUNE_COUNT; ++i)
+      if (!strcmp(name, st::kTuneNames[i])) return st::tuning(i);
+  return 0;
 }
+}
diff --git a/speecht_amd/csrc/conv_fft.hip b/speecht_amd/csrc/conv_fft.hip
--- a/speecht_amd/csrc/conv_fft.hip
+++ b/speecht_amd/csrc/conv_fft.hip
@@ -1,5 +1,6 @@
 #include <algorithm>
 
+#include "small_launches.h"
 #include "st_common.h"
 
 namespace {
@@ -626,14 +627,17 @@
 __global__ __launch_bounds__(256) void filters_dft_fwd_kernel(const float* __restrict__ packed, int width_rt, int cin, int cout,
                                                               int cpi, int cph, int npo, int n, int bins,
                                                               const f32x2* __restrict__ tw, float* __restrict__ gfwd,
-                                                              unsigned short* __restrict__ gb, size_t g_plane) {
+                                                              unsigned short* __restrict__ gb, size_t g_plane, int row_shift, int src_rows) {
   const int width = WT ? WT : width_rt;
   const int o = blockIdx.x * 256 + threadIdx.x, c = blockIdx.y;
   if (o >= npo) return;
   float f[WT ? WT : 64];
   const bool live = c < cin && o < cout;
 #pragma unroll
-  for (int w = 0; w < width; ++w) f[w] = live ? packed[((long)w * cpi + c) * npo + o] : 0.f;
+  for (int w = 0; w < width; ++w) {
+    const int row = st::shifted_tap_row(w * cpi + c, row_shift, src_rows);
+    f[w] = live && row >= 0 ? packed[(long)row * npo + o] : 0.f;
+  }
   const long plane = (long)2 * cph * 2 * npo;
   const int per = (bins + gridDim.z - 1) / gridDim.z, k_lo = blockIdx.z * per, k_hi = min(bins, k_lo + per);
   for (int k = k_lo; k < k_hi; ++k) {
@@ -672,7 +676,7 @@
 template <int WT>
 __global__ __launch_bounds__(256) void filters_idft_kernel(const float* __restrict__ q, int width_rt, int cin, int cout, int cpi, int cph,
                                                            int npo, int n, int bins, const f32x2* __restrict__ tw,
-                                                           float* __restrict__ dpacked, int split) {
+                                                           float* __restrict__ dpacked, int split, int row_shift, int dst_rows) {
   const int width = WT ? WT : width_rt;
   const int o = blockIdx.x * 256 + threadIdx.x, c = blockIdx.y;
   if (o >= npo) return;
@@ -704,19 +708,62 @@
     }
   }
 #pragma unroll
-  for (int w = 0; w < width; ++w) dpacked[((long)w * cpi + c) * npo + o] = acc[w];
+  for (int w = 0; w < width; ++w) {
+    const int row = st::shifted_tap_row(w * cpi + c, row_shift, dst_rows);
+    if (row >= 0) dpacked[(long)row * npo + o] = acc[w];
+  }
+}
+
+struct BiasSum {
+  const float* zf;
+  int rows, ld, channels, np, blocks;
+  float* dbias;
+};
+__device__ __forceinline__ void bias_from_spectra_block(const float* __restrict__ zf, int rows, int ld, int channels, int np,
+                                                        float* __restrict__ dbias, float (*red)[33], int block) {
+  const int cl = threadIdx.x & 31, r = threadIdx.x >> 5;
+  const int c = block * 32 + cl;
+  float s = 0.f;
+  if (c < channels) {
+    float p0 = 0.f, p1 = 0.f, p2 = 0.f, p3 = 0.f;
+    int k = r;
+    for (; k + 24 < rows; k += 32) {
+      const float a = zf[(long)k * ld + c], b = zf[(long)(k + 8) * ld + c], d = zf[(long)(k + 16) * ld + c],
+                  e = zf[(long)(k + 24) * ld + c];
+      p0 += a; p1 += b; p2 += d; p3 += e;
+    }
+    for (; k < rows; k += 8) p0 += zf[(long)k * ld + c];
+    s = (p0 + p1) + (p2 + p3);
+  }
+  red[r][cl] = s;
+  __syncthreads();
+  if (r == 0 && c < np) {
+    float t = red[0][cl];
+#pragma unroll
+    for (int k = 1; k < 8; ++k) t += red[k][cl];
+    dbias[c] = t;
+  }
+}
+__global__ __launch_bounds__(256) void bias_from_spectra_kernel(const float* __restrict__ zf, int rows, int ld, int channels, int np,
+                                                                float* __restrict__ dbias) {
+  __shared__ float red[8][33];
+  bias_from_spectra_block(zf, rows, ld, channels, np, dbias, red, blockIdx.x);
 }
 
 constexpr int FI_CH = 12;
 constexpr int FI_SMAX = 96;
 struct IdftParts { long off[4]; };
-template <int VW>
+template <int VW, bool EXTRA>
 __global__ __launch_bounds__(256, 2) void filters_idft_mfma_kernel(const float* __restrict__ q, int width, int cin, int cout, int cpi,
                                                                    int npo, int n, int bins, const f32x2* __restrict__ tw,
                                                                    float* __restrict__ dpacked, int pshift, long plane, IdftParts parts,
-                                                                   int ld, int ochunks, int items) {
+                                                                   int ld, int ochunks, int items, int row_shift, int dst_rows, BiasSum bias) {
   typedef float vec __attribute__((ext_vector_type(VW)));
   __shared__ float tl[FI_SMAX * 32 * 2];
+  if (EXTRA && (int)blockIdx.x < bias.blocks) {
+    bias_from_spectra_block(bias.zf, bias.rows, bias.ld, bias.channels, bias.np, bias.dbias, reinterpret_cast<float (*)[33]>(tl), blockIdx.x);
+    return;
+  }
   const int nparts = 1 << pshift, S = (nparts * bins) >> 1, stages = (S + FI_CH - 1) / FI_CH;
   {
     const float inv_n = 1.f / (float)n;
@@ -735,7 +782,8 @@
   }
   __syncthreads();
   const int lane = threadIdx.x & 63, l31 = lane & 31, h = lane >> 5;
-  const int gw = blockIdx.x * 4 + (threadIdx.x >> 6), total = gridDim.x * 4;
+  const int first = EXTRA ? bias.blocks : 0;
+  const int gw = (blockIdx.x - first) * 4 + (threadIdx.x >> 6), total = (gridDim.x - first) * 4;
   const float* afrag = tl + 2 * l31 + h;
   for (int item = gw; item < items; item += total) {
     const int c = item / ochunks, o0 = (item - c * ochunks) * (32 * VW) + l31 * VW;
@@ -781,43 +829,17 @@
 #pragma unroll
       for (int r = 0; r < 16; ++r) {
         const int w = (r & 3) + 8 * (r >> 2) + 4 * h;
-        if (w < width) {
+        const int row = EXTRA ? st::shifted_tap_row(w * cpi + c, row_shift, dst_rows) : w * cpi + c;
+        if (w < width && row >= 0) {
           vec v;
 #pragma unroll
           for (int e = 0; e < VW; ++e) {
             v[e] = o0 + e < cout ? acc[e][r] : 0.f;
           }
-          *reinterpret_cast<vec*>(dpacked + ((long)w * cpi + c) * npo + o0) = v;
+          *reinterpret_cast<vec*>(dpacked + (long)row * npo + o0) = v;
         }
       }
     }
-  }
-}
-
-__global__ __launch_bounds__(256) void bias_from_spectra_kernel(const float* __restrict__ zf, int rows, int ld, int channels, int np,
-                                                                float* __restrict__ dbias) {
-  __shared__ float red[8][33];
-  const int cl = threadIdx.x & 31, r = threadIdx.x >> 5;
-  const int c = blockIdx.x * 32 + cl;
-  float s = 0.f;
-  if (c < channels) {
-    float p0 = 0.f, p1 = 0.f, p2 = 0.f, p3 = 0.f;
-    int k = r;
-    for (; k + 24 < rows; k += 32) {
-      const float a = zf[(long)k * ld + c], b = zf[(long)(k + 8) * ld + c], d = zf[(long)(k + 16) * ld + c],
-                  e = zf[(long)(k + 24) * ld + c];
-      p0 += a; p1 += b; p2 += d; p3 += e;
-    }
-    for (; k < rows; k += 8) p0 += zf[(long)k * ld + c];
-    s = (p0 + p1) + (p2 + p3);
-  }
-  red[r][cl] = s;
-  __syncthreads();
-  if (r == 0 && c < np) {
-    float t = red[0][cl];
-#pragma unroll
-    for (int k = 1; k < 8; ++k) t += red[k][cl];
-    dbias[c] = t;
   }
 }
 
@@ -895,10 +917,10 @@
 void launch_filters_planes(int width, const dim3& grid, hipStream_t s, const float* packed, int cin, int cout, int cin_pitch, int cph,
                            int npo, int n, int bins, const f32x2* tw, unsigned short* gb, size_t g_plane) {
   float* none = nullptr;
-  if (width == 32) hipLaunchKernelGGL((filters_dft_fwd_kernel<32, OUTP>), grid, dim3(256), 0, s, packed, width, cin, cout, cin_pitch, cph, npo, n, bins, tw, none, gb, g_plane);
-  else if (width == 25) hipLaunchKernelGGL((filters_dft_fwd_kernel<25, OUTP>), grid, dim3(256), 0, s, packed, width, cin, cout, cin_pitch, cph, npo, n, bins, tw, none, gb, g_plane);
-  else if (width == 7) hipLaunchKernelGGL((filters_dft_fwd_kernel<7, OUTP>), grid, dim3(256), 0, s, packed, width, cin, cout, cin_pitch, cph, npo, n, bins, tw, none, gb, g_plane);
-  else hipLaunchKernelGGL((filters_dft_fwd_kernel<0, OUTP>), grid, dim3(256), 0, s, packed, width, cin, cout, cin_pitch, cph, npo, n, bins, tw, none, gb, g_plane);
+  if (width == 32) hipLaunchKernelGGL((filters_dft_fwd_kernel<32, OUTP>), grid, dim3(256), 0, s, packed, width, cin, cout, cin_pitch, cph, npo, n, bins, tw, none, gb, g_plane, 0, width * cin_pitch);
+  else if (width == 25) hipLaunchKernelGGL((filters_dft_fwd_kernel<25, OUTP>), grid, dim3(256), 0, s, packed, width, cin, cout, cin_pitch, cph, npo, n, bins, tw, none, gb, g_plane, 0, width * cin_pitch);
+  else if (width == 7) hipLaunchKernelGGL((filters_dft_fwd_kernel<7, OUTP>), grid, dim3(256), 0, s, packed, width, cin, cout, cin_pitch, cph, npo, n, bins, tw, none, gb, g_plane, 0, width * cin_pitch);
+  else hipLaunchKernelGGL((filters_dft_fwd_kernel<0, OUTP>), grid, dim3(256), 0, s, packed, width, cin, cout, cin_pitch, cph, npo, n, bins, tw, none, gb, g_plane, 0, width * cin_pitch);
 }
 
 bool planes_ok(int planes) { return planes == 1 || planes == 3; }
@@ -912,7 +934,8 @@
 
 
 void launch_filters_idft(const float* qf, int width, int cin, int cout, int cpi, int cph, int npo, int n, int bins, const f32x2* tw,
-                         float* dpacked, int split, hipStream_t s) {
+                         float* dpacked, int split, hipStream_t s, int row_shift = 0, int dst_rows = 0, const BiasSum* bias = nullptr) {
+  if (dst_rows <= 0) { row_shift = 0; dst_rows = width * cpi; }
   if (width <= 32 && npo % 128 == 0 && (split ? 2 : 4) * bins <= 2 * FI_SMAX && st::tuning(st::TUNE_FILTERS_IDFT_VALU) == 0) {
     IdftParts parts;
     long plane;
@@ -926,22 +949,35 @@
     }
     const int vw = (long)cpi * (npo / 128) >= 2048 ? 4 : ((long)cpi * (npo / 64) >= 2048 ? 2 : 1);
     const int ochunks = npo / (32 * vw), items = cpi * ochunks;
-    const dim3 grid(std::min(1024, st::ceil_div(items, 4)));
+    const bool extra = vw == 1 || bias || row_shift != 0 || dst_rows != width * cpi;
+    const BiasSum bsum = bias ? *bias : BiasSum{};
+    const dim3 grid(std::min(1024, st::ceil_div(items, 4)) + bsum.blocks);
     st::trace("filters_idft_mfma<%d> taps=%d bins=%d parts=%d items=%d gflop=%.3f mb=%.2f", vw, width, bins, split ? 2 : 4, items,
               4096e-9 * items * (double)vw * st::ceil_div((split ? 2 : 4) * bins / 2, FI_CH) * FI_CH,
               1e-6 * 4 * ((double)(split ? 2 : 4) * bins * cin * npo + (double)width * cpi * npo));
     st::LaunchTimer timer(s);
-#define ST_FI(VWV) st::launch_timed(timer, filters_idft_mfma_kernel<VWV>, grid, dim3(256), s, qf, width, cin, cout, cpi, npo, n, bins, tw, dpacked, \
-                                    split ? 1 : 2, plane, parts, ld, ochunks, items)
-    if (vw == 4) ST_FI(4); else if (vw == 2) ST_FI(2); else ST_FI(1);
+#define ST_FI(VWV, EX) st::launch_timed(timer, filters_idft_mfma_kernel<VWV, EX>, grid, dim3(256), s, qf, width, cin, cout, cpi, npo, n, bins, tw, dpacked, \
+                                        split ? 1 : 2, plane, parts, ld, ochunks, items, row_shift, dst_rows, bsum)
+    if (vw == 4) { if (extra) ST_FI(4, true); else ST_FI(4, false); }
+    else if (vw == 2) { if (extra) ST_FI(2, true); else ST_FI(2, false); }
+    else ST_FI(1, true);
 #undef ST_FI
     return;
   }
   const dim3 grid(st::ceil_div(npo, 256), cpi);
-  if (width == 32) hipLaunchKernelGGL(filters_idft_kernel<32>, grid, dim3(256), 0, s, qf, width, cin, cout, cpi, cph, npo, n, bins, tw, dpacked, split);
-  else if (width == 25) hipLaunchKernelGGL(filters_idft_kernel<25>, grid, dim3(256), 0, s, qf, width, cin, cout, cpi, cph, npo, n, bins, tw, dpacked, split);
-  else if (width == 7) hipLaunchKernelGGL(filters_idft_kernel<7>, grid, dim3(256), 0, s, qf, width, cin, cout, cpi, cph, npo, n, bins, tw, dpacked, split);
-  else hipLaunchKernelGGL(filters_idft_kernel<0>, grid, dim3(256), 0, s, qf, width, cin, cout, cpi, cph, npo, n, bins, tw, dpacked, split);
+  if (width == 32) hipLaunchKernelGGL(filters_idft_kernel<32>, grid, dim3(256), 0, s, qf, width, cin, cout, cpi, cph, npo, n, bins, tw, dpacked, split, row_shift, dst_rows);
+  else if (width == 25) hipLaunchKernelGGL(filters_idft_kernel<25>, grid, dim3(256), 0, s, qf, width, cin, cout, cpi, cph, npo, n, bins, tw, dpacked, split, row_shift, dst_rows);
+  else if (width == 7) hipLaunchKernelGGL(filters_idft_kernel<7>, grid, dim3(256), 0, s, qf, width, cin, cout, cpi, cph, npo, n, bins, tw, dpacked, split, row_shift, dst_rows);
+  else hipLaunchKernelGGL(filters_idft_kernel<0>, grid, dim3(256), 0, s, qf, width, cin, cout, cpi, cph, npo, n, bins, tw, dpacked, split, row_shift, dst_rows);
+  if (bias)
+    hipLaunchKernelGGL(bias_from_spectra_kernel, dim3(bias->blocks), dim3(256), 0, s, bias->zf, bias->rows, bias->ld, bias->channels, bias->np,
+                       bias->dbias);
+}
+
+BiasSum bias_sum_of(const st_tensor3& dz, int width, const Plan& p, const float* zf, float* dbias) {
+  const int np = st::npad_of(dz.channels);
+  const bool zf3 = zf3_form(width, dz.channels);
+  return BiasSum{zf + (zf3 ? np : 0), p.rows, (zf3 ? 3 : 2) * np, dz.channels, np, st::ceil_div(np, 32), dbias};
 }
 
 }
@@ -1037,6 +1073,12 @@
 
 int st_conv1d_fft_filters_f32(const float* packed, int width, int cin, int cout, int cin_pitch, const float* tables, float* gfwd,
                               void* stream) {
+  return st_conv1d_fft_filters_shifted_f32(packed, width, cin, cout, cin_pitch, tables, gfwd, 0, width * cin_pitch, stream);
+}
+
+int st_conv1d_fft_filters_shifted_f32(const float* packed, int width, int cin, int cout, int cin_pitch, const float* tables, float* gfwd,
+                                      int row_shift, int src_rows, void* stream) {
+  ST_REQUIRE(row_shift >= 0 && src_rows > 0, "fft filters: bad row shift");
   ST_REQUIRE(width_ok(width) && cin_pitch % 16 == 0 && tables && packed && gfwd, "fft filters: bad argument");
   ST_REQUIRE(st::npad_of(cout) % 128 == 0, "fft filters: the output channels must pack to a multiple of 128");
   hipStream_t s = st::as_stream(stream);
@@ -1053,12 +1095,12 @@
   const int gx = st::ceil_div(npo, 256), gy = half_of(cin_pitch);
   const dim3 grid(gx, gy, gx * gy < 1024 ? 4 : 1);
   if (g3_form(width, cin_pitch, cout)) {
-    if (width == 32) hipLaunchKernelGGL((filters_dft_fwd_kernel<32, 4>), grid, dim3(256), 0, s, packed, width, cin, cout, cin_pitch, half_of(cin_pitch), npo, n, bins, tw, gfwd, (unsigned short*)nullptr, (size_t)0);
-    else hipLaunchKernelGGL((filters_dft_fwd_kernel<0, 4>), grid, dim3(256), 0, s, packed, width, cin, cout, cin_pitch, half_of(cin_pitch), npo, n, bins, tw, gfwd, (unsigned short*)nullptr, (size_t)0);
+    if (width == 32) hipLaunchKernelGGL((filters_dft_fwd_kernel<32, 4>), grid, dim3(256), 0, s, packed, width, cin, cout, cin_pitch, half_of(cin_pitch), npo, n, bins, tw, gfwd, (unsigned short*)nullptr, (size_t)0, row_shift, src_rows);
+    else hipLaunchKernelGGL((filters_dft_fwd_kernel<0, 4>), grid, dim3(256), 0, s, packed, width, cin, cout, cin_pitch, half_of(cin_pitch), npo, n, bins, tw, gfwd, (unsigned short*)nullptr, (size_t)0, row_shift, src_rows);
     return st::check_launch("fft filters (three planes)");
   }
   ST_FFT_WIDTH_DISPATCH(filters_dft_fwd_kernel, packed, width, cin, cout, cin_pitch, half_of(cin_pitch), npo, n, bins, tw, gfwd,
-                        (unsigned short*)nullptr, (size_t)0);
+                        (unsigned short*)nullptr, (size_t)0, row_shift, src_rows);
   return st::check_launch("fft filters");
 }
 
@@ -1156,10 +1198,8 @@
 int st_conv1d_fft_bias_grad_f32(const st_tensor3* dz, int width, const float* zf, float* dbias, void* stream) {
   ST_REQUIRE(st::tensor_ok(dz) && zf && dbias && width_ok(width) && st::npad_of(dz->channels) % 128 == 0, "conv fft bias grad: bad argument");
   const Plan p = make_plan(width, dz->frames, dz->batch, ROWS_F32);
-  const int np = st::npad_of(dz->channels);
-  const bool zf3 = zf3_form(width, dz->channels);
-  hipLaunchKernelGGL(bias_from_spectra_kernel, dim3(st::ceil_div(np, 32)), dim3(256), 0, st::as_stream(stream), zf + (zf3 ? np : 0), p.rows,
-                     (zf3 ? 3 : 2) * np, dz->channels, np, dbias);
+  const BiasSum b = bias_sum_of(*dz, width, p, zf, dbias);
+  hipLaunchKernelGGL(bias_from_spectra_kernel, dim3(b.blocks), dim3(256), 0, st::as_stream(stream), b.zf, b.rows, b.ld, b.channels, b.np, b.dbias);
   return st::check_launch("conv fft bias grad");
 }
 
@@ -1375,6 +1415,13 @@
 
 int st_conv1d_nwc_bwd_filter_fft_f32(const st_tensor3* x, const st_tensor3* dz, const float* sf, const float* zf, int width,
                                      const float* tables, float* dpacked, void* workspace, size_t workspace_bytes, void* stream) {
+  return st_conv1d_nwc_bwd_filter_fft_bias_f32(x, dz, sf, zf, width, tables, dpacked, nullptr, 0, 0, workspace, workspace_bytes, stream);
+}
+
+int st_conv1d_nwc_bwd_filter_fft_bias_f32(const st_tensor3* x, const st_tensor3* dz, const float* sf, const float* zf, int width,
+                                          const float* tables, float* dpacked, float* dbias, int row_shift, int dst_rows, void* workspace,
+                                          size_t workspace_bytes, void* stream) {
+  ST_REQUIRE(row_shift >= 0 && dst_rows >= 0, "conv fft bwd_filter: bad row shift");
   ST_REQUIRE(st::tensor_ok(x) && st::tensor_ok(dz) && sf && zf && dpacked && workspace && tables && width_ok(width), "conv fft bwd_filter: bad argument");
   ST_REQUIRE(x->batch == dz->batch && x->frames == dz->frames, "conv fft bwd_filter: stride-1 layers only");
   ST_REQUIRE(st::npad_of(dz->channels) % 128 == 0 && workspace_bytes >= st_conv1d_fft_ws(x, dz, width), "conv fft bwd_filter: workspace / shape");
@@ -1385,22 +1432,24 @@
   float* qf = reinterpret_cast<float*>(workspace) + st::SK_WS_FLOATS;
   const long s_bin = 2L * p.rows_pad * ka;
   const bool zf3 = zf3_form(width, dz->channels);
+  const BiasSum bsum = bias_sum_of(*dz, width, p, zf, dbias);
+  const BiasSum* bias = dbias ? &bsum : nullptr;
   if (g3_form(width, x->c_pitch, dz->channels)) {
     const long a_off[3] = {2L * half, 3L * half, 0}, z_off[3] = {0, 2L * npo, npo};
     if (int e = st::gemm_tn_g3_batched(sf, 4L * half, s_bin, a_off, zf, 3L * npo, (long)p.rows_pad * 3 * npo, z_off, qf, 2L * half * npo,
                                        (long)half * npo, p.rows_pad, half, npo, p.bins, s))
       return e;
-    launch_filters_idft(qf, width, x->channels, dz->channels, x->c_pitch, half, npo, p.n, p.bins, tw, dpacked, 1, s);
+    launch_filters_idft(qf, width, x->channels, dz->channels, x->c_pitch, half, npo, p.n, p.bins, tw, dpacked, 1, s, row_shift, dst_rows, bias);
   } else if (split_lag_products(half)) {
     if (int e = st::gemm_tn_batched(sf, half, (long)p.rows_pad * ka, zf, npo, (long)p.rows_pad * nf, qf, (long)half * npo, 2 * p.rows_pad,
                                     half, npo, 2 * p.bins, s, 1))
       return e;
-    launch_filters_idft(qf, width, x->channels, dz->channels, x->c_pitch, half, npo, p.n, p.bins, tw, dpacked, 1, s);
+    launch_filters_idft(qf, width, x->channels, dz->channels, x->c_pitch, half, npo, p.n, p.bins, tw, dpacked, 1, s, row_shift, dst_rows, bias);
   } else {
     if (int e = st::gemm_tn_batched(sf, ka, s_bin, zf + (zf3 ? npo : 0), zf3 ? 3L * npo : nf, (long)p.rows_pad * (zf3 ? 3 * npo : nf), qf, (long)ka * nf,
                                     p.rows_pad, ka, nf, p.bins, s))
       return e;
-    launch_filters_idft(qf, width, x->channels, dz->channels, x->c_pitch, half, npo, p.n, p.bins, tw, dpacked, 0, s);
+    launch_filters_idft(qf, width, x->channels, dz->channels, x->c_pitch, half, npo, p.n, p.bins, tw, dpacked, 0, s, row_shift, dst_rows, bias);
   }
   return st::check_launch("conv fft bwd_filter");
 }
diff --git a/speecht_amd/csrc/conv_gemm.hip b/speecht_amd/csrc/conv_gemm.hip
--- a/speecht_amd/csrc/conv_gemm.hip
+++ b/speecht_amd/csrc/conv_gemm.hip
@@ -5,6 +5,7 @@
 
 #include <type_traits>
 
+#include "small_launches.h"
 #include "st_common.h"
 #include "streamk_map.h"
 
@@ -1406,10 +1407,8 @@
     st::set_error("gemm_tn_batched: bad shape M=%d K=%d N=%d tile_n=%d", M, K, N, tile_n);
     return ST_EINVAL;
   }
-  if (tile_n == 0) {
-    const long tiles128 = (long)batches * (K / 128) * (N / 128);
-    tile_n = (tiles128 > 256 && tiles128 <= 320 && M <= 512) ? 64 : 128;
-  }
+  if (tile_n == 0)
+    tile_n = st::tn_tile_by_shape((long)batches * (K / 128) * (N / 128), M, st::tuning(st::TUNE_SEPARATE_SMALL_LAUNCHES) != 0);
   TNParams p{};
   p.A = A;
   p.amap.frames = M; p.amap.row_stride = (int)lda; p.amap.batch_stride = 0; p.amap.row0 = 0;
diff --git a/speecht_amd/csrc/small_launches.h b/speecht_amd/csrc/small_launches.h
--- /dev/null
+++ b/speecht_amd/csrc/small_launches.h
@@ -0,0 +1,22 @@
+#pragma once
+
+#if defined(__HIPCC__)
+#define ST_HD __host__ __device__
+#else
+#define ST_HD
+#endif
+
+namespace st {
+
+ST_HD inline int tn_tile_by_shape(long tiles128, int M, bool one_round_only) {
+  if (M > 512 || tiles128 <= 256) return 128;
+  const long full = (tiles128 - 1) / 256, last = tiles128 - full * 256;
+  return last <= 64 && full <= (one_round_only ? 1 : 2) ? 64 : 128;
+}
+
+ST_HD inline int shifted_tap_row(int w, int shift, int rows) {
+  const int r = w - shift;
+  return r >= 0 && r < rows ? r : -1;
+}
+
+}
diff --git a/speecht_amd/csrc/st_common.h b/speecht_amd/csrc/st_common.h
--- a/speecht_amd/csrc/st_common.h
+++ b/speecht_amd/csrc/st_common.h
@@ -30,7 +30,7 @@
   else hipLaunchKernelGGL(kernel, grid, block, 0, s, static_cast<KArgs>(args)...);
 }
 enum { TUNE_STREAMK, TUNE_STREAMK_SLOTS, TUNE_STREAMK_TEST_DROP, TUNE_NO_FUSED_TRANSFORMS, TUNE_BF16_LAG_COPIES, TUNE_FILTERS_IDFT_VALU,
-       TUNE_BF16_TAPS_PANEL, TUNE_NO_G3, TUNE_G3_TILE, TUNE_COUNT };
+       TUNE_BF16_TAPS_PANEL, TUNE_NO_G3, TUNE_G3_TILE, TUNE_SEPARATE_SMALL_LAUNCHES, TUNE_COUNT };
 int tuning(int key);
 
 constexpr int SK_FLAGS = 0, SK_TIMEOUTS = 768, SK_CTRL_WORDS = 1024;
diff --git a/speecht_amd/modes/fp32.py b/speecht_amd/modes/fp32.py
--- a/speecht_amd/modes/fp32.py
+++ b/speecht_amd/modes/fp32.py
@@ -190,6 +190,15 @@
         polyphase = f['shift'] is not None
 
         def filter_gradient(f=f, l=l, i=i, gf=gf, gb=gb, need_bias=need_bias, polyphase=polyphase, ws=f.get('ws2', f['ws'])):
+          separate = _lib.get_tuning('separate_small_launches')
+          if (polyphase and 'dpacked2' not in f) or (not polyphase and not separate):
+            cp = X[i].c_pitch
+            call('st_conv1d_nwc_bwd_filter_fft_bias_f32', f['xref'], dZ[i].ref, ptr(f['sf']), ptr(f['zf']), f['width'], ptr(f['tables']),
+                 ptr(gf), ptr(gb) if need_bias and not separate else None, f['shift'] * cp if polyphase else 0,
+                 l.width * cp if polyphase else 0, ptr(ws), ws.numel() * 4, e.stream_ptr)
+            if need_bias and separate:
+              call('st_conv1d_fft_bias_grad_f32', dZ[i].ref, f['width'], ptr(f['zf']), ptr(gb), e.stream_ptr)
+            return
           call('st_conv1d_nwc_bwd_filter_fft_f32', f['xref'], dZ[i].ref, ptr(f['sf']), ptr(f['zf']), f['width'], ptr(f['tables']),
                ptr(f['dpacked2'] if polyphase else gf), ptr(ws), ws.numel() * 4, e.stream_ptr)
           if polyphase:
diff --git a/speecht_amd/modes/spectral.py b/speecht_amd/modes/spectral.py
--- a/speecht_amd/modes/spectral.py
+++ b/speecht_amd/modes/spectral.py
@@ -16,6 +16,9 @@
     pl2 = (pl + 1) // 2
     shift = 2 * pl2 - pl
     return (l.width + shift + 1) // 2, pl2, shift
+
+  def _shift_in_kernel(self):
+    return self.e.conv_mode == 'fp32' and not _lib.get_tuning('separate_small_launches')
 
   def _use_fft(self, i, batch, geo):
     e = self.e
@@ -46,12 +49,13 @@
         cp2 = 2 * x.c_pitch
         f.update(x=Tensor3(x.buf.data_ptr(), batch, t_out, cp2, x.halo // 2, x.t_pitch // 2, cp2), width=width2, pl=pl2,
                  cin=cp2, cin_pitch=cp2, shift=shift)
-        rows = 2 * width2 * x.c_pitch * l.n_pad
-        f['packed2'], fresh_p = view('packed2', rows)
-        f['dpacked2'] = view('dpacked2', rows)[0]
-        if fresh_p:
-          f['packed2'].zero_()
-          self._gfwd_fresh = False
+        if not self._shift_in_kernel():
+          rows = 2 * width2 * x.c_pitch * l.n_pad
+          f['packed2'], fresh_p = view('packed2', rows)
+          f['dpacked2'] = view('dpacked2', rows)[0]
+          if fresh_p:
+            f['packed2'].zero_()
+            self._gfwd_fresh = False
       f['xref'] = ctypes.byref(f['x'])
       tables, fresh_tables = view('tables', lib.st_conv1d_fft_table_floats())
       if self._fft_table_key.get(i) != (f['width'], f['pl']):
@@ -92,14 +96,19 @@
         continue
       l = e.layers[i]
       pf = e._slice(e.params, i)[0]
-      if f['shift'] is not None:
+      if f['shift'] is not None and 'packed2' not in f:
         cp = sh.X[i].c_pitch
-        n = l.width * cp * l.n_pad
-        with torch.cuda.stream(stream):
-          f['packed2'][f['shift'] * cp * l.n_pad:f['shift'] * cp * l.n_pad + n].copy_(pf[:n], non_blocking=True)
-        pf = f['packed2']
-      call('st_conv1d_fft_filters_f32', ptr(pf), f['width'], f['cin'], l.cout, f['cin_pitch'], ptr(f['tables']), ptr(f['gfwd']),
-           e.stream_ptr)
+        call('st_conv1d_fft_filters_shifted_f32', ptr(pf), f['width'], f['cin'], l.cout, f['cin_pitch'], ptr(f['tables']),
+             ptr(f['gfwd']), f['shift'] * cp, l.width * cp, e.stream_ptr)
+      else:
+        if f['shift'] is not None:
+          cp = sh.X[i].c_pitch
+          n = l.width * cp * l.n_pad
+          with torch.cuda.stream(stream):
+            f['packed2'][f['shift'] * cp * l.n_pad:f['shift'] * cp * l.n_pad + n].copy_(pf[:n], non_blocking=True)
+          pf = f['packed2']
+        call('st_conv1d_fft_filters_f32', ptr(pf), f['width'], f['cin'], l.cout, f['cin_pitch'], ptr(f['tables']), ptr(f['gfwd']),
+             e.stream_ptr)
       if stream is e._side:
         ev = torch.cuda.Event()
         ev.record(stream)
```

New measurement: 4899 (median of 6 runs). Within noise of the previous version (+0.3%).
